# ugadiarov-la-phystech-edu/OCRL

Measured on AMD Instinct MI355X. Metric: images/sec (node) SLATE pretrain 128x128, 6 slots, 3 iters, higher is better.
Workload: dtype f32

## Files before the change

include/ocrl_hip.h:

```cpp
#ifndef OCRL_HIP_H
#define OCRL_HIP_H
#include <stddef.h>

#ifdef __cplusplus
extern "C" {
#endif

#define OCRL_ABI_VERSION 5

const char* ocrl_last_error(void);
int ocrl_abi_version(void);

typedef struct ocrl_slate ocrl_slate;
typedef struct ocrl_slate_config {
    int obs_size, obs_channels;
    int vocab_size, d_model;
    int cnn_hidden;
    int num_slots, num_iterations, slot_size, mlp_hidden;
    int num_dec_blocks, num_dec_heads;
    float dropout;
    int max_batch;
    int use_bcdec;
    int hard;
    int num_slot_heads;
} ocrl_slate_config;

size_t ocrl_slate_config_size(void);
int ocrl_slate_create(const ocrl_slate_config* cfg, ocrl_slate** out);
void ocrl_slate_destroy(ocrl_slate* h);

int ocrl_slate_param_count(const ocrl_slate* h);
int ocrl_slate_param_info(const ocrl_slate* h, int i, char* name, int name_cap, int shape[4], int* ndim,
                          long long* offset, long long* numel, int* group);
long long ocrl_slate_flat_size(const ocrl_slate* h);
long long ocrl_slate_group_begin(const ocrl_slate* h, int group);
size_t ocrl_slate_workspace_bytes(const ocrl_slate* h);

int ocrl_slate_bind(ocrl_slate* h, float* params, float* grads, float* adam_m, float* adam_v, void* workspace, size_t workspace_bytes);

int ocrl_slate_forward(ocrl_slate* h, const float* obs, int B, float tau, int train, unsigned long long seed,
                       const float* noise_z, const float* noise_zh, const float* noise_slots, void* stream);
int ocrl_slate_backward(ocrl_slate* h, void* stream);
int ocrl_slate_encode(ocrl_slate* h, const float* obs, int B, unsigned long long seed, const float* noise_slots, void* stream);
int ocrl_slate_encode_backward(ocrl_slate* h, const float* dslots, void* stream);
int ocrl_slate_freeze_weights(ocrl_slate* h, int on);
int ocrl_slate_generate(ocrl_slate* h, void* stream);
int ocrl_slate_clip_adam(ocrl_slate* h, const float lr[3], float clip, int step, float grad_scale, void* stream);
int ocrl_slate_grad_norm(ocrl_slate* h, void* stream);
float* ocrl_slate_metrics(const ocrl_slate* h);
int ocrl_slate_tensor(const ocrl_slate* h, const char* name, float** ptr, long long* count);
int ocrl_slate_soft_z(ocrl_slate* h, void* stream);
int ocrl_slate_dropout_mask(const ocrl_slate* h, unsigned site, long long n, float* out, void* stream);

int ocrl_gemm(const float* A, const float* B, float* C, int M, int N, int K, int lda, int ldb, int ldc, int akc, int bkc,
              float alpha, const float* bias, int relu, const float* mask, int ldmask, const float* resid, int ldr,
              int splitk, float* ws, void* stream);
typedef struct ocrl_gemm_desc {
    const float* A; const float* B; float* C;
    int M, N, K, lda, ldb, ldc;
    int akc, bkc;
    int batch, batch_inner;
    long long sA, sB, sC, sAi, sBi, sCi;
    int splitk; float alpha;
    const float* bias; int relu;
    float drop_p; unsigned long long drop_seed; unsigned drop_site;
    const float* mask; int ldmask; long long sMask; int mask_elu;
    const float* resid; int ldr; long long sR;
    float adrop_p; unsigned adrop_site; int adrop_ld;
    float* bias_out; long long sBias;
    int a_mode, b_mode; const float* x_lse; const int* x_tok; float x_scale;
    int epi_mode; float* stat; float* hstat; int* hidx; const float* e1; const float* e2; unsigned long long e_seed;
    const float* e_lse; const float* e_rowvec; float e_scale;
    int force_tile, force_sb;
} ocrl_gemm_desc;
size_t ocrl_gemm_desc_size(void);
int ocrl_gemm_ex(const ocrl_gemm_desc* d, float* ws, size_t ws_floats, void* stream);
int ocrl_gemm_plan(const ocrl_gemm_desc* d, int out[6]);
int ocrl_conv2d_fwd(const float* x, const float* w, const float* bias, float* y, int B, int H, int W, int cin, int cin_pad, int ks,
                    int relu, float* ws, void* stream);
int ocrl_conv2d_fwd_lowlat(const float* x, const float* w, const float* bias, float* y, int B, int H, int W, int cin, int cin_pad, int ks,
                           int relu, float* ws, void* stream);
size_t ocrl_conv2d_x3_ws_floats(void);
int ocrl_conv2d_fwd_x3(const float* x, const float* w, const float* bias, float* y, int B, int H, int W, int ks, int relu, float* ws, void* stream);
int ocrl_conv2d_bwd_data_x3(const float* dy, const float* w, const float* mask, float* dx, int B, int H, int W, int ks, float* ws, void* stream);
int ocrl_conv2d_bwd_weight_x3(const float* x, const float* dy, float* dw, int B, int H, int W, int ks, float* ws, size_t ws_floats, void* stream);
int ocrl_conv2d_bwd_data(const float* dy, const float* w, const float* mask, float* dx, int B, int H, int W, int ks, float* ws, void* stream);
size_t ocrl_conv2d_wgrad_ws_floats(int B, int H, int W, int ks, int cin_pad);
int ocrl_conv2d_bwd_weight(const float* x, const float* dy, float* dw, float* db, int B, int H, int W, int cin, int cin_pad, int ks,
                           float* ws, size_t ws_floats, void* stream);
typedef struct ocrl_conv_desc {
    const float* x; const float* w; float* y;
    int B, H, W, cin, cin_pad, ks;
    const float* bias; int relu;
    const float* posmap; const float* mask; int mask_elu;
    int transposed, low_latency;
} ocrl_conv_desc;
size_t ocrl_conv_desc_size(void);
int ocrl_conv2d_ex(const ocrl_conv_desc* d, float* ws, size_t ws_floats, void* stream);
typedef struct ocrl_conv_wgrad_desc {
    const float* x; const float* dy; float* dw; float* db;
    int B, H, W, cin, cin_pad, ks;
    int accumulate;
} ocrl_conv_wgrad_desc;
size_t ocrl_conv_wgrad_desc_size(void);
int ocrl_conv2d_bwd_weight_ex(const ocrl_conv_wgrad_desc* d, float* ws, size_t ws_floats, void* stream);
size_t ocrl_conv2d_first_fwd_ws_floats(void);
int ocrl_conv2d_first_fwd(const float* obs, const float* w, const float* bias, float* y, int B, int H, int W, int relu, float* ws, size_t ws_floats,
                          void* stream);
size_t ocrl_conv2d_first_wgrad_ws_floats(int B, int H, int W);
int ocrl_conv2d_first_bwd_weight(const float* obs, const float* dy, float* dw, float* db, int B, int H, int W, int accumulate, float* ws, size_t ws_floats,
                                 void* stream);
int ocrl_layernorm_fwd(const float* x, const float* gamma, const float* beta, float* y, float* mean, float* rstd, long long R, int F, void* stream);
int ocrl_layernorm_bwd(const float* dy, const float* x, const float* mean, const float* rstd, const float* gamma, float* dx, float* dgb,
                       long long R, int F, float* ws, size_t ws_floats, void* stream);

int ocrl_sa_input_plan(long long R, int out[3]);
int ocrl_sa_input_fwd(const float* e4, const float* gamma, const float* beta, const float* W0, const float* b0, const float* W2, const float* b2,
                      float* mean, float* rstd, float* h1, float* x, long long R, int max_wgs, void* stream);
int ocrl_sa_input_bwd(const float* dx, const float* h1, const float* e4, const float* mean, const float* rstd, const float* gamma, const float* beta,
                      const float* W0, const float* W2, float* de4, float* dW0, float* db0, float* dW2, float* db2, float* dgamma, float* dbeta,
                      long long R, int max_wgs, float* ws, size_t ws_floats, void* stream);

int ocrl_attention_fwd(const float* q, const float* k, const float* v, float* o, float* lse, int B, int T, int d, int h, int ld,
                       float p, unsigned long long seed, unsigned site, void* stream);
int ocrl_attention_bwd(const float* q, const float* k, const float* v, const float* o, const float* lse, const float* dO,
                       float* dq, float* dk, float* dv, float* delta, int B, int T, int d, int h, int ld,
                       float p, unsigned long long seed, unsigned site, void* stream);

int ocrl_obs_u8_to_f32(const unsigned char* obs_hwc, float* obs_chw, int B, int H, int W, int C, void* stream);

int ocrl_prof_enable(unsigned tag_mask);
int ocrl_prof_collect(double* ms, long long* count, int ntags);

size_t ocrl_slot_attention_ws_floats(int B, int K, int D, int H, int I);
int ocrl_slot_attention_fwd(const float* x, const float* slots0, const float* const* w, float* slots, float* attn, int B, int N, int K, int D,
                            int H, int I, float* ws, size_t ws_floats, void* stream);
int ocrl_slot_attention_bwd(const float* x, const float* dslots, float* dx, float* dslots0, float* const* dw, int B, int N, int K, int D, int H,
                            int I, float* ws, size_t ws_floats, void* stream);
size_t ocrl_slot_attention_mh_ws_floats(int B, int N, int K, int D, int H, int I, int heads);
int ocrl_slot_attention_mh_fwd(const float* x, const float* slots0, const float* const* w, float* slots, float* attn, int B, int N, int K, int D,
                               int H, int I, int heads, float* ws, size_t ws_floats, void* stream);
int ocrl_slot_attention_mh_bwd(const float* x, const float* dslots, float* dx, float* dslots0, float* const* dw, int B, int N, int K, int D, int H,
                               int I, int heads, float* ws, size_t ws_floats, void* stream);
int ocrl_slot_attention_plan(int K, int D, int H, int heads, int* out6);

#define OCRL_POOL_MAX_LAYERS 8
size_t ocrl_pool_transformer_ws_floats(int B, int K, int d, int nhead, int ff, int L);
int ocrl_pool_transformer_fwd(const float* slots, const float* const* w, const float* pos, float* out, int B, int K, int Din, int d, int nhead,
                              int ff, int L, float drop_p, unsigned long long seed, float* ws, size_t ws_floats, void* stream);
int ocrl_pool_transformer_bwd(const float* slots, const float* dout, const float* const* w, float* dslots, float* const* dw, int B, int K, int Din,
                              int d, int nhead, int ff, int L, float drop_p, unsigned long long seed, float* ws, size_t ws_floats, void* stream);
int ocrl_pool_transformer_dropout_mask(int layer, int which, long long n, float drop_p, unsigned long long seed, float* out, void* stream);
size_t ocrl_pool_transformer_long_ws_floats(int B, int K, int Din, int d, int nhead, int ff, int L);
int ocrl_pool_transformer_long_fwd(const float* slots, const float* const* w, const float* pos, float* out, int B, int K, int Din, int d, int nhead,
                                   int ff, int L, float drop_p, unsigned long long seed, float* ws, size_t ws_floats, void* stream);
int ocrl_pool_transformer_long_bwd(const float* slots, const float* dout, const float* const* w, float* dslots, float* const* dw, int B, int K,
                                   int Din, int d, int nhead, int ff, int L, float drop_p, unsigned long long seed, float* ws, size_t ws_floats,
                                   void* stream);

#define OCRL_POOL_RN_MAX_LAYERS 16
size_t ocrl_pool_rn_ws_floats(int B, int K, int D, int ng, const int* g_dims, int nf, const int* f_dims);
int ocrl_pool_rn_fwd(const float* slots, const float* const* w, float* out, int B, int K, int D, int ng, const int* g_dims, int nf, const int* f_dims,
                     float* ws, size_t ws_floats, void* stream);
int ocrl_pool_rn_bwd(const float* slots, const float* dout, const float* const* w, float* dslots, float* const* dw, int B, int K, int D, int ng,
                     const int* g_dims, int nf, const int* f_dims, float* ws, size_t ws_floats, void* stream);

#define OCRL_NATURECNN_MAX_GROUPS 16
#define OCRL_NATURECNN_MAX_CONVS 4
size_t ocrl_naturecnn_ws_floats(int B, int H, int W, int cin, int groups, int cnn_feat_size, int use_cnn_feat, int rep_dim);
int ocrl_naturecnn_fwd(const float* obs, const float* const* w, float* out, int B, int H, int W, int cin, int groups, int cnn_feat_size,
                       int use_cnn_feat, int rep_dim, int save, float* ws, size_t ws_floats, void* stream);
int ocrl_naturecnn_bwd(const float* obs, const float* dout, const float* const* w, float* const* dw, int B, int H, int W, int cin, int groups,
                       int cnn_feat_size, int use_cnn_feat, int rep_dim, float* ws, size_t ws_floats, void* stream);

size_t ocrl_pool_cnn_ws_floats(int B, int H, int W, int D, int rep_dim);
int ocrl_pool_cnn_fwd(const float* tokens, const float* const* w, float* out, int B, int H, int W, int D, int rep_dim, int save, float* ws,
                      size_t ws_floats, void* stream);
int ocrl_pool_cnn_bwd(const float* tokens, const float* dout, const float* const* w, float* dtokens, float* const* dw, int B, int H, int W, int D,
                      int rep_dim, float* ws, size_t ws_floats, void* stream);

#define OCRL_VAE_MAX_STAGES 6
size_t ocrl_vae_ws_floats(int B, int obs_size, int obs_channels, int cnn_feat_size, int latent_dim, int use_cnn_feat, int full);
int ocrl_vae_fwd(const float* obs, const float* const* w, const float* eps, float* rep, float* metrics, float* recon, int B, int obs_size,
                 int obs_channels, int cnn_feat_size, int latent_dim, int use_cnn_feat, float kld_weight, int full, float* ws, size_t ws_floats,
                 void* stream);
int ocrl_vae_bwd(const float* obs, const float* eps, const float* const* w, const float* dloss, const float* drep, float* const* dw, int B,
                 int obs_size, int obs_channels, int cnn_feat_size, int latent_dim, int use_cnn_feat, float kld_weight, int full, float* ws,
                 size_t ws_floats, void* stream);

#define OCRL_MAE_MAX_DEPTH 32
size_t ocrl_mae_ws_floats(int B, int obs_size, int patch, int D, int depth, int heads, int Dd, int ddepth, int dheads, int len_keep, int full);
int ocrl_mae_fwd(const float* obs, const float* const* w, const float* noise, float* rep, float* metrics, float* pred, float* mask,
                 int* ids_restore, int B, int obs_size, int patch, int D, int depth, int heads, int Dd, int ddepth, int dheads, int len_keep,
                 int full, float* ws, size_t ws_floats, void* stream);
int ocrl_mae_bwd(const float* obs, const float* const* w, const float* dloss, const float* drep, float* const* dw, int B, int obs_size,
                 int patch, int D, int depth, int heads, int Dd, int ddepth, int dheads, int len_keep, int full, float* ws, size_t ws_floats,
                 void* stream);
int ocrl_mae_rank(const float* noise, int* ids_restore, int* ids_keep, float* mask, int B, int L, int len_keep, void* stream);

#define OCRL_PROBE_MAX_SLOTS 12
#define OCRL_PROBE_MAX_PROPS 8
#define OCRL_PROBE_MAX_LAYERS 8
size_t ocrl_probe_ws_floats(int B, int K, int N, int D, int O, int slot_rows, int nl, const int* dims, int P);
int ocrl_probe_fwd(const float* rows, const float* const* w, const float* y, float* out, float* cost, int* col, float* metrics, int B, int K, int N,
                   int D, int T, int O, int slot_rows, int nl, const int* dims, float slope, int P, const int* tgt_range, const int* out_range,
                   const int* kind, float* ws, size_t ws_floats, void* stream);
int ocrl_probe_bwd(const float* rows, const float* dloss, const float* const* w, float* const* dw, int B, int K, int N, int D, int O, int slot_rows,
                   int nl, const int* dims, float slope, int P, float* ws, size_t ws_floats, void* stream);
size_t ocrl_probe_match_ws_floats(int B, int P);
int ocrl_probe_match(const float* out, int ld_row, long long ld_img, const float* y, const float* dloss, float* cost, int* col, float* metrics,
                     float* dout, int B, int K, int N, int T, int O, int P, const int* tgt_range, const int* out_range, const int* kind, float* ws,
                     size_t ws_floats, void* stream);

#define OCRL_ARI_MAX_CHANNELS 32
int ocrl_ari_counts(const float* truth, long long t_sb, long long t_sc, long long t_sn, int Ct, const float* pred, long long p_sb,
                    long long p_sc, long long p_sn, int Cp, int fuse_fg, int B, long long N, int* table, long long* sums, void* stream);

#define OCRL_ACNET_MAX_LAYERS 8
typedef struct {
    int B, F, A;
    int n[3];
    int dims[3][OCRL_ACNET_MAX_LAYERS];
    int acts[3][OCRL_ACNET_MAX_LAYERS];
} ocrl_acnet_desc;
size_t ocrl_acnet_desc_size(void);
size_t ocrl_acnet_ws_floats(const ocrl_acnet_desc* d);
int ocrl_acnet_fwd(const ocrl_acnet_desc* d, const float* features, const float* const* w, float* latent_pi, float* latent_vf, float* logits,
                   float* values, int save, float* ws, size_t ws_floats, void* stream);
int ocrl_acnet_bwd(const ocrl_acnet_desc* d, const float* features, const float* const* w, const float* dlatent_pi, const float* dlatent_vf,
                   const float* dlogits, const float* dvalues, float* dfeatures, float* const* dw, float* ws, size_t ws_floats, void* stream);
int ocrl_acnet_ppo_fwd_bwd(const ocrl_acnet_desc* d, const float* features, const float* const* w, const long long* actions,
                           const float* old_log_prob, const float* advantages, const float* returns, float clip_range, float vf_coef,
                           float ent_coef, int normalize_advantage, float* scalars, float* dfeatures, float* const* dw, float* ws,
                           size_t ws_floats, void* stream);
int ocrl_acnet_a2c_fwd_bwd(const ocrl_acnet_desc* d, const float* features, const float* const* w, const long long* actions,
                           const float* advantages, const float* returns, float vf_coef, float ent_coef, int normalize_advantage,
                           float* scalars, float* dfeatures, float* const* dw, float* ws, size_t ws_floats, void* stream);
int ocrl_acnet_act(const ocrl_acnet_desc* d, const float* features, const float* const* w, unsigned long long seed,
                   unsigned long long row_offset, const float* uniforms , int deterministic, long long* actions, float* values,
                   float* log_prob, float* logits , void* stream);
int ocrl_acnet_act_uniforms(unsigned long long seed, unsigned long long row_offset, long long n, float* out, void* stream);
int ocrl_gae(const float* rewards, const float* values, const float* episode_starts, const float* last_values, const float* dones,
             float* advantages, float* returns, int T, int E, float gamma, float gae_lambda, void* stream);

#define OCRL_SPRITE_MAX_OBJECTS 15
typedef struct {
    int E, H;
    int lo, hi;
    int mode;
    int rew_type;
    int occlusion, max_steps;
    int n_colors, n_shapes, n_scales;
    int colors[8], shapes[8];
    float scales[8];
    int target_color, target_shape;
    float target_scale;
    int agent_color, agent_shape;
    float agent_scale, agent_x, agent_y;
    float step_size, dist_agent, dist_objs, dist_wall;
    int task;
    int obj_comp;
    int unseen_mode;
    int unseen_colors[2];
} ocrl_sprite_env_desc;
size_t ocrl_sprite_env_desc_size(void);
size_t ocrl_sprite_env_state_floats(const ocrl_sprite_env_desc* d);
int ocrl_sprite_env_reset(const ocrl_sprite_env_desc* d, float* state, unsigned long long seed, const unsigned char* mask ,
                          long long episode, void* stream);
// ... 65 lines not shown
```

ocrl_amd/_lib.py:

```python
import ctypes
import os
from ctypes import POINTER, c_char_p, c_float, c_int, c_longlong, c_size_t, c_uint, c_ulonglong, c_void_p

_HERE = os.path.dirname(os.path.abspath(__file__))
LIB_PATH = os.environ.get("OCRL_HIP_LIB") or os.path.join(_HERE, "libocrl_hip.so")
_lib = None


class SlateConfig(ctypes.Structure):
    _fields_ = [(n, c_int) for n in ("obs_size", "obs_channels", "vocab_size", "d_model", "cnn_hidden", "num_slots",
                                      "num_iterations", "slot_size", "mlp_hidden", "num_dec_blocks", "num_dec_heads")] + \
               [("dropout", c_float), ("max_batch", c_int), ("use_bcdec", c_int), ("hard", c_int), ("num_slot_heads", c_int)]


class IodineConfig(ctypes.Structure):
    _fields_ = [(n, c_int) for n in ("obs_size", "obs_channels", "slot_size", "num_iterations", "num_slots")] + \
               [("sigma", c_float), ("beta", c_float), ("layer_norm", c_int), ("ref_mlp_hidden", c_int), ("max_batch", c_int)]


class GemmDesc(ctypes.Structure):
    _fields_ = [("A", c_void_p), ("B", c_void_p), ("C", c_void_p)] + \
               [(n, c_int) for n in ("M", "N", "K", "lda", "ldb", "ldc", "akc", "bkc", "batch", "batch_inner")] + \
               [(n, c_longlong) for n in ("sA", "sB", "sC", "sAi", "sBi", "sCi")] + \
               [("splitk", c_int), ("alpha", c_float), ("bias", c_void_p), ("relu", c_int),
                ("drop_p", c_float), ("drop_seed", c_ulonglong), ("drop_site", c_uint),
                ("mask", c_void_p), ("ldmask", c_int), ("sMask", c_longlong), ("mask_elu", c_int),
                ("resid", c_void_p), ("ldr", c_int), ("sR", c_longlong),
                ("adrop_p", c_float), ("adrop_site", c_uint), ("adrop_ld", c_int),
                ("bias_out", c_void_p), ("sBias", c_longlong),
                ("a_mode", c_int), ("b_mode", c_int), ("x_lse", c_void_p), ("x_tok", c_void_p), ("x_scale", c_float),
                ("epi_mode", c_int), ("stat", c_void_p), ("hstat", c_void_p), ("hidx", c_void_p), ("e1", c_void_p), ("e2", c_void_p),
                ("e_seed", c_ulonglong), ("e_lse", c_void_p), ("e_rowvec", c_void_p), ("e_scale", c_float),
                ("force_tile", c_int), ("force_sb", c_int)]


class ConvDesc(ctypes.Structure):
    _fields_ = [("x", c_void_p), ("w", c_void_p), ("y", c_void_p)] + \
               [(n, c_int) for n in ("B", "H", "W", "cin", "cin_pad", "ks")] + \
               [("bias", c_void_p), ("relu", c_int), ("posmap", c_void_p), ("mask", c_void_p), ("mask_elu", c_int),
                ("transposed", c_int), ("low_latency", c_int)]


class ConvWgradDesc(ctypes.Structure):
    _fields_ = [("x", c_void_p), ("dy", c_void_p), ("dw", c_void_p), ("db", c_void_p)] + \
               [(n, c_int) for n in ("B", "H", "W", "cin", "cin_pad", "ks", "accumulate")]


class AcnetDesc(ctypes.Structure):
    _fields_ = [("B", c_int), ("F", c_int), ("A", c_int), ("n", c_int * 3), ("dims", (c_int * 8) * 3), ("acts", (c_int * 8) * 3)]


class SpriteEnvDesc(ctypes.Structure):
    _fields_ = [(n, c_int) for n in ("E", "H", "lo", "hi", "mode", "rew_type", "occlusion", "max_steps", "n_colors", "n_shapes", "n_scales")] + \
               [("colors", c_int * 8), ("shapes", c_int * 8), ("scales", c_float * 8), ("target_color", c_int), ("target_shape", c_int),
                ("target_scale", c_float), ("agent_color", c_int), ("agent_shape", c_int)] + \
               [(n, c_float) for n in ("agent_scale", "agent_x", "agent_y", "step_size", "dist_agent", "dist_objs", "dist_wall")] + \
               [("task", c_int), ("obj_comp", c_int), ("unseen_mode", c_int), ("unseen_colors", c_int * 2)]


class ScenesDesc(ctypes.Structure):
    _fields_ = [("H", c_int), ("K", c_int)]


def acnet_desc(B, F, A, dims, acts):
    d = AcnetDesc(B=B, F=F, A=A)
    for t in range(3):
        if len(dims[t]) > 8:
            raise ValueError(f"ocrl_amd: at most 8 layers per trunk (got {len(dims[t])})")
        d.n[t] = len(dims[t])
        for l, (w, a) in enumerate(zip(dims[t], acts[t])):
            d.dims[t][l], d.acts[t][l] = int(w), int(a)
    return d


def gemm_desc(**kw):
    d = GemmDesc(batch=1, batch_inner=1, splitk=1, alpha=1.0, x_scale=1.0, e_scale=1.0, force_sb=-1)
    for k, v in kw.items():
        setattr(d, k, v)
    return d


def conv_desc(**kw):
    d = ConvDesc()
    for k, v in kw.items():
        setattr(d, k, v)
    return d


def conv_wgrad_desc(**kw):
    d = ConvWgradDesc()
    for k, v in kw.items():
        setattr(d, k, v)
    return d


def lib():
    global _lib
    if _lib is not None:
        return _lib
    if not os.path.exists(LIB_PATH):
        raise RuntimeError(
            f"{LIB_PATH} is missing: build it with `python -c 'import __graft_entry__ as g; g.build()'` "
            "(make -C ocrl_amd/csrc).  ocrl_amd has no CPU fallback.")
    import torch
    L = ctypes.CDLL(LIB_PATH)
    p = c_void_p
    L.ocrl_last_error.restype = c_char_p
    L.ocrl_abi_version.restype = c_int
    L.ocrl_slate_config_size.restype = c_size_t
    if L.ocrl_slate_config_size() != ctypes.sizeof(SlateConfig):
        raise RuntimeError(f"libocrl_hip.so: ocrl_slate_config is {L.ocrl_slate_config_size()} bytes, this binding's SlateConfig {ctypes.sizeof(SlateConfig)}")
    L.ocrl_slate_create.argtypes = [POINTER(SlateConfig), POINTER(p)]
    L.ocrl_slate_destroy.argtypes = [p]
    L.ocrl_slate_destroy.restype = None
    L.ocrl_slate_param_count.argtypes = [p]
    L.ocrl_slate_param_info.argtypes = [p, c_int, c_char_p, c_int, POINTER(c_int * 4), POINTER(c_int), POINTER(c_longlong),
                                        POINTER(c_longlong), POINTER(c_int)]
    L.ocrl_slate_flat_size.argtypes = [p]
    L.ocrl_slate_flat_size.restype = c_longlong
    L.ocrl_slate_group_begin.argtypes = [p, c_int]
    L.ocrl_slate_group_begin.restype = c_longlong
    L.ocrl_slate_workspace_bytes.argtypes = [p]
    L.ocrl_slate_workspace_bytes.restype = c_size_t
    L.ocrl_slate_bind.argtypes = [p, p, p, p, p, p, c_size_t]
    L.ocrl_slate_forward.argtypes = [p, p, c_int, c_float, c_int, c_ulonglong, p, p, p, p]
    L.ocrl_slate_backward.argtypes = [p, p]
    L.ocrl_slate_generate.argtypes = [p, p]
    L.ocrl_slate_encode.argtypes = [p, p, c_int, c_ulonglong, p, p]
    L.ocrl_slate_encode_backward.argtypes = [p, p, p]
    L.ocrl_slate_freeze_weights.argtypes = [p, c_int]
    L.ocrl_slate_clip_adam.argtypes = [p, POINTER(c_float * 3), c_float, c_int, c_float, p]
    L.ocrl_slate_grad_norm.argtypes = [p, p]
    L.ocrl_slate_metrics.argtypes = [p]
    L.ocrl_slate_metrics.restype = p
    L.ocrl_slate_tensor.argtypes = [p, c_char_p, POINTER(p), POINTER(c_longlong)]
    L.ocrl_slate_dropout_mask.argtypes = [p, c_uint, c_longlong, p, p]
    L.ocrl_slate_soft_z.argtypes = [p, p]
    L.ocrl_gemm.argtypes = [p, p, p, c_int, c_int, c_int, c_int, c_int, c_int, c_int, c_int, c_float, p, c_int, p, c_int, p, c_int,
                            c_int, p, p]
    L.ocrl_gemm_desc_size.restype = c_size_t
    L.ocrl_gemm_ex.argtypes = [POINTER(GemmDesc), p, c_size_t, p]
    L.ocrl_gemm_plan.argtypes = [POINTER(GemmDesc), POINTER(c_int * 6)]
    L.ocrl_conv2d_fwd.argtypes = [p, p, p, p, c_int, c_int, c_int, c_int, c_int, c_int, c_int, p, p]
    L.ocrl_conv2d_fwd_lowlat.argtypes = [p, p, p, p, c_int, c_int, c_int, c_int, c_int, c_int, c_int, p, p]
    L.ocrl_conv2d_x3_ws_floats.restype = c_size_t
    L.ocrl_conv2d_fwd_x3.argtypes = [p, p, p, p, c_int, c_int, c_int, c_int, c_int, p, p]
    L.ocrl_conv2d_bwd_data_x3.argtypes = [p, p, p, p, c_int, c_int, c_int, c_int, p, p]
    L.ocrl_conv2d_bwd_weight_x3.argtypes = [p, p, p, c_int, c_int, c_int, c_int, p, c_size_t, p]
    L.ocrl_conv2d_bwd_data.argtypes = [p, p, p, p, c_int, c_int, c_int, c_int, p, p]
    L.ocrl_conv2d_wgrad_ws_floats.argtypes = [c_int, c_int, c_int, c_int, c_int]
    L.ocrl_conv2d_wgrad_ws_floats.restype = c_size_t
    L.ocrl_conv2d_bwd_weight.argtypes = [p, p, p, p, c_int, c_int, c_int, c_int, c_int, c_int, p, c_size_t, p]
    L.ocrl_conv_desc_size.restype = c_size_t
    L.ocrl_conv_wgrad_desc_size.restype = c_size_t
    for name, cls in (("ocrl_conv_desc", ConvDesc), ("ocrl_conv_wgrad_desc", ConvWgradDesc)):
        n = getattr(L, name + "_size")()
        if n != ctypes.sizeof(cls):
            raise RuntimeError(f"libocrl_hip.so: {name} is {n} bytes, this binding's {cls.__name__} {ctypes.sizeof(cls)}")
    L.ocrl_conv2d_ex.argtypes = [POINTER(ConvDesc), p, c_size_t, p]
    L.ocrl_conv2d_bwd_weight_ex.argtypes = [POINTER(ConvWgradDesc), p, c_size_t, p]
    L.ocrl_conv2d_first_fwd_ws_floats.restype = c_size_t
    L.ocrl_conv2d_first_fwd.argtypes = [p, p, p, p, c_int, c_int, c_int, c_int, p, c_size_t, p]
    L.ocrl_conv2d_first_wgrad_ws_floats.argtypes = [c_int, c_int, c_int]
    L.ocrl_conv2d_first_wgrad_ws_floats.restype = c_size_t
    L.ocrl_conv2d_first_bwd_weight.argtypes = [p, p, p, p, c_int, c_int, c_int, c_int, p, c_size_t, p]
    L.ocrl_layernorm_fwd.argtypes = [p, p, p, p, p, p, c_longlong, c_int, p]
    L.ocrl_layernorm_bwd.argtypes = [p, p, p, p, p, p, p, c_longlong, c_int, p, c_size_t, p]
    L.ocrl_sa_input_plan.argtypes = [c_longlong, POINTER(c_int * 3)]
    L.ocrl_sa_input_fwd.argtypes = [p] * 11 + [c_longlong, c_int, p]
    L.ocrl_sa_input_bwd.argtypes = [p] * 16 + [c_longlong, c_int, p, c_size_t, p]
    L.ocrl_attention_fwd.argtypes = [p, p, p, p, p, c_int, c_int, c_int, c_int, c_int, c_float, c_ulonglong, c_uint, p]
    L.ocrl_attention_bwd.argtypes = [p, p, p, p, p, p, p, p, p, p, c_int, c_int, c_int, c_int, c_int, c_float, c_ulonglong, c_uint, p]
    L.ocrl_obs_u8_to_f32.argtypes = [p, p, c_int, c_int, c_int, c_int, p]
    L.ocrl_prof_enable.argtypes = [c_uint]
    L.ocrl_prof_collect.argtypes = [POINTER(ctypes.c_double * 8), POINTER(c_longlong * 8), c_int]
    L.ocrl_iodine_create.argtypes = [POINTER(IodineConfig), POINTER(p)]
    L.ocrl_iodine_destroy.argtypes = [p]
    L.ocrl_iodine_destroy.restype = None
    L.ocrl_iodine_param_count.argtypes = [p]
    L.ocrl_iodine_param_info.argtypes = [p, c_int, c_char_p, c_int, POINTER(c_int * 4), POINTER(c_int), POINTER(c_longlong), POINTER(c_longlong)]
    L.ocrl_iodine_flat_size.argtypes = [p]
    L.ocrl_iodine_flat_size.restype = c_longlong
    L.ocrl_iodine_workspace_bytes.argtypes = [p]
    L.ocrl_iodine_workspace_bytes.restype = c_size_t
    L.ocrl_iodine_bind.argtypes = [p, p, p, p, p, p, c_size_t]
    L.ocrl_iodine_forward.argtypes = [p, p, c_int, c_ulonglong, p, p]
    L.ocrl_iodine_backward.argtypes = [p, p]
    L.ocrl_iodine_clip_adam.argtypes = [p, c_float, c_float, c_int, c_float, p]
    L.ocrl_iodine_grad_norm.argtypes = [p, p]
    L.ocrl_iodine_metrics.argtypes = [p]
    L.ocrl_iodine_metrics.restype = p
    L.ocrl_iodine_tensor.argtypes = [p, c_char_p, POINTER(p), POINTER(c_longlong)]
    L.ocrl_slot_attention_ws_floats.argtypes = [c_int, c_int, c_int, c_int, c_int]
    L.ocrl_slot_attention_ws_floats.restype = c_size_t
    L.ocrl_slot_attention_fwd.argtypes = [p, p, POINTER(p), p, p, c_int, c_int, c_int, c_int, c_int, c_int, p, c_size_t, p]
    L.ocrl_slot_attention_bwd.argtypes = [p, p, p, p, POINTER(p), c_int, c_int, c_int, c_int, c_int, c_int, p, c_size_t, p]
    L.ocrl_slot_attention_mh_ws_floats.argtypes = [c_int] * 7
    L.ocrl_slot_attention_mh_ws_floats.restype = c_size_t
    L.ocrl_slot_attention_mh_fwd.argtypes = [p, p, POINTER(p), p, p] + [c_int] * 7 + [p, c_size_t, p]
    L.ocrl_slot_attention_mh_bwd.argtypes = [p, p, p, p, POINTER(p)] + [c_int] * 7 + [p, c_size_t, p]
    L.ocrl_slot_attention_plan.argtypes = [c_int, c_int, c_int, c_int, POINTER(c_int * 6)]
    L.ocrl_pool_transformer_ws_floats.argtypes = [c_int, c_int, c_int, c_int, c_int, c_int]
    L.ocrl_pool_transformer_ws_floats.restype = c_size_t
    L.ocrl_pool_transformer_fwd.argtypes = [p, POINTER(p), p, p, c_int, c_int, c_int, c_int, c_int, c_int, c_int, c_float, c_ulonglong, p, c_size_t, p]
    L.ocrl_pool_transformer_bwd.argtypes = [p, p, POINTER(p), p, POINTER(p), c_int, c_int, c_int, c_int, c_int, c_int, c_int, c_float, c_ulonglong, p,
                                            c_size_t, p]
    L.ocrl_pool_transformer_dropout_mask.argtypes = [c_int, c_int, c_longlong, c_float, c_ulonglong, p, p]
    L.ocrl_pool_transformer_long_ws_floats.argtypes = [c_int] * 7
    L.ocrl_pool_transformer_long_ws_floats.restype = c_size_t
    L.ocrl_pool_transformer_long_fwd.argtypes = L.ocrl_pool_transformer_fwd.argtypes
    L.ocrl_pool_transformer_long_bwd.argtypes = L.ocrl_pool_transformer_bwd.argtypes
    L.ocrl_pool_rn_ws_floats.argtypes = [c_int, c_int, c_int, c_int, POINTER(c_int), c_int, POINTER(c_int)]
    L.ocrl_pool_rn_ws_floats.restype = c_size_t
    L.ocrl_pool_rn_fwd.argtypes = [p, POINTER(p), p, c_int, c_int, c_int, c_int, POINTER(c_int), c_int, POINTER(c_int), p, c_size_t, p]
    L.ocrl_pool_rn_bwd.argtypes = [p, p, POINTER(p), p, POINTER(p), c_int, c_int, c_int, c_int, POINTER(c_int), c_int, POINTER(c_int), p, c_size_t, p]
    L.ocrl_naturecnn_ws_floats.argtypes = [c_int] * 8
    L.ocrl_naturecnn_ws_floats.restype = c_size_t
    L.ocrl_naturecnn_fwd.argtypes = [p, POINTER(p), p] + [c_int] * 9 + [p, c_size_t, p]
    L.ocrl_naturecnn_bwd.argtypes = [p, p, POINTER(p), POINTER(p)] + [c_int] * 8 + [p, c_size_t, p]
    L.ocrl_pool_cnn_ws_floats.argtypes = [c_int] * 5
    L.ocrl_pool_cnn_ws_floats.restype = c_size_t
    L.ocrl_pool_cnn_fwd.argtypes = [p, POINTER(p), p] + [c_int] * 6 + [p, c_size_t, p]
    L.ocrl_pool_cnn_bwd.argtypes = [p, p, POINTER(p), p, POINTER(p)] + [c_int] * 5 + [p, c_size_t, p]
    L.ocrl_vae_ws_floats.argtypes = [c_int] * 7
    L.ocrl_vae_ws_floats.restype = c_size_t
    L.ocrl_vae_fwd.argtypes = [p, POINTER(p), p, p, p, p] + [c_int] * 6 + [c_float, c_int, p, c_size_t, p]
    L.ocrl_vae_bwd.argtypes = [p, p, POINTER(p), p, p, POINTER(p)] + [c_int] * 6 + [c_float, c_int, p, c_size_t, p]
    L.ocrl_mae_ws_floats.argtypes = [c_int] * 11
    L.ocrl_mae_ws_floats.restype = c_size_t
    L.ocrl_mae_fwd.argtypes = [p, POINTER(p), p, p, p, p, p, p] + [c_int] * 11 + [p, c_size_t, p]
    L.ocrl_mae_bwd.argtypes = [p, POINTER(p), p, p, POINTER(p)] + [c_int] * 11 + [p, c_size_t, p]
    L.ocrl_mae_rank.argtypes = [p, p, p, p, c_int, c_int, c_int, p]
    L.ocrl_probe_ws_floats.argtypes = [c_int] * 7 + [POINTER(c_int), c_int]
    L.ocrl_probe_ws_floats.restype = c_size_t
    L.ocrl_probe_fwd.argtypes = [p, POINTER(p), p, p, p, p, p] + [c_int] * 8 + [POINTER(c_int), c_float, c_int, POINTER(c_int), POINTER(c_int),
                                 POINTER(c_int), p, c_size_t, p]
    L.ocrl_probe_bwd.argtypes = [p, p, POINTER(p), POINTER(p)] + [c_int] * 7 + [POINTER(c_int), c_float, c_int, p, c_size_t, p]
    L.ocrl_probe_match_ws_floats.argtypes = [c_int, c_int]
    L.ocrl_probe_match_ws_floats.restype = c_size_t
    L.ocrl_probe_match.argtypes = [p, c_int, c_longlong, p, p, p, p, p, p] + [c_int] * 6 + [POINTER(c_int)] * 3 + [p, c_size_t, p]
    L.ocrl_ari_counts.argtypes = [p, c_longlong, c_longlong, c_longlong, c_int, p, c_longlong, c_longlong, c_longlong, c_int, c_int, c_int, c_longlong, p, p, p]
    L.ocrl_acnet_desc_size.restype = c_size_t
    if L.ocrl_acnet_desc_size() != ctypes.sizeof(AcnetDesc):
        raise RuntimeError(f"libocrl_hip.so: ocrl_acnet_desc is {L.ocrl_acnet_desc_size()} bytes, this binding's AcnetDesc {ctypes.sizeof(AcnetDesc)}")
    L.ocrl_acnet_ws_floats.argtypes = [POINTER(AcnetDesc)]
    L.ocrl_acnet_ws_floats.restype = c_size_t
    L.ocrl_acnet_fwd.argtypes = [POINTER(AcnetDesc), p, POINTER(p), p, p, p, p, c_int, p, c_size_t, p]
    L.ocrl_acnet_bwd.argtypes = [POINTER(AcnetDesc), p, POINTER(p), p, p, p, p, p, POINTER(p), p, c_size_t, p]
    L.ocrl_acnet_ppo_fwd_bwd.argtypes = [POINTER(AcnetDesc), p, POINTER(p), p, p, p, p, c_float, c_float, c_float, c_int, p, p, POINTER(p), p, c_size_t, p]
    L.ocrl_acnet_a2c_fwd_bwd.argtypes = [POINTER(AcnetDesc), p, POINTER(p), p, p, p, c_float, c_float, c_int, p, p, POINTER(p), p, c_size_t, p]
    L.ocrl_acnet_act.argtypes = [POINTER(AcnetDesc), p, POINTER(p), c_ulonglong, c_ulonglong, p, c_int, p, p, p, p, p]
    L.ocrl_acnet_act_uniforms.argtypes = [c_ulonglong, c_ulonglong, c_longlong, p, p]
    L.ocrl_flat_clip_adam_ws_floats.argtypes = []
    L.ocrl_flat_clip_adam_ws_floats.restype = c_size_t
    L.ocrl_flat_clip_adam_l2.argtypes = [p, p, p, p, c_longlong, c_float, c_float, c_float, c_float, c_float, c_int, p, p, c_size_t, p]
    L.ocrl_flat_clip_rmsprop_ws_floats.argtypes = []
    L.ocrl_flat_clip_rmsprop_ws_floats.restype = c_size_t
    L.ocrl_flat_clip_rmsprop_l2.argtypes = [p, p, p, c_longlong, c_float, c_float, c_float, c_float, p, p, c_size_t, p]
    L.ocrl_gae.argtypes = [p, p, p, p, p, p, p, c_int, c_int, c_float, c_float, p]
    L.ocrl_sprite_env_desc_size.restype = c_size_t
    if L.ocrl_sprite_env_desc_size() != ctypes.sizeof(SpriteEnvDesc):
        raise RuntimeError(f"libocrl_hip.so: ocrl_sprite_env_desc is {L.ocrl_sprite_env_desc_size()} bytes, this binding's SpriteEnvDesc "
                           f"{ctypes.sizeof(SpriteEnvDesc)}")
    L.ocrl_sprite_env_state_floats.argtypes = [POINTER(SpriteEnvDesc)]
    L.ocrl_sprite_env_state_floats.restype = c_size_t
    L.ocrl_sprite_env_reset.argtypes = [POINTER(SpriteEnvDesc), p, c_ulonglong, p, c_longlong, p]
    L.ocrl_sprite_env_step.argtypes = [POINTER(SpriteEnvDesc), p, c_ulonglong, p, p, p, p, p, p, p]
    L.ocrl_sprite_render.argtypes = [p, c_int, c_int, c_int, c_int, p, p]
    L.ocrl_sprite_state_obs.argtypes = [p, c_int, c_int, p, p]
    L.ocrl_gt_mlp_ws_floats.argtypes = [c_int, c_int, c_int, POINTER(c_int)]
    L.ocrl_gt_mlp_ws_floats.restype = c_size_t
    L.ocrl_gt_mlp_fwd.argtypes = [p, POINTER(p), p, c_int, c_int, c_int, POINTER(c_int), POINTER(c_int), p, c_size_t, p]
    L.ocrl_gt_mlp_bwd.argtypes = [p, p, POINTER(p), p, POINTER(p), c_int, c_int, c_int, POINTER(c_int), POINTER(c_int), p, c_size_t, p]
    L.ocrl_sprite_env_uniforms.argtypes = [c_ulonglong, c_longlong, c_int, c_longlong, c_int, c_int, p, p]
    L.ocrl_scenes_batch.argtypes = [POINTER(ScenesDesc), c_ulonglong, p, c_int, p, p, p, p, p]
    L.ocrl_scenes_uniforms.argtypes = [c_ulonglong, c_longlong, c_int, c_int, p, p]
    L.ocrl_comm_unique_id.argtypes = [p, c_size_t]
    L.ocrl_comm_init.argtypes = [POINTER(p), c_int, c_int, p]
    L.ocrl_comm_allreduce.argtypes = [p, p, c_longlong, p]
    L.ocrl_comm_world.argtypes = [p]
    L.ocrl_comm_destroy.argtypes = [p]
    L.ocrl_comm_destroy.restype = None
    if L.ocrl_abi_version() != 5:
        raise RuntimeError("libocrl_hip.so ABI version mismatch")
    _lib = L
    return L


def check(rc):
    if rc:
        raise RuntimeError("ocrl_hip: " + lib().ocrl_last_error().decode())


def ptr(t):
    return None if t is None else ctypes.c_void_p(t.data_ptr())


def ptrs(ts):
    return (ctypes.c_void_p * len(ts))(*[t.data_ptr() if t is not None else None for t in ts])


def stream(device=None):
    import torch
    return ctypes.c_void_p(torch.cuda.current_stream(device).cuda_stream)
```

ocrl_amd/csrc/capi.cpp:

```cpp
#include <stdarg.h>
#include <stdint.h>
#include <string.h>

#include <new>

#include "../../include/ocrl_hip.h"
#include "iodine_model.h"
#include "slate_model.h"

static thread_local char g_err[512] = "";

void ocrl_set_error(const char* fmt, ...) {
    va_list ap;
    va_start(ap, fmt);
    vsnprintf(g_err, sizeof g_err, fmt, ap);
    va_end(ap);
}

template <class M>
struct Handle {
    using Model = M;
    M* m = nullptr;
};
struct ocrl_slate : Handle<SlateModel> {};
// ... 140 lines not shown
    a.A = d.A; a.B = d.B; a.C = d.C; a.M = d.M; a.N = d.N; a.K = d.K; a.lda = d.lda; a.ldb = d.ldb; a.ldc = d.ldc; a.akc = d.akc; a.bkc = d.bkc;
    a.batch = d.batch; a.batch_inner = d.batch_inner; a.sA = d.sA; a.sB = d.sB; a.sC = d.sC; a.sAi = d.sAi; a.sBi = d.sBi; a.sCi = d.sCi;
    a.splitk = d.splitk; a.alpha = d.alpha; a.bias = d.bias; a.relu = d.relu; a.drop_p = d.drop_p; a.drop_seed = d.drop_seed; a.drop_site = d.drop_site;
    a.mask = d.mask; a.ldmask = d.ldmask; a.sMask = d.sMask; a.mask_elu = d.mask_elu; a.resid = d.resid; a.ldr = d.ldr; a.sR = d.sR;
    a.adrop_p = d.adrop_p; a.adrop_site = d.adrop_site; a.adrop_ld = d.adrop_ld; a.bias_out = d.bias_out; a.sBias = d.sBias;
    a.a_mode = d.a_mode; a.b_mode = d.b_mode; a.x_lse = d.x_lse; a.x_tok = d.x_tok; a.x_scale = d.x_scale;
    a.epi_mode = d.epi_mode; a.stat = d.stat; a.hstat = d.hstat; a.hidx = d.hidx; a.e1 = d.e1; a.e2 = d.e2; a.e_seed = d.e_seed;
    a.e_lse = d.e_lse; a.e_rowvec = d.e_rowvec; a.e_scale = d.e_scale; a.force_tile = d.force_tile; a.force_sb = d.force_sb;
    return a;
}
size_t ocrl_gemm_desc_size(void) { return sizeof(ocrl_gemm_desc); }
int ocrl_gemm_plan(const ocrl_gemm_desc* d, int out[6]) {
    if (!d || !out) { ocrl_set_error("ocrl_gemm_plan: null argument"); return 1; }
    GemmArgs a = gemm_args(*d);
    if (a.splitk > 1) gemm_splitk_layout(a, a.C, a.sBias ? a.sBias : (a.M + 3) & ~3);
    GemmPlan p;
    if (gemm_plan(a, &p)) return 1;
    out[0] = p.bm; out[1] = p.bn; out[2] = p.sb; out[3] = p.xf; out[4] = p.epi; out[5] = p.layout;
    return 0;
}
int ocrl_gemm_ex(const ocrl_gemm_desc* d, float* ws, size_t ws_floats, void* stream) {
    if (!d) { ocrl_set_error("ocrl_gemm_ex: null descriptor"); return 1; }
    GemmArgs a = gemm_args(*d);
    if (a.splitk <= 1) return gemm_launch(a, ST(stream));
    const long long slab = (long long)a.M * a.N, bslab = a.sBias ? a.sBias : (a.M + 3) & ~3;
    const size_t need = (size_t)a.splitk * slab + (a.bias_out ? (size_t)a.splitk * bslab : 0);
    if (a.ldc != a.N || !ws || ws_floats < need || bslab % 4) {
        ocrl_set_error("ocrl_gemm_ex: split-k needs ldc == N, sBias %% 4 == 0 and a workspace of %zu floats", need);
        return 1;
    }
    if (a.bias || a.relu || a.drop_p > 0.f || a.mask || a.resid || a.epi_mode) {
        ocrl_set_error("ocrl_gemm_ex: split-k partial products take no epilogue");
        return 1;
    }
    return gemm_splitk_launch(a, ws, bslab, 0, ST(stream));
}
int ocrl_conv2d_fwd(const float* x, const float* w, const float* bias, float* y, int B, int H, int W, int cin, int cin_pad, int ks, int relu,
                    float* ws, void* stream) {
    if (conv_pack_launch(w, ws, nullptr, ks, cin_pad, 64, cin, ST(stream))) return 1;
    ConvArgs a;
    a.X = x; a.Wp = ws; a.Y = y; a.B = B; a.H = H; a.W = W; a.bias = bias; a.relu = relu;
    return conv_fwd_launch(a, ks, cin_pad, 64, ST(stream));
}
int ocrl_conv2d_fwd_lowlat(const float* x, const float* w, const float* bias, float* y, int B, int H, int W, int cin, int cin_pad, int ks, int relu,
                           float* ws, void* stream) {
    if (conv_pack_launch(w, ws, nullptr, ks, cin_pad, 64, cin, ST(stream))) return 1;
    ConvArgs a;
    a.X = x; a.Wp = ws; a.Y = y; a.B = B; a.H = H; a.W = W; a.bias = bias; a.relu = relu;
    return conv_fwd_launch(a, ks, cin_pad, 64, ST(stream), 1);
}
size_t ocrl_conv2d_x3_ws_floats(void) { return 2 * conv_x3_pack_floats(5); }
int ocrl_conv2d_fwd_x3(const float* x, const float* w, const float* bias, float* y, int B, int H, int W, int ks, int relu, float* ws, void* stream) {
    if (ks != 3 && ks != 5) { ocrl_set_error("ocrl_conv2d_fwd_x3: ks must be 3 or 5"); return 1; }
    if (conv_pack_x3_launch(w, ws, nullptr, ST(stream), ks)) return 1;
    ConvArgs a;
    a.X = x; a.Y = y; a.B = B; a.H = H; a.W = W; a.bias = bias; a.relu = relu;
    return conv_x3_launch(a, ws, ST(stream), ks);
}
int ocrl_conv2d_bwd_data_x3(const float* dy, const float* w, const float* mask, float* dx, int B, int H, int W, int ks, float* ws, void* stream) {
    if (ks != 3 && ks != 5) { ocrl_set_error("ocrl_conv2d_bwd_data_x3: ks must be 3 or 5"); return 1; }
    if (conv_pack_x3_launch(w, ws, ws + conv_x3_pack_floats(5), ST(stream), ks)) return 1;
    ConvArgs a;
    a.X = dy; a.Y = dx; a.B = B; a.H = H; a.W = W; a.mask = mask;
    return conv_x3_launch(a, ws + conv_x3_pack_floats(5), ST(stream), ks);
}
int ocrl_conv2d_bwd_data(const float* dy, const float* w, const float* mask, float* dx, int B, int H, int W, int ks, float* ws, void* stream) {
    float* bw = ws + (size_t)ks * ks * 64 * 64;
    if (conv_pack_launch(w, ws, bw, ks, 64, 64, 64, ST(stream))) return 1;
    ConvArgs a;
    a.X = dy; a.Wp = bw; a.Y = dx; a.B = B; a.H = H; a.W = W; a.mask = mask;
    return conv_fwd_launch(a, ks, 64, 64, ST(stream));
}
size_t ocrl_conv2d_wgrad_ws_floats(int B, int H, int W, int ks, int cin_pad) {
    const size_t slabs = (size_t)conv_wgrad_slabs(B, H, W, ks, cin_pad);
    return slabs * ks * ks * 64 * cin_pad + (1 << 16);
}
int ocrl_conv2d_bwd_weight(const float* x, const float* dy, float* dw, float* db, int B, int H, int W, int cin, int cin_pad, int ks, float* ws,
                           size_t ws_floats, void* stream) {
    if (ws_floats < ocrl_conv2d_wgrad_ws_floats(B, H, W, ks, cin_pad)) { ocrl_set_error("ocrl_conv2d_bwd_weight: workspace too small"); return 1; }
    WgradArgs a;
    a.X = x; a.dY = dy; a.part = ws; a.B = B; a.H = H; a.W = W;
    return conv_wgrad_launch(a, ks, cin_pad, 64, cin, dw, db, 0, ST(stream), 0);
}
int ocrl_conv2d_bwd_weight_x3(const float* x, const float* dy, float* dw, int B, int H, int W, int ks, float* ws, size_t ws_floats, void* stream) {
    if (ks != 3 && ks != 5) { ocrl_set_error("ocrl_conv2d_bwd_weight_x3: ks must be 3 or 5"); return 1; }
    if (ws_floats < ocrl_conv2d_wgrad_ws_floats(B, H, W, ks, 64)) { ocrl_set_error("ocrl_conv2d_bwd_weight_x3: workspace too small"); return 1; }
    WgradArgs a;
    a.X = x; a.dY = dy; a.part = ws; a.B = B; a.H = H; a.W = W;
    return conv_wgrad_launch(a, ks, 64, 64, 64, dw, nullptr, 0, ST(stream), 1);
}
static bool conv_kernel_built(int ks, int cin_pad) { return (ks == 5 && (cin_pad == 64 || cin_pad == 8)) || (ks == 3 && cin_pad == 64); }
static bool aligned16(const void* p) { return ((uintptr_t)p & 15) == 0; }
size_t ocrl_conv_desc_size(void) { return sizeof(ocrl_conv_desc); }
int ocrl_conv2d_ex(const ocrl_conv_desc* d, float* ws, size_t ws_floats, void* stream) {
    if (!d) { ocrl_set_error("ocrl_conv2d_ex: null descriptor"); return 1; }
    if (!d->x || !d->w || !d->y || !ws || d->B < 1 || d->H < 1 || d->W < 1) { ocrl_set_error("ocrl_conv2d_ex: x, w, y, ws and a non-empty image are required"); return 1; }
    if (!conv_kernel_built(d->ks, d->cin_pad)) { ocrl_set_error("ocrl_conv2d_ex: no kernel for ks=%d cin_pad=%d (built: 5/64, 5/8, 3/64)", d->ks, d->cin_pad); return 1; }
    if (d->cin < 1 || d->cin > d->cin_pad) { ocrl_set_error("ocrl_conv2d_ex: cin %d outside 1 .. cin_pad %d", d->cin, d->cin_pad); return 1; }
    if (d->relu < 0 || d->relu > 2) { ocrl_set_error("ocrl_conv2d_ex: relu must be 0, 1 (ReLU) or 2 (ELU), got %d", d->relu); return 1; }
    if (d->mask_elu && !d->mask) { ocrl_set_error("ocrl_conv2d_ex: mask_elu needs a mask"); return 1; }
    if (d->transposed && (d->cin != 64 || d->cin_pad != 64)) { ocrl_set_error("ocrl_conv2d_ex: the transposed (backward-data) form needs cin = cin_pad = 64"); return 1; }
    if (!aligned16(d->x) || !aligned16(d->y) || !aligned16(ws) || !aligned16(d->bias) || !aligned16(d->posmap) || !aligned16(d->mask)) {
        ocrl_set_error("ocrl_conv2d_ex: x, y, ws, bias, posmap and mask must be 16-byte aligned");
        return 1;
    }
    const size_t pack = (size_t)d->ks * d->ks * d->cin_pad * 64, need = d->transposed ? 2 * pack : pack;
    if (ws_floats < need) { ocrl_set_error("ocrl_conv2d_ex: workspace of %zu floats, %zu needed", ws_floats, need); return 1; }
    float* bw = d->transposed ? ws + pack : nullptr;
    if (conv_pack_launch(d->w, ws, bw, d->ks, d->cin_pad, 64, d->cin, ST(stream))) return 1;
    ConvArgs a;
    a.X = d->x; a.Wp = bw ? bw : ws; a.Y = d->y; a.B = d->B; a.H = d->H; a.W = d->W; a.bias = d->bias; a.relu = d->relu;
    a.posmap = d->posmap; a.mask = d->mask; a.mask_elu = d->mask_elu ? 1 : 0;
    return conv_fwd_launch(a, d->ks, d->cin_pad, 64, ST(stream), d->low_latency ? 1 : 0);
}
size_t ocrl_conv_wgrad_desc_size(void) { return sizeof(ocrl_conv_wgrad_desc); }
int ocrl_conv2d_bwd_weight_ex(const ocrl_conv_wgrad_desc* d, float* ws, size_t ws_floats, void* stream) {
    if (!d) { ocrl_set_error("ocrl_conv2d_bwd_weight_ex: null descriptor"); return 1; }
    if (!d->x || !d->dy || !d->dw || !ws || d->B < 1 || d->H < 1 || d->W < 1) { ocrl_set_error("ocrl_conv2d_bwd_weight_ex: x, dy, dw, ws and a non-empty image are required"); return 1; }
    if (!conv_kernel_built(d->ks, d->cin_pad)) { ocrl_set_error("ocrl_conv2d_bwd_weight_ex: no kernel for ks=%d cin_pad=%d (built: 5/64, 5/8, 3/64)", d->ks, d->cin_pad); return 1; }
    if (d->cin < 1 || d->cin > d->cin_pad) { ocrl_set_error("ocrl_conv2d_bwd_weight_ex: cin %d outside 1 .. cin_pad %d", d->cin, d->cin_pad); return 1; }
    if (!aligned16(d->x) || !aligned16(d->dy) || !aligned16(ws)) { ocrl_set_error("ocrl_conv2d_bwd_weight_ex: x, dy and ws must be 16-byte aligned"); return 1; }
    const size_t need = ocrl_conv2d_wgrad_ws_floats(d->B, d->H, d->W, d->ks, d->cin_pad);
    if (ws_floats < need) { ocrl_set_error("ocrl_conv2d_bwd_weight_ex: workspace of %zu floats, %zu needed", ws_floats, need); return 1; }
    const int acc = d->accumulate ? 1 : 0;
    WgradArgs a;
    a.X = d->x; a.dY = d->dy; a.part = ws; a.B = d->B; a.H = d->H; a.W = d->W;
    return conv_wgrad_launch(a, d->ks, d->cin_pad, 64, d->cin, d->dw, d->db, acc, ST(stream), 0);
}
size_t ocrl_conv2d_first_fwd_ws_floats(void) { return conv_first_pack_floats(); }
int ocrl_conv2d_first_fwd(const float* obs, const float* w, const float* bias, float* y, int B, int H, int W, int relu, float* ws, size_t ws_floats,
                          void* stream) {
    if (!obs || !w || !y || !ws || B < 1 || H < 1 || W < 1) { ocrl_set_error("ocrl_conv2d_first_fwd: obs, w, y, ws and a non-empty image are required"); return 1; }
    if (relu < 0 || relu > 1) { ocrl_set_error("ocrl_conv2d_first_fwd: relu must be 0 or 1, got %d", relu); return 1; }
    if (ws_floats < conv_first_pack_floats()) { ocrl_set_error("ocrl_conv2d_first_fwd: workspace of %zu floats, %zu needed", ws_floats, conv_first_pack_floats()); return 1; }
    if (conv_first_pack_launch(w, ws, ST(stream))) return 1;
    return conv_first_fwd_launch(obs, ws, bias, y, B, H, W, relu, ST(stream));
}
size_t ocrl_conv2d_first_wgrad_ws_floats(int B, int H, int W) { return conv_first_wgrad_ws_floats(B, H, W); }
int ocrl_conv2d_first_bwd_weight(const float* obs, const float* dy, float* dw, float* db, int B, int H, int W, int accumulate, float* ws, size_t ws_floats,
                                 void* stream) {
    if (!obs || !dy || !dw || !ws || B < 1 || H < 1 || W < 1) { ocrl_set_error("ocrl_conv2d_first_bwd_weight: obs, dy, dw, ws and a non-empty image are required"); return 1; }
    const size_t need = conv_first_wgrad_ws_floats(B, H, W);
    if (ws_floats < need) { ocrl_set_error("ocrl_conv2d_first_bwd_weight: workspace of %zu floats, %zu needed", ws_floats, need); return 1; }
    return conv_first_wgrad_launch(obs, dy, ws, dw, db, B, H, W, accumulate ? 1 : 0, ST(stream));
}
int ocrl_layernorm_fwd(const float* x, const float* g, const float* b, float* y, float* mean, float* rstd, long long R, int F, void* stream) {
    return layernorm_fwd_launch(x, g, b, y, mean, rstd, R, F, ST(stream));
}
int ocrl_layernorm_bwd(const float* dy, const float* x, const float* mean, const float* rstd, const float* g, float* dx, float* dgb, long long R,
                       int F, float* ws, size_t ws_floats, void* stream) {
    return layernorm_bwd_launch(dy, x, mean, rstd, g, dx, dgb, R, F, 0, 0, ws, ws_floats, ST(stream));
}

int ocrl_sa_input_plan(long long R, int out[3]) {
    if (!out || R <= 0) { ocrl_set_error("ocrl_sa_input_plan: needs R > 0 and an output array"); return 1; }
    sa_input_plan(R, 0, out);
    return 0;
}
int ocrl_sa_input_fwd(const float* e4, const float* gamma, const float* beta, const float* W0, const float* b0, const float* W2, const float* b2,
                      float* mean, float* rstd, float* h1, float* x, long long R, int max_wgs, void* stream) {
    return sa_input_fwd_launch(e4, gamma, beta, W0, b0, W2, b2, mean, rstd, nullptr, h1, x, R, max_wgs, ST(stream));
}
int ocrl_sa_input_bwd(const float* dx, const float* h1, const float* e4, const float* mean, const float* rstd, const float* gamma, const float* beta,
                      const float* W0, const float* W2, float* de4, float* dW0, float* db0, float* dW2, float* db2, float* dgamma, float* dbeta,
                      long long R, int max_wgs, float* ws, size_t ws_floats, void* stream) {
    return sa_input_bwd_launch(dx, h1, e4, mean, rstd, gamma, beta, W0, W2, de4, dW0, db0, dW2, db2, dgamma, dbeta, R, max_wgs, ws, ws_floats,
                               ST(stream));
}

int ocrl_attention_fwd(const float* q, const float* k, const float* v, float* o, float* lse, int B, int T, int d, int h, int ld, float p,
                       unsigned long long seed, unsigned site, void* stream) {
    AttnArgs a;
    a.q = q; a.k = k; a.v = v; a.o = o; a.lse = lse; a.B = B; a.T = T; a.d = d; a.h = h; a.ld = ld; a.p = p; a.seed = seed; a.site = site;
    return attn_launch(a, 0, ST(stream));
}
int ocrl_attention_bwd(const float* q, const float* k, const float* v, const float* o, const float* lse, const float* dO, float* dq,
                       float* dk, float* dv, float* delta, int B, int T, int d, int h, int ld, float p, unsigned long long seed,
                       unsigned site, void* stream) {
    AttnArgs a;
    a.q = q; a.k = k; a.v = v; a.o = const_cast<float*>(o); a.lse = const_cast<float*>(lse); a.B = B; a.T = T; a.d = d; a.h = h; a.ld = ld;
    a.p = p; a.seed = seed; a.site = site; a.dO = dO; a.dq = dq; a.dk = dk; a.dv = dv; a.delta = delta;
    return attn_launch(a, 1, ST(stream));
}


int ocrl_iodine_create(const ocrl_iodine_config* c, ocrl_iodine** out) {
    if (!c || !out) { ocrl_set_error("ocrl_iodine_create: null argument"); return 1; }
    if (c->obs_size < 16 || c->obs_size % 16 || c->obs_channels != 3 || c->slot_size < 4 || c->slot_size % 4 || c->slot_size > 256 ||
        c->num_iterations < 1 || c->num_slots < 1 || c->num_slots > 16 || c->ref_mlp_hidden < 64 || c->ref_mlp_hidden % 64 || c->max_batch < 1 ||
        !(c->sigma > 0.f)) {
        ocrl_set_error("ocrl_iodine_create: invalid configuration");
        return 1;
    }
    IodineConfig k;
    k.obs_size = c->obs_size; k.obs_channels = c->obs_channels; k.slot_size = c->slot_size; k.num_iters = c->num_iterations;
    k.num_slots = c->num_slots; k.sigma = c->sigma; k.beta = c->beta; k.layer_norm = c->layer_norm; k.ref_mlp_hidden = c->ref_mlp_hidden;
    k.max_batch = c->max_batch;
    return h_create(k, out);
}
void ocrl_iodine_destroy(ocrl_iodine* h) { h_destroy(h); }
int ocrl_iodine_param_count(const ocrl_iodine* h) { return h_param_count(h); }
int ocrl_iodine_param_info(const ocrl_iodine* h, int i, char* name, int name_cap, int shape[4], int* ndim, long long* offset, long long* numel) {
    return h_param_info(h, i, name, name_cap, shape, ndim, offset, numel, nullptr);
}
long long ocrl_iodine_flat_size(const ocrl_iodine* h) { return h_flat_size(h); }
size_t ocrl_iodine_workspace_bytes(const ocrl_iodine* h) { return h_workspace_bytes(h); }
int ocrl_iodine_bind(ocrl_iodine* h, float* p, float* g, float* m, float* v, void* ws, size_t n) { return h_bind(h, p, g, m, v, ws, n); }
int ocrl_iodine_forward(ocrl_iodine* h, const float* obs, int B, unsigned long long seed, const float* noise, void* stream) {
    GUARD(h);
    return h->m->forward(obs, B, seed, noise, ST(stream));
}
int ocrl_iodine_backward(ocrl_iodine* h, void* stream) { GUARD(h); return h->m->backward(ST(stream)); }
int ocrl_iodine_clip_adam(ocrl_iodine* h, float lr, float clip, int step, float gscale, void* stream) {
    GUARD(h);
    return h->m->clip_adam(lr, clip, step, gscale, ST(stream));
}
int ocrl_iodine_grad_norm(ocrl_iodine* h, void* stream) { GUARD(h); return h->m->grad_norm(ST(stream)); }
float* ocrl_iodine_metrics(const ocrl_iodine* h) { return h_metrics(h); }
int ocrl_iodine_tensor(const ocrl_iodine* h, const char* name, float** ptr, long long* count) { return h_tensor(h, name, ptr, count); }
}
```

ocrl_amd/csrc/kernels.h:

```cpp
#pragma once
#include "common.h"
#include "../../include/ocrl_hip.h"

enum { PROF_CONV5 = 0, PROF_CONV_OTHER = 1, PROF_WGRAD = 2, PROF_GEMM = 3, PROF_SA_FWD = 4, PROF_SA_BWD = 5, PROF_ATTN_FWD = 6, PROF_ATTN_BWD = 7, PROF_NTAGS = 8 };
int prof_begin(int tag, hipStream_t st);
void prof_end(int idx, hipStream_t st);

struct GemmArgs {
    const float* A = nullptr;
    const float* B = nullptr;
    float* C = nullptr;
    int M = 0, N = 0, K = 0;
    int lda = 0, ldb = 0, ldc = 0;
    int akc = 1, bkc = 1;
    int batch = 1;
    int batch_inner = 1;
    long long sA = 0, sB = 0, sC = 0;
    long long sAi = 0, sBi = 0, sCi = 0;
    int splitk = 1;
    long long sCsplit = 0;
    float alpha = 1.f;
    const float* bias = nullptr;
    int relu = 0;
    float drop_p = 0.f;
// ... 69 lines not shown
int rn_pairsum_fwd_launch(const float* gL, float* y, int B, int P, int g, hipStream_t st);
int rn_pairsum_bwd_launch(const float* dy, const float* gL, float* dgL, int B, int P, int g, hipStream_t st);

struct NcMap { long long sN = 0, sG = 0, sC = 0, sH = 0, sW = 0; };
struct NcFwdArgs {
    const float* X = nullptr; NcMap x;
    float* Y = nullptr; float* Y2 = nullptr; NcMap y;
    const float* w[OCRL_NATURECNN_MAX_GROUPS] = {}; const float* bias[OCRL_NATURECNN_MAX_GROUPS] = {};
    int B = 0, G = 1, cin = 0, cout = 0, H = 0, W = 0, OH = 0, OW = 0, ks = 0, stride = 0;
    int pad = 0;
};
struct NcBwdArgs {
    const float* X = nullptr; NcMap x;
    const float* dY = nullptr; NcMap dy;
    float* dX = nullptr;
    float* part = nullptr;
    int slabs = 1, slab_rows = 0;
    const float* w[OCRL_NATURECNN_MAX_GROUPS] = {};
    int B = 0, G = 1, cin = 0, cout = 0, H = 0, W = 0, OH = 0, OW = 0, ks = 0, stride = 0;
    int pad = 0;
    long long dw_tiles = 0, dx_tiles = 0; int dw_blocks = 0;
};
struct NcReduceLayer { const float* part = nullptr; int slabs = 0, G = 0, cout = 0, K = 0; long long n = 0; };
struct NcReduceArgs {
    NcReduceLayer L[OCRL_NATURECNN_MAX_CONVS];
    float* dw[OCRL_NATURECNN_MAX_CONVS][OCRL_NATURECNN_MAX_GROUPS] = {};
    float* db[OCRL_NATURECNN_MAX_CONVS][OCRL_NATURECNN_MAX_GROUPS] = {};
    int nlayers = 0;
};
int nc_conv_fwd_launch(const NcFwdArgs& a, hipStream_t st);
int nc_conv_bwd_launch(NcBwdArgs a, hipStream_t st);
int nc_dw_reduce_launch(const NcReduceArgs& a, hipStream_t st);
int nc_relu_mask_launch(const float* d, const float* act, float* out, long long n, hipStream_t st);

struct PcGeom {
    int OH = 0, OW = 0, OWT = 0;
    int NG = 0, nchunk = 0;
    size_t wp_floats = 0;
    long long units = 0; int slab_units = 0, slabs = 0; size_t part_floats = 0;
    int passes = 0, nbg = 0, Dp = 0; size_t wd_floats = 0;
    int HB = 0, WB = 0, WT = 0; long long dx_units = 0; int upw = 0;
};
PcGeom pc_geom(int B, int H, int W, int D);
struct PcFwdArgs {
    const float* X = nullptr; const float* Wp = nullptr; const float* bias = nullptr; float* Y = nullptr;
    int B = 0, H = 0, W = 0, D = 0, OH = 0, OW = 0, OWT = 0, nchunk = 0, NG = 0;
};
struct PcDwArgs {
    const float* X = nullptr; const float* dY = nullptr; float* part = nullptr; float* partb = nullptr;
    int B = 0, H = 0, W = 0, D = 0, OH = 0, OW = 0, OWT = 0, nchunk = 0, slab_units = 0;
    long long units = 0;
};
struct PcDxArgs {
    const float* dY = nullptr; const float* Wd = nullptr; float* dX = nullptr;
    int H = 0, W = 0, D = 0, OH = 0, OW = 0, HB = 0, WT = 0, Dp = 0, passes = 0, upw = 0;
    long long units = 0, groups = 0;
};
int pc_conv1_fwd_launch(const float* X, const float* w, const float* bias, float* Wp, float* Y, int B, int H, int W, int D, hipStream_t st);
int pc_conv1_dw_launch(const float* X, const float* dY, float* part, int B, int H, int W, int D, hipStream_t st);
int pc_conv1_dw_reduce_launch(const float* part, float* dw, float* db, int B, int H, int W, int D, hipStream_t st);
int pc_conv1_dx_launch(const float* dY, const float* w, float* Wd, float* dX, int B, int H, int W, int D, hipStream_t st);

#define PROBE_MAX_SLOTS 12
#define PROBE_MAX_PROPS 8
#define PROBE_MAX_WIDTH 256
struct ProbeSchema { int P; int t[PROBE_MAX_PROPS], a[PROBE_MAX_PROPS], b[PROBE_MAX_PROPS], kind[PROBE_MAX_PROPS]; };
int probe_schema_check(const ProbeSchema& sc, int T, int O);
int probe_match_check(int B, int K, int N, int T, int O);
int probe_match_launch(const float* out, int ld_row, long long ld_img, const float* y, const float* dloss, float* cost, int* col, float* part,
                       float* metrics, float* dout, int B, int K, int N, int T, int O, const ProbeSchema& sc, hipStream_t st);
int probe_leaky_fwd_launch(float* x, long long n, float slope, hipStream_t st);
int probe_leaky_bwd_launch(float* dx, const float* h, long long n, float slope, hipStream_t st);

int vae_permute_launch(const float* src, float* dst, long long R, int C, int HW, int rows, int pack, hipStream_t st);
int vae_pad_rows_launch(const float* src, float* dst, int rows, int rows_pad, int K, hipStream_t st);
int vae_kl_fwd_launch(const float* ml, const float* eps, float* latent, float* part, float* rep, int B, int L, hipStream_t st);
int vae_loss_launch(const float* part, float* metrics, int B, float kld_weight, hipStream_t st);
int vae_kl_bwd_launch(const float* ml, const float* eps, const float* dlat, const float* drep, const float* dloss, float* dml, int B, int L,
                      float kld_weight, hipStream_t st);
int vae_scale_launch(const float* x, float* y, const float* g, long long n, hipStream_t st);
int vae_recon_nchw_launch(const float* r4, float* out, int B, int C, int HW, hipStream_t st);

#define MAE_MAX_PATCHES 1024
int mae_rank_launch(const float* noise, int* restore, int* keep, float* mask, int* restore_out, float* mask_out, int B, int L, int len_keep,
                    hipStream_t st);
int mae_patch_gather_launch(const float* obs, const int* ids, float* out, int B, int n, int S, int p, hipStream_t st);
int mae_tokens_fwd_launch(const float* embed, const float* cls, const float* pos, const int* ids, float* x0, int B, int n, int D, hipStream_t st);
int mae_tokens_bwd_launch(const float* dx0, float* dembed, float* dcls, int B, int n, int D, hipStream_t st);
int mae_unshuffle_fwd_launch(const float* e, const float* mtok, const float* dpos, const int* restore, float* xd, int B, int L, int len_keep, int Dd,
                             hipStream_t st);
int mae_unshuffle_bwd_launch(const float* dxd, const int* keep, const float* mask, float* de, float* dmtok, float* part, int B, int L, int len_keep,
                             int Dd, hipStream_t st);
int mae_gelu_fwd_launch(const float* pre, float* y, long long n, hipStream_t st);
int mae_gelu_bwd_launch(const float* dy, const float* pre, float* dpre, long long n, hipStream_t st);
int mae_ln_fwd_launch(const float* x, const float* g, const float* b, float* y, float* mean, float* rstd, long long R, int F, float eps, hipStream_t st);
int mae_ln_chunks(long long R);
int mae_ln_bwd_launch(const float* dy, const float* x, const float* mean, const float* rstd, const float* g, const float* resid, float* dx, float* dg,
                      float* db, float* part, long long R, int F, hipStream_t st);
int mae_loss_launch(const float* pred, const float* obs, const float* mask, const float* dloss, float* part, float* loss, float* dpred, int B, int L,
                    int len_keep, int S, int p, hipStream_t st);

struct ConvArgs {
    const float* X = nullptr;
    const float* Wp = nullptr;
    float* Y = nullptr;
    int B = 0, H = 0, W = 0;
    const float* bias = nullptr;
    int relu = 0;
    const float* posmap = nullptr;
    const float* mask = nullptr;
    int mask_elu = 0;
};
size_t conv_x3_pack_floats(int KS = 5);
int conv_pack_x3_launch(const float* W, float* fwd3, float* bwd3, hipStream_t st, int KS = 5);
int conv_x3_launch(const ConvArgs& a, const float* pack3, hipStream_t st, int KS = 5);
struct WgradArgs;
int conv_wgrad_x3_stage(const WgradArgs& a, int nchunk, hipStream_t st, int KS = 5);
struct WgradArgs {
    const float* X = nullptr;
    const float* dY = nullptr;
    float* part = nullptr;
    int B = 0, H = 0, W = 0;
    float* bpart = nullptr;
};
int conv_fwd_launch(const ConvArgs& a, int KS, int CIN, int COUT, hipStream_t st, int low_latency = 0);
int conv_wgrad_launch(const WgradArgs& a, int KS, int CIN, int COUT, int cin_real, float* dW, float* db, int accumulate, hipStream_t st, int x3 = -1);
int conv_wgrad_slabs(int B, int H, int W, int KS, int CIN);
size_t conv_wgrad_ws_floats(int B, int H, int W, int KS, int CIN, bool with_db = true);
int conv_pack_launch(const float* W, float* fwd, float* bwd, int KS, int CIN, int COUT, int cin_real, hipStream_t st);

size_t conv_first_pack_floats();
int conv_first_pack_launch(const float* W, float* pack, hipStream_t st);
int conv_first_fwd_launch(const float* obs, const float* pack, const float* bias, float* Y, int B, int H, int W, int relu, hipStream_t st);
int conv_first_wgrad_workers(int B, int H, int W);
size_t conv_first_wgrad_ws_floats(int B, int H, int W);
int conv_first_wgrad_launch(const float* obs, const float* dY, float* ws, float* dW, float* db, int B, int H, int W, int accumulate, hipStream_t st);

int nchw_to_nhwc8_launch(const float* in, float* out, int B, int C, int H, int W, hipStream_t st);
int patchify4_launch(const float* in, float* out, int B, int C, int S, hipStream_t st);
int pixel_shuffle_launch(const float* in, float* out, int B, int h, int w, int Cout, int forward, const float* mask, hipStream_t st);
int layernorm_fwd_launch(const float* x, const float* g, const float* b, float* y, float* mean, float* rstd, long long R, int F, hipStream_t st);
int layernorm_bwd_launch(const float* dy, const float* x, const float* mean, const float* rstd, const float* g, float* dx,
                         float* dgb, long long R, int F, int accumulate_dx, int accumulate_dgb, float* ws, size_t ws_floats, hipStream_t st);
int colsum_launch(const float* X, long long ld, float* out, long long R, int F, int accumulate, float scale, float* ws, size_t ws_floats, hipStream_t st);

#define SA_INPUT_SLAB (2 * 4096 + 4 * 64)
void sa_input_plan(long long R, int max_wgs, int out[3]);
int sa_input_fwd_launch(const float* e4, const float* gamma, const float* beta, const float* W0, const float* b0, const float* W2, const float* b2,
                        float* mean, float* rstd, float* ln0, float* h1, float* x, long long R, int max_wgs, hipStream_t st);
int sa_input_bwd_launch(const float* dx, const float* h1, const float* e4, const float* mean, const float* rstd, const float* gamma, const float* beta,
                        const float* W0, const float* W2, float* de4, float* dW0, float* db0, float* dW2, float* db2, float* dgamma, float* dbeta,
                        long long R, int max_wgs, float* ws, size_t ws_floats, hipStream_t st);
int reduce_partials_launch(const float* part, int n, float* out, float scale, int accumulate, hipStream_t st);
int mse_launch(const float* obs, const float* recon, float* drecon, float* out, int B, int C, int H, int W, float* ws, size_t ws_floats, hipStream_t st);
int gumbel_softmax_launch(const float* raw, const float* e1, const float* e2, float* z, int* tokens, long long R, int V, float tau,
                          unsigned long long seed, hipStream_t st, float* zst = nullptr);
int softmax_bwd_rows_launch(const float* z, float* d, long long R, int V, float scale, hipStream_t st);
int softmax_stat_combine_launch(const float* stat, int nseg, long long R, float* lse, const float* hstat, const int* hidx, int* tokens,
                                const float* pred, int ldp, const int* tok, float* out, float scale, float* ws, size_t ws_floats, hipStream_t st,
                                const float* cdf_scores = nullptr, int cdf_V = 0, float cdf_tau = 1.f, unsigned long long cdf_seed = 0);
int exp_rows_launch(const float* y, const float* lse, float* z, long long R, int V, hipStream_t st);
int rowdot_bias64_launch(const float* g, const float* act, const float* bias, long long R, float* out, hipStream_t st);
int embed_fwd_launch(const int* tokens, const float* dict, const float* bos, const float* pe, float* out, int B, int T, int d, float p,
                     unsigned long long seed, hipStream_t st);
size_t embed_bwd_ws_floats(long long BT, int V, int d);
int embed_bwd_launch(float* g, const int* tokens, float* ddict, int B, int T, int V, int d, float p, unsigned long long seed, float* ws,
                     size_t ws_floats, hipStream_t st);
int dropout_apply_launch(const float* x, float* y, long long n, float p, unsigned long long seed, unsigned site, hipStream_t st);
int dropout_mask_launch(float* y, long long n, float p, unsigned long long seed, unsigned site, hipStream_t st);
int cross_attn_fwd_launch(const float* Q, const float* Km, const float* Vm, float* O, float* P, int B, int T, int K, int d, int h, float p,
                          unsigned long long seed, unsigned site, hipStream_t st);
size_t cross_attn_bwd_ws_floats(int B, int T, int K, int d, int h);
int cross_attn_bwd_launch(const float* dO, const float* Q, const float* Km, const float* Vm, const float* P, float* dQ, float* dKm, float* dVm,
                          int B, int T, int K, int d, int h, float p, unsigned long long seed, unsigned site, float* part, size_t part_floats,
                          hipStream_t st);
int obs_u8_to_f32_launch(const unsigned char* in, float* out, int B, int H, int W, int C, hipStream_t st);
int fill_launch(float* x, long long n, float v, hipStream_t st);
int axpy_launch(const float* x, float* y, long long n, float a, hipStream_t st);
int posmap_launch(const float* Wpos, const float* bpos, float* out, int S, int C, hipStream_t st);
int posgrid_launch(float* out, int S, hipStream_t st);
int im2col5_launch(const float* x8, float* col, long long npix, int H, int W, int C, int ldc, hipStream_t st);
int unpack5_launch(const float* dWp, float* dW, int C, int ldc, hipStream_t st);
int pad_cols_launch(const float* in, int ldi, float* out, int ldo, long long R, int C, int Cout, hipStream_t st);

bool xattn_supported(int K, int d, int h);
int xattn_kp(int K, int h);
struct XaFoldHost {
    const float* mem = nullptr;
    const float* Wq[8]; const float* Wk[8]; const float* Wv[8]; const float* Wo[8];
    float* ck[8]; float* cv[8];
    float* Ab[8]; float* AbT[8]; float* Vo[8]; float* VoT[8];
    int B = 0, K = 0, d = 0, h = 0, nblk = 0;
};
int xattn_fold_fwd_launch(const XaFoldHost& f, hipStream_t st);
struct XaHost {
    const float* x = nullptr;
    const float* resid = nullptr;
    float* y = nullptr;
    float* P = nullptr;
    const float *Ab = nullptr, *AbT = nullptr, *Vo = nullptr, *VoT = nullptr;
    const float* gd = nullptr;
    float *Pd = nullptr, *dS = nullptr;
    int B = 0, T = 0, K = 0, d = 0, h = 0;
    float p = 0.f; unsigned long long seed = 0; unsigned site_p = 0, site_o = 0;
};
int xattn_launch(const XaHost& h, int backward, hipStream_t st);


struct SaWts {
    int ln_in_g, ln_in_b, ln_s_g, ln_s_b, ln_m_g, ln_m_b;
    int Wq, WqT, Wk, WkT, Wv, WvT, Wih, WihT, Whh, WhhT, bih, bhh, W0, W0T, b0, W2, W2T, b2;
    int total;
};
static inline SaWts sa_wts_layout(int C, int D, int H) {
    SaWts o; int a = 0;
    auto take = [&](int n) { int r = a; a += (n + 3) & ~3; return r; };
    o.ln_in_g = take(C); o.ln_in_b = take(C); o.ln_s_g = take(D); o.ln_s_b = take(D); o.ln_m_g = take(D); o.ln_m_b = take(D);
    o.Wq = take(D * D); o.WqT = take(D * D); o.Wk = take(D * C); o.WkT = take(C * D); o.Wv = take(D * C); o.WvT = take(C * D);
    o.Wih = take(3 * D * D); o.WihT = take(3 * D * D); o.Whh = take(3 * D * D); o.WhhT = take(3 * D * D);
    o.bih = take(3 * D); o.bhh = take(3 * D);
    o.W0 = take(H * D); o.W0T = take(H * D); o.b0 = take(H); o.W2 = take(D * H); o.W2T = take(D * H); o.b2 = take(D);
    o.total = a;
    return o;
}
struct SaSave { int sprev, sn, q, u, r, z, n, hn, sg, m, hid, qp, up, upn, csum, ld; };
static inline SaSave sa_save_layout(int C, int D, int H, int NH = 1) {
    SaSave o;
    o.sprev = 0; o.sn = D; o.q = 2 * D; o.u = 3 * D; o.r = 4 * D; o.z = 5 * D; o.n = 6 * D; o.hn = 7 * D; o.sg = 8 * D; o.m = 9 * D;
    o.hid = 10 * D; o.qp = 10 * D + H; o.up = o.qp + NH * C; o.upn = o.up + NH * C; o.csum = o.upn + NH * C; o.ld = o.csum + ((NH + 3) & ~3);
    return o;
}
struct SaGrad { int out, hid, gi, gh, u, q, qp, ld; };
static inline SaGrad sa_grad_layout(int C, int D, int H, int NH = 1) {
    SaGrad o;
    o.out = 0; o.hid = D; o.gi = D + H; o.gh = 4 * D + H; o.u = 7 * D + H; o.q = 8 * D + H; o.qp = 9 * D + H; o.ld = 9 * D + H + NH * C;
    return o;
}
struct SlotAttnArgs {
    int B = 0, N = 0, C = 64, K = 0, D = 0, H = 0, I = 0;
    int NH = 1;
    float eps = 1e-8f, scale = 1.f;
    const float* x = nullptr;
    const float* slots0 = nullptr;
    const float* wts = nullptr;
    float* slots = nullptr;
    float* attn = nullptr;
    float* attn_heads = nullptr;
    float* save = nullptr;
    const float* dslots = nullptr;
    float* dx = nullptr;
    float* dslots0 = nullptr;
    float* grows = nullptr;
    float* g_small = nullptr;
    float* xchg = nullptr;
    float* parts = nullptr;
    int phase = 0;
};
size_t sa_xchg_floats_host(int K, int D);
size_t sa_parts_floats_host(int B, int K);
struct SaPlan { int G, NB, KB, KS; size_t smem_fwd, smem_bwd; };
int sa_plan(int K, int D, int H, int NH, SaPlan* plan);
int slot_attn_launch(const SlotAttnArgs& a, int backward, hipStream_t st);

struct PackEntry { const float* src; int rows, cols, dst_off, transpose; };
int pack_launch(const PackEntry* entries_dev, int n_entries, int max_elems, float* dst, hipStream_t st);

int absmax_launch(const float* g, long long n, float* out, float* ws, size_t ws_floats, hipStream_t st);
int clip_adam_launch(float* p, const float* g, float* m, float* v, long long n, const float* norm, float clip, float lr, double b1,
                     double b2, double eps, int step, float gscale, hipStream_t st);
int clip_adam_tail_launch(float* p, const float* g, float* m, float* v, int n, const float* norm, float clip, float lr, double b1, double b2,
                          double eps, int step, float gscale, hipStream_t st);
int clip_rmsprop_launch(float* p, const float* g, float* sq, long long n, const float* norm, float clip, float lr, double alpha, double eps,
                        hipStream_t st);
int clip_rmsprop_tail_launch(float* p, const float* g, float* sq, int n, const float* norm, float clip, float lr, double alpha, double eps,
                             hipStream_t st);
int store_u64_launch(unsigned long long* dst, unsigned long long v, hipStream_t st);
int slot_init_launch(const float* mu, const float* logsig, const float* noise, float* slots0, int BK, int D, unsigned long long seed, hipStream_t st,
                     const unsigned long long* seed_dev = nullptr);
int slot_init_bwd_launch(const float* dslots0, const float* logsig, const float* noise, float* dmu, float* dlogsig, int BK, int D, unsigned long long seed, hipStream_t st);
int copy_launch(const float* src, float* dst, long long n, hipStream_t st);
int argmax_pos_launch(const float* pred, int* tokens, int B, int T, int V, int t, hipStream_t st, int dense_rows = 0);
int embed_step_launch(const int* tokens, const float* dict, const float* bos, const float* pe, float* out, int B, int T, int d, int t, hipStream_t st);
int decode_attn_launch(const float* qkv, float* out, int B, int T, int t, int d, int h, int ld, hipStream_t st);
int onehot_launch(const int* tokens, float* z, long long rows, int V, hipStream_t st);

struct AttnArgs {
    const float *q = nullptr, *k = nullptr, *v = nullptr;
    float* o = nullptr;
    float* lse = nullptr;
    int B = 0, T = 0, d = 0, h = 0;
    int ld = 0;
    float p = 0.f;
    unsigned long long seed = 0;
    unsigned site = 0;
    const float* dO = nullptr;
    float *dq = nullptr, *dk = nullptr, *dv = nullptr, *delta = nullptr;
};
int attn_launch(const AttnArgs& a, int mode, hipStream_t st);

enum { BCAST_L1_RELU = 0, BCAST_L1_ELU = 1 };
int bcast_l1_class_sum_launch(const float* in, float* out, long long BK, int ks, int forward, hipStream_t st);
int bcast_l1_fwd_launch(const float* P1, const float* T, const float* bias, float* c1, long long BK, int S, int ks, int act, hipStream_t st);
size_t bcast_l1_bwd_ws_floats(long long BK, int S, int ks);
int bcast_l1_bwd_launch(const float* g, float* dT, long long BK, int S, int ks, float* ws, size_t ws_floats, hipStream_t st);
int bc_posconv_launch(const float* Wc, float* P1, int S, hipStream_t st);
int bc_posconv_bwd_launch(const float* G, float* dWc, int S, hipStream_t st);
// ... 38 lines not shown
```

ocrl_amd/csrc/slate_model.cpp:

```cpp
#include "slate_model.h"

#include <stdlib.h>

#include <math.h>
#include <stdarg.h>
#include <string.h>

static std::string fmt(const char* f, ...) {
    char buf[256];
    va_list ap;
    va_start(ap, f);
    vsnprintf(buf, sizeof buf, f, ap);
    va_end(ap);
    return buf;
}

SlateModel::SlateModel(const SlateConfig& c) : cfg(c) {
    S = c.obs_size; E = S / 4; T = E * E; N = S * S; V = c.vocab; d = c.d_model; C = c.cnn_hidden;
    K = c.num_slots; I = c.num_iters; D = c.slot_size; H = c.mlp_hidden; NB = c.num_blocks; NH = c.num_heads;
    DH = d / NH; Bmax = c.max_batch; SH = c.slot_heads > 0 ? c.slot_heads : 1;
    const int ch = c.obs_channels;
    add_param("_dvae._encoder.0.m.weight", {64, ch, 4, 4}, 0); add_param("_dvae._encoder.0.m.bias", {64}, 0);
    for (int i = 1; i < 7; ++i) { add_param(fmt("_dvae._encoder.%d.m.weight", i), {64, 64, 1, 1}, 0); add_param(fmt("_dvae._encoder.%d.m.bias", i), {64}, 0); }
    add_param("_dvae._encoder.7.weight", {V, 64, 1, 1}, 0); add_param("_dvae._encoder.7.bias", {V}, 0);
// ... 41 lines not shown
        add_param(p + "ffn_layer_norm.weight", {d}, 2); add_param(p + "ffn_layer_norm.bias", {d}, 2);
        add_param(p + "ffn.0.weight", {4 * d, d}, 2); add_param(p + "ffn.0.bias", {4 * d}, 2);
        add_param(p + "ffn.2.weight", {d, 4 * d}, 2); add_param(p + "ffn.2.bias", {d}, 2);
    }
    add_param("_tfdec.layer_norm.weight", {d}, 2); add_param("_tfdec.layer_norm.bias", {d}, 2);
    add_param("_out.weight", {V, d}, 2);

    finish_params(group_begin_, 3);
    resolve_params();
    blk_.resize(NB);
    layout_workspace(false);
}

void SlateModel::resolve_params() {
    Weights& w = w_;
    for (int i = 0; i < 8; ++i) w.dvae_enc[i] = ref_pair(fmt(i < 7 ? "_dvae._encoder.%d.m" : "_dvae._encoder.%d", i));
    for (int i = 0; i < 12; ++i)
        if (i != 5 && i != 10) w.dvae_dec[i] = ref_pair(fmt(i < 11 ? "_dvae._decoder.%d.m" : "_dvae._decoder.%d", i));
    for (int i = 0; i < 4; ++i) w.enc[i] = ref_pair(fmt(i < 3 ? "_enc._encoder.%d.m" : "_enc._encoder.%d", i));
    w.enc_pos = ref_pair("_enc_pos.channels_map");
    w.sa.mu = ref("_slotattn.slot_mu"); w.sa.log_sigma = ref("_slotattn.slot_log_sigma");
    w.sa.ln = ref_pair("_slotattn.layer_norm"); w.sa.mlp0 = ref_pair("_slotattn.mlp.0"); w.sa.mlp2 = ref_pair("_slotattn.mlp.2");
    const std::string sa = "_slotattn.slot_attention.";
    w.sa.norm_inputs = ref_pair(sa + "norm_inputs"); w.sa.norm_slots = ref_pair(sa + "norm_slots"); w.sa.norm_mlp = ref_pair(sa + "norm_mlp");
    w.sa.q = ref(sa + "project_q.weight"); w.sa.k = ref(sa + "project_k.weight"); w.sa.v = ref(sa + "project_v.weight");
    w.sa.gru_wih = ref(sa + "gru.weight_ih"); w.sa.gru_whh = ref(sa + "gru.weight_hh");
    w.sa.gru_bih = ref(sa + "gru.bias_ih"); w.sa.gru_bhh = ref(sa + "gru.bias_hh");
    w.sa.m0 = ref_pair(sa + "mlp.0"); w.sa.m2 = ref_pair(sa + "mlp.2");
    w.slotproj = ref("_slotproj.weight");
    if (cfg.use_bcdec) {
        for (int i = 0; i < 4; ++i) w.bc[i] = ref_pair(fmt(i < 3 ? "_dec._decoder.%d.m" : "_dec._decoder.%d", i));
        w.bc_pos = ref_pair("_dec._pos_emb.channels_map");
    }
    w.dict = ref("_dict.dictionary.weight"); w.bos = ref("_bos_token._bos_token"); w.pe = ref("_z_pos.pe");
    w.blk.resize(NB);
    for (int b = 0; b < NB; ++b) {
        const std::string p = fmt("_tfdec.blocks.%d.", b);
        DecBlockW& k = w.blk[b];
        k.ln1 = ref_pair(p + "self_attn_layer_norm"); k.ln2 = ref_pair(p + "encoder_decoder_attn_layer_norm"); k.ln3 = ref_pair(p + "ffn_layer_norm");
        k.qkv = ref(p + "self_attn.proj_q.weight"); k.o = ref(p + "self_attn.proj_o.weight");
        k.cq = ref(p + "encoder_decoder_attn.proj_q.weight"); k.ck = ref(p + "encoder_decoder_attn.proj_k.weight");
        k.cv = ref(p + "encoder_decoder_attn.proj_v.weight"); k.co = ref(p + "encoder_decoder_attn.proj_o.weight");
        k.ffn0 = ref_pair(p + "ffn.0"); k.ffn2 = ref_pair(p + "ffn.2");
    }
    w.lnf = ref_pair("_tfdec.layer_norm"); w.out = ref("_out.weight");
    w.enc_grads_end = group_begin_[2];
    for (const ParamInfo& q : params_)
        if (q.group == 1 && (q.name.rfind("_slotproj.", 0) == 0 || q.name.rfind("_dec.", 0) == 0) && q.offset < w.enc_grads_end) w.enc_grads_end = q.offset;
}

SlateModel::~SlateModel() {
    if (ev_fork_) (void)hipEventDestroy(ev_fork_);
    if (ev_join_) (void)hipEventDestroy(ev_join_);
    if (ev_tokens_) (void)hipEventDestroy(ev_tokens_);
    if (side_) (void)hipStreamDestroy(side_);
    for (auto& kv : enc_graphs_) if (kv.second.exec) (void)hipGraphExecDestroy(kv.second.exec);
    for (hipEvent_t e : ev_dw_) if (e) (void)hipEventDestroy(e);
    if (ev_join2_) (void)hipEventDestroy(ev_join2_);
    if (side2_) (void)hipStreamDestroy(side2_);
    if (cap_) (void)hipStreamDestroy(cap_);
}

void SlateModel::layout_workspace(bool commit) {
    begin_layout(commit);
    x3_of_.clear();
    const size_t B = Bmax, BT = B * T, BN = B * N, BK = B * K;
    metrics_ = carve("metrics", 64);
    scratch_floats_ = 0;
    {
        size_t need = conv_wgrad_ws_floats((int)(B * (cfg.use_bcdec ? K : 1)), S, S, 5, 64) + (size_t)512 * 2304 * 2;
        if (conv_first_wgrad_ws_floats((int)B, S, S) > need) need = conv_first_wgrad_ws_floats((int)B, S, S);
        size_t sk = (size_t)32 * V * d + (size_t)(1 << 20);
        if (sk > need) need = sk;
        size_t cs = (size_t)N * C * 8 + (size_t)T * d * 8 + (1 << 20);
        if (cs > need) need = cs;
        if (cfg.use_bcdec && bcast_l1_bwd_ws_floats((long long)BK, S, 5) > need) need = bcast_l1_bwd_ws_floats((long long)BK, S, 5);
        const size_t ca = cross_attn_bwd_ws_floats((int)B, T, K, d, NH), eb = embed_bwd_ws_floats((long long)B * T, V, d);
        if (ca > need) need = ca;
        if (eb > need) need = eb;
        scratch_floats_ = need + (1 << 20);
    }
    scratch_ = carve(nullptr, scratch_floats_);
    scratch2_ = cfg.use_bcdec ? scratch_ : carve(nullptr, scratch_floats_);
    obs8_ = first_direct() ? nullptr : carve("obs8", BN * 8);
    obs_keep_ = first_direct() ? carve(nullptr, BN * cfg.obs_channels) : nullptr;
    obs_stage_ = carve(nullptr, (B < 32 ? B : 32) * (size_t)cfg.obs_channels * N);
    seed_dev_ = reinterpret_cast<unsigned long long*>(carve(nullptr, 64));
    e1_ = carve("enc1", BN * 64); e2_ = carve("enc2", BN * 64); e3_ = carve("enc3", BN * 64); e4_ = carve("feats", BN * 64);
    posmap_ = carve(nullptr, (size_t)N * C); gridT_ = carve(nullptr, (size_t)N * 4);
    ln0_ = carve(nullptr, BN * 64); ln0_mean_ = carve(nullptr, BN); ln0_rstd_ = carve(nullptr, BN);
    h1_ = carve("sa_mlp_hidden", BN * 64); x_ = carve("sa_inputs", BN * 64);
    slots0_ = carve("slots0", BK * D); slot_noise_ = carve(nullptr, BK * D); slots_ = carve("slots", BK * D);
    attn_ = carve("attn", BN * K);
    attn_heads_ = SH > 1 ? carve(nullptr, BN * K * SH) : nullptr;
    const SaSave so = sa_save_layout(C, D, H, SH);
    const SaGrad go = sa_grad_layout(C, D, H, SH);
    const SaWts wo = sa_wts_layout(C, D, H);
    sa_save_ = carve("sa_save", BK * I * so.ld);
    sa_grows_ = carve(nullptr, BK * I * go.ld);
    sa_wts_ = carve(nullptr, wo.total);
    sa_small_ = carve(nullptr, B * (4 * D + 2 * C));
    sa_xchg_ = carve(nullptr, B * sa_xchg_floats_host(K * SH, D));
    sa_parts_ = carve(nullptr, sa_parts_floats_host((int)B, K * SH));
    sa_pack_dev_ = reinterpret_cast<PackEntry*>(carve(nullptr, 64 * sizeof(PackEntry) / 4 + 64));
    for (int i = 0; i < 4; ++i) {
        const int cin = i == 0 ? 8 : 64;
        cw_fwd_[i] = carve(nullptr, (size_t)25 * cin * 64);
        cw_bwd_[i] = i == 0 ? nullptr : carve(nullptr, (size_t)25 * 64 * 64);
        if (conv_x3_ < 0) { const char* e = getenv("OCRL_CONV_X3"); conv_x3_ = e ? atoi(e) : 0; }
        if (conv_x3_ && i > 0) {
            float* f3 = carve(nullptr, conv_x3_pack_floats());
            float* b3 = carve(nullptr, conv_x3_pack_floats());
            if (ws_commit_) { x3_of_[cw_fwd_[i]] = f3; x3_of_[cw_bwd_[i]] = b3; }
        }
    }
    gslots_ = carve(nullptr, BK * D); gslots0_ = carve(nullptr, BK * D);
    gA_ = carve(nullptr, BN * 64); gB_ = carve(nullptr, BN * 64); gC_ = cfg.use_bcdec ? gA_ : carve(nullptr, BN * 64);
    gmap_ = carve(nullptr, (size_t)N * C);
    if (cfg.use_bcdec) {
        const size_t BKN = BK * (size_t)N;
        bc_Wc_ = carve(nullptr, 25 * 64 * 5 + 64); bc_W1r_ = carve(nullptr, (size_t)25 * 64 * D); bc_P1_ = carve(nullptr, (size_t)N * 64);
        bc_M_ = carve(nullptr, BK * 1600); bc_T_ = carve(nullptr, BK * 1600);
        bc_c1_ = carve("bc_c1", BKN * 64); bc_c2_ = carve("bc_c2", BKN * 64); bc_c3_ = carve("bc_c3", BKN * 64);
        bc_out4_ = carve(nullptr, BKN * 4); bc_dout4_ = carve(nullptr, BKN * 4);
        bc_gA_ = carve(nullptr, BKN * 64); bc_gB_ = carve(nullptr, BKN * 64);
        for (int i = 0; i < 2; ++i) {
            bc_pk_[i] = carve(nullptr, 25 * 64 * 64); bc_pkb_[i] = carve(nullptr, 25 * 64 * 64);
            if (conv_x3_ > 0) {
                float* f3 = carve(nullptr, conv_x3_pack_floats());
                float* b3 = carve(nullptr, conv_x3_pack_floats());
                if (ws_commit_) { x3_of_[bc_pk_[i]] = f3; x3_of_[bc_pkb_[i]] = b3; }
            }
        }
        bc_Wk4_ = carve(nullptr, 9 * 64 * 4); bc_Wb4_ = carve(nullptr, 9 * 64 * 4);
        bc_dW1r_ = carve(nullptr, (size_t)25 * 64 * D); bc_dWc_ = carve(nullptr, 25 * 64 * 5 + 64);
        bc_dT_ = carve(nullptr, BK * 1600); bc_dM_ = carve(nullptr, BK * 1600); bc_G1_ = carve(nullptr, (size_t)N * 64);
        recon_ = carve("recon", BN * 4);
    } else {
    patches_ = carve("patches", BT * 16 * cfg.obs_channels);
    for (int i = 0; i < 7; ++i) de_[i] = carve(fmt("dvae_enc%d", i).c_str(), BT * 64);
    zraw_ = carve("zraw", BT * V);
    z_ = carve("z", BT * V);
    zdec_ = cfg.hard ? carve("z_st", BT * V) : z_;
    tokens_ = reinterpret_cast<int*>(carve("tokens", BT));
    {
        const size_t nseg = (size_t)gemm_stat_segments(V);
        zstat_ = carve(nullptr, BT * nseg * 2); zhstat_ = carve(nullptr, BT * nseg); zhidx_ = reinterpret_cast<int*>(carve(nullptr, BT * nseg));
        zlse_ = carve("z_lse", BT); zdot_ = carve(nullptr, BT);
        cestat_ = carve(nullptr, BT * nseg * 2); celse_ = carve("ce_lse", BT); cepart_ = carve(nullptr, BT / 16 + 16);
    }
    dd0_ = carve("dvae_dec0", BT * 64); dd1_ = carve("dvae_dec1", BT * 64); dd2_ = carve("dvae_dec2", BT * 64); dd3_ = carve("dvae_dec3", BT * 64);
    dd4_ = carve("dvae_dec4", BT * 256); ps1_ = carve(nullptr, BT * 256);
    dd6_ = carve("dvae_dec6", BT * 256); dd7_ = carve("dvae_dec7", BT * 256); dd8_ = carve("dvae_dec8", BT * 256);
    dd9_ = carve("dvae_dec9", BT * 1024); ps2_ = carve(nullptr, BN * 64);
    recon_ = carve("recon", BN * 4); drecon_ = carve(nullptr, BN * 4);
    for (int i = 0; i < 2; ++i) {
        dw_fwd_[i] = carve(nullptr, 9 * 64 * 64); dw_bwd_[i] = carve(nullptr, 9 * 64 * 64);
        if (conv_x3_ > 0) {
            float* f3 = carve(nullptr, conv_x3_pack_floats(3));
            float* b3 = carve(nullptr, conv_x3_pack_floats(3));
            if (ws_commit_) { x3_of_[dw_fwd_[i]] = f3; x3_of_[dw_bwd_[i]] = b3; }
        }
    }
    w11p_ = carve(nullptr, 4 * 64);
    mem_ = carve("mem", BK * d); emb_ = carve("emb", BT * d);
    for (int b = 0; b < NB; ++b) {
        Blk& k = blk_[b];
        k.ln1 = carve(nullptr, BT * d); k.ln1_mean = carve(nullptr, BT); k.ln1_rstd = carve(nullptr, BT);
        k.q = carve(nullptr, BT * 3 * d); k.k = k.q + d; k.v = k.q + 2 * d;
        k.lse = carve(nullptr, B * NH * (size_t)T); k.ao = carve(nullptr, BT * d); k.x1 = carve(nullptr, BT * d);
        k.ln2 = carve(nullptr, BT * d); k.ln2_mean = carve(nullptr, BT); k.ln2_rstd = carve(nullptr, BT);
        k.cq = carve(nullptr, BT * d); k.ck = carve(nullptr, BK * d); k.cv = carve(nullptr, BK * d);
        k.cP = carve(nullptr, B * NH * (size_t)T * K); k.cao = carve(nullptr, BT * d); k.x2 = carve(nullptr, BT * d);
        k.ln3 = carve(nullptr, BT * d); k.ln3_mean = carve(nullptr, BT); k.ln3_rstd = carve(nullptr, BT);
        k.f1 = carve(fmt("blk%d.ffn_hidden", b).c_str(), BT * 4 * d); k.x3 = carve(nullptr, BT * d);
    }
    bg_.resize(NB);
    {
        const size_t NC = xattn_supported(K, d, NH) ? (size_t)NH * xattn_kp(K, NH) : 16;
        xa_zero_base_ = carve_pos();
        for (int b = 0; b < NB; ++b) {
            Blk& k = blk_[b];
            k.xaAb = carve(nullptr, B * NC * d); k.xaAbT = carve(nullptr, B * NC * d); k.xaVo = carve(nullptr, B * NC * d); k.xaVoT = carve(nullptr, B * NC * d);
        }
        xa_zero_floats_ = (size_t)(carve_pos() - xa_zero_base_);
        for (int b = 0; b < NB; ++b) { bg_[b].xaPd = carve(nullptr, BT * NC); bg_[b].xaDs = carve(nullptr, BT * NC); }
        xa_dAb_ = carve(nullptr, B * NC * d); xa_dVo_ = carve(nullptr, B * NC * d);
        xa_pq_ = carve(nullptr, B * (size_t)d * d); xa_po_ = carve(nullptr, B * (size_t)d * d);
    }
    attn_delta_ = carve(nullptr, B * NH * (size_t)T);
    lnf_ = carve("dec_out", BT * d); lnf_mean_ = carve(nullptr, BT); lnf_rstd_ = carve(nullptr, BT);
    pred_ = carve("pred", BT * V);
    gx_ = carve(nullptr, BT * d); gbr_ = carve(nullptr, BT * d); gt1_ = carve(nullptr, BT * d); gt2_ = carve(nullptr, BT * d);
    gt3_ = carve(nullptr, BT * d); gf1_ = carve(nullptr, BT * 4 * d); gqkv_ = carve(nullptr, BT * 3 * d);
    for (int b = 0; b < NB; ++b) {
        BlkG& q = bg_[b];
        if (b == 0) { q.gbr[0] = gbr_; q.gf1 = gf1_; q.gt2 = gt2_; q.gqkv = gqkv_; }
        else { q.gbr[0] = carve(nullptr, BT * d); q.gf1 = carve(nullptr, BT * 4 * d); q.gt2 = carve(nullptr, BT * d); q.gqkv = carve(nullptr, BT * 3 * d); }
        q.gbr[1] = carve(nullptr, BT * d); q.gbr[2] = carve(nullptr, BT * d);
    }
    scratch3_ = carve(nullptr, scratch_floats_);
    gmem_ = carve(nullptr, BK * d); gck_ = carve(nullptr, BK * d); gcv_ = carve(nullptr, BK * d);
    gdA_ = carve(nullptr, BN * 64); gdB_ = carve(nullptr, BN * 64);
    }
    col0_ = dw0p_ = nullptr;
    if (!first_direct()) {
        const int ldc0 = (25 * cfg.obs_channels + 3) & ~3;
        col0_ = carve(nullptr, BN * ldc0); dw0p_ = carve(nullptr, (size_t)64 * ldc0);
    }
    end_layout();
}

int SlateModel::bind(float* p, float* g, float* m, float* v, void* ws, size_t ws_bytes) {
    RC(check_buffers(p, g, ws, ws_bytes));
    OCRL_REQUIRE(d % 64 == 0 && d <= 256 && D % 64 == 0 && C == 64 && V % 256 == 0 && S % 4 == 0 && d % NH == 0 && DH % 4 == 0 && DH <= 64,
                 "unsupported configuration (d_model/slot_size multiples of 64 <= 256, cnn hidden 64, vocab %% 256, obs_size %% 4)");
    OCRL_REQUIRE(cfg.obs_channels == 3, "obs_channels must be 3");
    OCRL_REQUIRE(T % 4 == 0, "obs_size/4 squared must be a multiple of 4");
    adopt_buffers(p, g, m, v, ws);
    clear_encode_graphs();
    packs_valid_ = false;
    layout_workspace(true);
    if (!side_) {
        const char* e = getenv("OCRL_OVERLAP");
        overlap_mode_ = e ? atoi(e) : 5;
        if (overlap_mode_) {
            OCRL_HIP(hipStreamCreateWithFlags(&side_, hipStreamNonBlocking));
            OCRL_HIP(hipEventCreateWithFlags(&ev_fork_, hipEventDisableTiming));
            OCRL_HIP(hipEventCreateWithFlags(&ev_join_, hipEventDisableTiming));
            OCRL_HIP(hipEventCreateWithFlags(&ev_tokens_, hipEventDisableTiming));
            const char* w = getenv("OCRL_DW_SIDE");
            dw_mode_ = (overlap_mode_ >= 3 && !cfg.use_bcdec) ? (w ? atoi(w) : 2) : 0;
            if (dw_mode_) {
                for (hipEvent_t& ev : ev_dw_) OCRL_HIP(hipEventCreateWithFlags(&ev, hipEventDisableTiming));
                OCRL_HIP(hipEventCreateWithFlags(&ev_join2_, hipEventDisableTiming));
                if (dw_mode_ == 2) OCRL_HIP(hipStreamCreateWithFlags(&side2_, hipStreamNonBlocking));
            }
        }
    }
    {
        const char* e = getenv("OCRL_SA_INPUT");
        sa_input_ = e ? atoi(e) : 1;
    }
    {
        const char* e = getenv("OCRL_XATTN");
        xattn_ = !cfg.use_bcdec && xattn_supported(K, d, NH) && (e ? atoi(e) != 0 : true);
        if (!cfg.use_bcdec && xa_zero_floats_) OCRL_HIP(hipMemset(xa_zero_base_, 0, xa_zero_floats_ * sizeof(float)));
    }
    RC(posgrid_launch(gridT_, S, 0));
    RC(fill_launch(recon_, (long long)Bmax * N * 4, 0.f, 0));
    const SaWts wo = sa_wts_layout(C, D, H);
    const SlotAttnW& sa = w_.sa;
    std::vector<PackEntry> ent;
    auto e = [&](ParamRef r, int rows, int cols, int off, int tr) {
        PackEntry x; x.src = P(r); x.rows = rows; x.cols = cols; x.dst_off = off; x.transpose = tr;
        ent.push_back(x);
    };
    e(sa.norm_inputs.w, 1, C, wo.ln_in_g, 0); e(sa.norm_inputs.b, 1, C, wo.ln_in_b, 0);
    e(sa.norm_slots.w, 1, D, wo.ln_s_g, 0); e(sa.norm_slots.b, 1, D, wo.ln_s_b, 0);
    e(sa.norm_mlp.w, 1, D, wo.ln_m_g, 0); e(sa.norm_mlp.b, 1, D, wo.ln_m_b, 0);
    e(sa.q, D, D, wo.Wq, 2); e(sa.q, D, D, wo.WqT, 3);
    e(sa.k, D, C, wo.Wk, 2); e(sa.k, D, C, wo.WkT, 3);
    e(sa.v, D, C, wo.Wv, 2); e(sa.v, D, C, wo.WvT, 3);
    e(sa.gru_wih, 3 * D, D, wo.Wih, 2); e(sa.gru_wih, 3 * D, D, wo.WihT, 3);
    e(sa.gru_whh, 3 * D, D, wo.Whh, 2); e(sa.gru_whh, 3 * D, D, wo.WhhT, 3);
    e(sa.gru_bih, 1, 3 * D, wo.bih, 0); e(sa.gru_bhh, 1, 3 * D, wo.bhh, 0);
    e(sa.m0.w, H, D, wo.W0, 2); e(sa.m0.w, H, D, wo.W0T, 3); e(sa.m0.b, 1, H, wo.b0, 0);
    e(sa.m2.w, D, H, wo.W2, 2); e(sa.m2.w, D, H, wo.W2T, 3); e(sa.m2.b, 1, D, wo.b2, 0);
    sa_pack_n_ = (int)ent.size();
    sa_pack_max_ = 3 * D * D;
    OCRL_REQUIRE(sa_pack_n_ <= 64, "pack table overflow");
    OCRL_HIP(hipMemcpy(sa_pack_dev_, ent.data(), ent.size() * sizeof(PackEntry), hipMemcpyHostToDevice));
    OCRL_HIP(hipDeviceSynchronize());
    have_fwd_ = false;
    return 0;
}

int SlateModel::soft_z(hipStream_t st) {
    if (!fused_heads() || cfg.use_bcdec) return 0;
    OCRL_REQUIRE(have_scores_, "soft_z: no forward since the last backward (the scores have been overwritten by their gradient)");
    return exp_rows_launch(zraw_, zlse_, z_, (long long)last_.B * T, V, st);
}
int SlateModel::dropout_mask(unsigned site, long long n, float* out, hipStream_t st) const {
    return dropout_mask_launch(out, n, pdrop_, last_.seed, site, st);
}

int SlateModel::conv_layer_fwd(const float* x, const float* pack, const float* bias, float* y, int Bn, int Hh, int Ww, int KS, int CIN,
                               int relu, const float* posmap, const float* mask, const Lane& L) {
    ConvArgs a;
    a.X = x; a.Wp = pack; a.Y = y; a.B = Bn; a.H = Hh; a.W = Ww; a.bias = bias; a.relu = relu; a.posmap = posmap; a.mask = mask;
    if (conv_x3_ > 0 && (KS == 5 || KS == 3) && CIN == 64 && !conv_lowlat_) {
        auto it = x3_of_.find(pack);
        if (it != x3_of_.end()) return conv_x3_launch(a, it->second, L, KS);
    }
    return conv_fwd_launch(a, KS, CIN, 64, L, conv_lowlat_);
}
int SlateModel::conv_layer_wgrad(const float* x, const float* dy, float* dW, float* db, int Bn, int Hh, int Ww, int KS, int CIN,
                                 int cin_real, const Lane& L) {
    WgradArgs a;
    a.X = x; a.dY = dy; a.part = L.scratch; a.B = Bn; a.H = Hh; a.W = Ww;
    OCRL_REQUIRE(conv_wgrad_ws_floats(Bn, Hh, Ww, KS, CIN) <= L.scratch_floats, "conv wgrad: scratch too small");
    const bool x3 = conv_x3_ > 0 && CIN == 64;
    RC(conv_wgrad_launch(a, KS, CIN, 64, cin_real, dW, x3 ? nullptr : db, 0, L, x3 ? 1 : 0));
    if (db && x3) RC(colsum_launch(dy, 64, db, (long long)Bn * Hh * Ww, 64, 0, 1.f, L.scratch, L.scratch_floats, L));
    return 0;
}

int SlateModel::pack_weights(const Lane& L, bool encoder_only) {
    if (first_direct()) RC(conv_first_pack_launch(P(w_.enc[0].w), cw_fwd_[0], L));
    else RC(conv_pack_launch(P(w_.enc[0].w), cw_fwd_[0], nullptr, 5, 8, 64, cfg.obs_channels, L));
    RC(conv_pack_launch(P(w_.enc[1].w), cw_fwd_[1], cw_bwd_[1], 5, 64, 64, 64, L));
    RC(conv_pack_launch(P(w_.enc[2].w), cw_fwd_[2], cw_bwd_[2], 5, 64, 64, 64, L));
    RC(conv_pack_launch(P(w_.enc[3].w), cw_fwd_[3], cw_bwd_[3], 5, 64, 64, 64, L));
    if (conv_x3_ > 0) {
        for (int i = 1; i < 4; ++i) {
            auto f = x3_of_.find(cw_fwd_[i]), b = x3_of_.find(cw_bwd_[i]);
            if (f != x3_of_.end()) RC(conv_pack_x3_launch(P(w_.enc[i].w), const_cast<float*>(f->second), b != x3_of_.end() ? const_cast<float*>(b->second) : nullptr, L));
        }
    }
    if (!cfg.use_bcdec && !encoder_only) {
        RC(conv_pack_launch(P(w_.dvae_dec[1].w), dw_fwd_[0], dw_bwd_[0], 3, 64, 64, 64, L));
        RC(conv_pack_launch(P(w_.dvae_dec[6].w), dw_fwd_[1], dw_bwd_[1], 3, 64, 64, 64, L));
        if (conv_x3_ > 0) {
            for (int i = 0; i < 2; ++i) {
                auto f = x3_of_.find(dw_fwd_[i]), b = x3_of_.find(dw_bwd_[i]);
                if (f != x3_of_.end()) RC(conv_pack_x3_launch(P(w_.dvae_dec[i ? 6 : 1].w), const_cast<float*>(f->second), b != x3_of_.end() ? const_cast<float*>(b->second) : nullptr, L, 3));
            }
        }
        RC(copy_launch(P(w_.dvae_dec[11].w), w11p_, cfg.obs_channels * 64, L));
        RC(fill_launch(w11p_ + cfg.obs_channels * 64, (4 - cfg.obs_channels) * 64, 0.f, L));
    }
    RC(pack_launch(sa_pack_dev_, sa_pack_n_, sa_pack_max_, sa_wts_, L));
    RC(posmap_launch(P(w_.enc_pos.w), P(w_.enc_pos.b), posmap_, S, C, L));
    return 0;
}

int SlateModel::fwd_encoder(const StepInputs& in, const Lane& L, int fork_dvae) {
    const int B = in.B;
    const long long BN = (long long)B * N;
    auto fork_here = [&]() -> int {
        RC(after(dvae_lane(), L, ev_fork_));
        return fwd_dvae(in, dvae_lane());
    };
    RC(slot_init_launch(P(w_.sa.mu), P(w_.sa.log_sigma), in.noise_slots, slots0_, B * K, D, in.seed, L, in.seed_dev));
    SlotAttnArgs a;
    a.B = B; a.N = N; a.C = C; a.K = K; a.D = D; a.H = H; a.I = I; a.NH = SH; a.eps = 1e-8f; a.scale = 1.0f / sqrtf((float)(D / SH));
    a.x = x_; a.slots0 = slots0_; a.wts = sa_wts_; a.slots = slots_; a.attn = attn_; a.attn_heads = attn_heads_; a.save = sa_save_;
    if (conv_lowlat_ && frozen_) a.save = nullptr;
    a.xchg = sa_xchg_; a.parts = sa_parts_;
    a.phase = 1;
    RC(slot_attn_launch(a, 0, L));
    if (fork_dvae == 2) RC(fork_here());
    if (first_direct()) {
        RC(conv_first_fwd_launch(in.obs, cw_fwd_[0], P(w_.enc[0].b), e1_, B, S, S, 1, L));
        if (!(conv_lowlat_ && frozen_))
            OCRL_HIP(hipMemcpyAsync(obs_keep_, in.obs, (size_t)BN * cfg.obs_channels * sizeof(float), hipMemcpyDeviceToDevice, L));
    } else {
        RC(nchw_to_nhwc8_launch(in.obs, obs8_, B, cfg.obs_channels, S, S, L));
        RC(conv_layer_fwd(obs8_, cw_fwd_[0], P(w_.enc[0].b), e1_, B, S, S, 5, 8, 1, nullptr, nullptr, L));
    }
    RC(conv_layer_fwd(e1_, cw_fwd_[1], P(w_.enc[1].b), e2_, B, S, S, 5, 64, 1, nullptr, nullptr, L));
    RC(conv_layer_fwd(e2_, cw_fwd_[2], P(w_.enc[2].b), e3_, B, S, S, 5, 64, 1, nullptr, nullptr, L));
    RC(conv_layer_fwd(e3_, cw_fwd_[3], P(w_.enc[3].b), e4_, B, S, S, 5, 64, 0, posmap_, nullptr, L));
    if (fork_dvae == 3) RC(fork_here());
    if (sa_input_ && C == 64 && !(conv_lowlat_ && frozen_)) {
        RC(sa_input_fwd_launch(e4_, P(w_.sa.ln.w), P(w_.sa.ln.b), P(w_.sa.mlp0.w),
                               P(w_.sa.mlp0.b), P(w_.sa.mlp2.w), P(w_.sa.mlp2.b), ln0_mean_, ln0_rstd_,
                               sa_input_ == 2 ? ln0_ : nullptr, h1_, x_, BN, 0, L));
    } else {
        RC(layernorm_fwd_launch(e4_, P(w_.sa.ln.w), P(w_.sa.ln.b), ln0_, ln0_mean_, ln0_rstd_, BN, C, L));
        RC(lin_fwd(ln0_, C, P(w_.sa.mlp0.w), P(w_.sa.mlp0.b), h1_, C, BN, C, C, 1, nullptr, 0, 0.f, 0, L));
        RC(lin_fwd(h1_, C, P(w_.sa.mlp2.w), P(w_.sa.mlp2.b), x_, C, BN, C, C, 0, nullptr, 0, 0.f, 0, L));
    }
    if (fork_dvae == 1) RC(fork_here());
    a.phase = 2;
    RC(slot_attn_launch(a, 0, L));
    return 0;
}

int SlateModel::fwd_dvae(const StepInputs& in, const Lane& L) {
    const int B = in.B;
    const long long BT = (long long)B * T, BN = (long long)B * N;
    const int ch = cfg.obs_channels;
    RC(patchify4_launch(in.obs, patches_, B, ch, S, L));
    RC(lin_fwd(patches_, 16 * ch, P(w_.dvae_enc[0].w), P(w_.dvae_enc[0].b), de_[0], 64, BT, 64, 16 * ch, 1, nullptr, 0, 0.f, 0, L));
    for (int i = 1; i < 7; ++i)
        RC(lin_fwd(de_[i - 1], 64, P(w_.dvae_enc[i].w), P(w_.dvae_enc[i].b), de_[i], 64, BT, 64, 64, 1, nullptr, 0, 0.f, 0, L));
    if (fused_heads()) {
        GemmArgs a;
        a.A = de_[6]; a.B = P(w_.dvae_enc[7].w); a.C = zraw_; a.M = (int)BT; a.N = V; a.K = 64; a.lda = 64; a.ldb = 64; a.ldc = V;
        a.bias = P(w_.dvae_enc[7].b);
        a.epi_mode = 2; a.stat = zstat_; a.hstat = zhstat_; a.hidx = zhidx_; a.e1 = in.noise_z; a.e2 = in.noise_zh; a.e_seed = in.seed;
        a.e_scale = 1.0f / in.tau;
        RC(gemm_launch(a, L));
        RC(softmax_stat_combine_launch(zstat_, gemm_stat_segments(V), BT, zlse_, zhstat_, zhidx_, tokens_, nullptr, 0, nullptr, nullptr, 0.f, nullptr, 0, L,
                                       in.noise_z ? nullptr : zraw_, V, in.tau, in.seed));
        have_scores_ = true;
    } else {
    RC(lin_fwd(de_[6], 64, P(w_.dvae_enc[7].w), P(w_.dvae_enc[7].b), zraw_, V, BT, V, 64, 0, nullptr, 0, 0.f, 0, L));
    RC(gumbel_softmax_launch(zraw_, in.noise_z, in.noise_zh, z_, tokens_, BT, V, in.tau, in.seed, L, cfg.hard ? zdec_ : nullptr));
    }
    if (side_ && L.st == side_ && ev_tokens_) OCRL_HIP(hipEventRecord(ev_tokens_, L.st));
    RC(dvae_decode(B, drecon_, L));
    return 0;
}

int SlateModel::dvae_decode(int B, float* drecon, const Lane& L, const float* zin) {
    const long long BT = (long long)B * T, BN = (long long)B * N;
    const int ch = cfg.obs_channels;
    if (!zin && fused_heads()) {
        GemmArgs a;
        a.A = zraw_; a.B = P(w_.dvae_dec[0].w); a.C = dd0_; a.M = (int)BT; a.N = 64; a.K = V; a.lda = V; a.ldb = V; a.ldc = 64;
        a.bias = P(w_.dvae_dec[0].b); a.relu = 1; a.a_mode = 2; a.x_lse = zlse_;
        RC(gemm_launch(a, L));
    } else {
    if (!zin) zin = zdec_;
    RC(lin_fwd(zin, V, P(w_.dvae_dec[0].w), P(w_.dvae_dec[0].b), dd0_, 64, BT, 64, V, 1, nullptr, 0, 0.f, 0, L));
    }
    RC(conv_layer_fwd(dd0_, dw_fwd_[0], P(w_.dvae_dec[1].b), dd1_, B, E, E, 3, 64, 1, nullptr, nullptr, L));
    RC(lin_fwd(dd1_, 64, P(w_.dvae_dec[2].w), P(w_.dvae_dec[2].b), dd2_, 64, BT, 64, 64, 1, nullptr, 0, 0.f, 0, L));
    RC(lin_fwd(dd2_, 64, P(w_.dvae_dec[3].w), P(w_.dvae_dec[3].b), dd3_, 64, BT, 64, 64, 1, nullptr, 0, 0.f, 0, L));
    RC(lin_fwd(dd3_, 64, P(w_.dvae_dec[4].w), P(w_.dvae_dec[4].b), dd4_, 256, BT, 256, 64, 1, nullptr, 0, 0.f, 0, L));
    RC(pixel_shuffle_launch(dd4_, ps1_, B, E, E, 64, 1, nullptr, L));
    RC(conv_layer_fwd(ps1_, dw_fwd_[1], P(w_.dvae_dec[6].b), dd6_, B, 2 * E, 2 * E, 3, 64, 1, nullptr, nullptr, L));
    RC(lin_fwd(dd6_, 64, P(w_.dvae_dec[7].w), P(w_.dvae_dec[7].b), dd7_, 64, 4 * BT, 64, 64, 1, nullptr, 0, 0.f, 0, L));
    RC(lin_fwd(dd7_, 64, P(w_.dvae_dec[8].w), P(w_.dvae_dec[8].b), dd8_, 64, 4 * BT, 64, 64, 1, nullptr, 0, 0.f, 0, L));
    RC(lin_fwd(dd8_, 64, P(w_.dvae_dec[9].w), P(w_.dvae_dec[9].b), dd9_, 256, 4 * BT, 256, 64, 1, nullptr, 0, 0.f, 0, L));
    RC(pixel_shuffle_launch(dd9_, ps2_, B, 2 * E, 2 * E, 64, 1, nullptr, L));
    RC(lin_fwd(ps2_, 64, P(w_.dvae_dec[11].w), P(w_.dvae_dec[11].b), recon_, 4, BN, ch, 64, 0, nullptr, 0, 0.f, 0, L));
    RC(mse_launch(last_.obs, recon_, drecon, metrics_ + (drecon ? 0 : 4), B, ch, S, S, L.scratch, L.scratch_floats, L));
    return 0;
}

AttnArgs SlateModel::self_attn_args(int b) const {
    const Blk& k = blk_[b];
    AttnArgs a;
    a.q = k.q; a.k = k.k; a.v = k.v; a.o = k.ao; a.lse = k.lse; a.B = last_.B; a.T = T; a.d = d; a.h = NH; a.ld = 3 * d;
    a.p = pdrop_; a.seed = last_.seed; a.site = SITE_BLK_BASE + 8 * b + 0;
    return a;
}
XaHost SlateModel::xattn_args(int b) const {
    const Blk& k = blk_[b];
    const unsigned site = SITE_BLK_BASE + 8 * b;
    XaHost hx;
    hx.x = k.ln2; hx.P = k.cP; hx.Ab = k.xaAb; hx.AbT = k.xaAbT; hx.Vo = k.xaVo; hx.VoT = k.xaVoT;
    hx.B = last_.B; hx.T = T; hx.K = K; hx.d = d; hx.h = NH; hx.p = pdrop_; hx.seed = last_.seed; hx.site_p = site + 2; hx.site_o = site + 3;
    return hx;
}

int SlateModel::fwd_decoder(const Lane& L, bool with_ce) {
    const int B = last_.B;
    const long long BT = (long long)B * T;
    const float p = pdrop_;
    RC(lin_fwd(slots_, D, P(w_.slotproj), nullptr, mem_, d, (long long)B * K, d, D, 0, nullptr, 0, 0.f, 0, L));
    RC(embed_fwd_launch(tokens_, P(w_.dict), P(w_.bos), P(w_.pe), emb_, B, T, d, p, last_.seed, L));
    const Lane F = side2_ ? dw_lane(L) : L;
    if (xattn_) {
        XaFoldHost f;
        f.mem = mem_; f.B = B; f.K = K; f.d = d; f.h = NH; f.nblk = NB;
        OCRL_REQUIRE(NB <= 8, "more than 8 decoder blocks: set OCRL_XATTN=0");
        for (int b = 0; b < NB; ++b) {
            const DecBlockW& bw = w_.blk[b];
            f.Wq[b] = P(bw.cq); f.Wk[b] = P(bw.ck); f.Wv[b] = P(bw.cv); f.Wo[b] = P(bw.co);
            f.ck[b] = blk_[b].ck; f.cv[b] = blk_[b].cv; f.Ab[b] = blk_[b].xaAb; f.AbT[b] = blk_[b].xaAbT; f.Vo[b] = blk_[b].xaVo; f.VoT[b] = blk_[b].xaVoT;
        }
        RC(after(F, L, ring_event()));
        RC(xattn_fold_fwd_launch(f, F));
    }
    const float* xin = emb_;
    for (int b = 0; b < NB; ++b) {
        Blk& k = blk_[b];
        const DecBlockW& bw = w_.blk[b];
        const unsigned site = SITE_BLK_BASE + 8 * b;
        RC(layernorm_fwd_launch(xin, P(bw.ln1.w), P(bw.ln1.b), k.ln1, k.ln1_mean, k.ln1_rstd, BT, d, L));
        const float* res = (b == 0) ? k.ln1 : xin;
        RC(lin_fwd(k.ln1, d, P(bw.qkv), nullptr, k.q, 3 * d, BT, 3 * d, d, 0, nullptr, 0, 0.f, 0, L));
        {
            const AttnArgs a = self_attn_args(b);
            RC(attn_launch(a, 0, L));
        }
        RC(lin_fwd(k.ao, d, P(bw.o), nullptr, k.x1, d, BT, d, d, 0, res, d, p, site + 1, L));
        RC(layernorm_fwd_launch(k.x1, P(bw.ln2.w), P(bw.ln2.b), k.ln2, k.ln2_mean, k.ln2_rstd, BT, d, L));
        if (xattn_) {
            if (b == 0) RC(after(L, F, ev_join2_));
            XaHost hx = xattn_args(b);
            hx.resid = k.x1; hx.y = k.x2;
            RC(xattn_launch(hx, 0, L));
        } else {
        RC(lin_fwd(k.ln2, d, P(bw.cq), nullptr, k.cq, d, BT, d, d, 0, nullptr, 0, 0.f, 0, L));
        RC(lin_fwd(mem_, d, P(bw.ck), nullptr, k.ck, d, (long long)B * K, d, d, 0, nullptr, 0, 0.f, 0, L));
        RC(lin_fwd(mem_, d, P(bw.cv), nullptr, k.cv, d, (long long)B * K, d, d, 0, nullptr, 0, 0.f, 0, L));
        RC(cross_attn_fwd_launch(k.cq, k.ck, k.cv, k.cao, k.cP, B, T, K, d, NH, p, last_.seed, site + 2, L));
        RC(lin_fwd(k.cao, d, P(bw.co), nullptr, k.x2, d, BT, d, d, 0, k.x1, d, p, site + 3, L));
        }
        RC(layernorm_fwd_launch(k.x2, P(bw.ln3.w), P(bw.ln3.b), k.ln3, k.ln3_mean, k.ln3_rstd, BT, d, L));
        RC(lin_fwd(k.ln3, d, P(bw.ffn0.w), P(bw.ffn0.b), k.f1, 4 * d, BT, 4 * d, d, 1, nullptr, 0, 0.f, 0, L));
        RC(lin_fwd(k.f1, 4 * d, P(bw.ffn2.w), P(bw.ffn2.b), k.x3, d, BT, d, 4 * d, 0, k.x2, d, p, site + 4, L));
        xin = k.x3;
    }
    RC(layernorm_fwd_launch(xin, P(w_.lnf.w), P(w_.lnf.b), lnf_, lnf_mean_, lnf_rstd_, BT, d, L));
    if (with_ce) {
        GemmArgs a;
        a.A = lnf_; a.B = P(w_.out); a.C = pred_; a.M = (int)BT; a.N = V; a.K = d; a.lda = d; a.ldb = d; a.ldc = V;
        a.epi_mode = 1; a.stat = cestat_;
        RC(gemm_launch(a, L));
        RC(softmax_stat_combine_launch(cestat_, gemm_stat_segments(V), BT, celse_, nullptr, nullptr, nullptr, pred_, V, tokens_, metrics_ + 1, 1.0f / B,
                                       cepart_, (size_t)(BT / 16 + 16), L));
    } else RC(lin_fwd(lnf_, d, P(w_.out), nullptr, pred_, V, BT, V, d, 0, nullptr, 0, 0.f, 0, L));
    return 0;
}

int SlateModel::forward(const StepInputs& in, hipStream_t st) {
    OCRL_REQUIRE(p_ && ws_, "forward: model not bound");
    OCRL_REQUIRE(in.B >= 1 && in.B <= Bmax, "forward: batch %d outside [1,%d]", in.B, Bmax);
    OCRL_REQUIRE(in.obs && in.tau > 0.f, "forward: bad inputs");
    last_ = in;
    have_enc_ = false;
    pdrop_ = in.train ? cfg.dropout : 0.f;
    const Lane L = main_lane(st);
    RC(pack_weights(L));
    if (cfg.use_bcdec) {
        RC(fwd_encoder(in, L));
        RC(pack_bcdec(L));
        RC(fwd_bcdec(L));
        RC(fill_launch(metrics_ + 1, 1, 0.f, L));
        RC(copy_launch(metrics_ + 0, metrics_ + 2, 1, L));
        have_fwd_ = true;
        return 0;
    }
    if (side_ && overlap_mode_ >= 2) {
        RC(fwd_encoder(in, L, overlap_mode_ == 4 ? 2 : (overlap_mode_ == 5 ? 3 : 1)));
        if (overlap_mode_ >= 3 && !getenv("OCRL_TOKENS_LATE")) {
            OCRL_HIP(hipStreamWaitEvent(L, ev_tokens_, 0));
            RC(fwd_decoder(L));
            RC(after(L, dvae_lane(), ev_join_));
            RC(copy_launch(metrics_ + 0, metrics_ + 2, 1, L));
            RC(axpy_launch(metrics_ + 1, metrics_ + 2, 1, 1.f, L));
            have_fwd_ = true;
            return 0;
        }
        RC(after(L, dvae_lane(), ev_join_));
    } else if (side_) {
        RC(after(dvae_lane(), L, ev_fork_));
        RC(fwd_dvae(in, dvae_lane()));
        RC(fwd_encoder(in, L));
        RC(after(L, dvae_lane(), ev_join_));
    } else {
        RC(fwd_dvae(in, L));
        RC(fwd_encoder(in, L));
    }
    RC(fwd_decoder(L));
    RC(copy_launch(metrics_ + 0, metrics_ + 2, 1, L));
    RC(axpy_launch(metrics_ + 1, metrics_ + 2, 1, 1.f, L));
    have_fwd_ = true;
    return 0;
}

int SlateModel::encode(const StepInputs& in, hipStream_t st) {
    OCRL_REQUIRE(p_ && ws_, "encode: model not bound");
    OCRL_REQUIRE(in.B >= 1 && in.B <= Bmax && in.obs, "encode: bad inputs");
    last_ = in;
    pdrop_ = 0.f;
    have_fwd_ = false;
    have_enc_ = true;
    const Lane L = main_lane(st);
    if (enc_graph_mode_ < 0) { const char* e = getenv("OCRL_ENCODE_GRAPH"); enc_graph_mode_ = e ? atoi(e) : 0; }
    const bool graph = enc_graph_mode_ && in.B <= 32 && !in.noise_slots && obs_stage_;
    const bool need_pack = !(frozen_ && packs_valid_);
    struct LowLat { int& f; LowLat(int& x) : f(x) { f = 1; } ~LowLat() { f = 0; } } lowlat(conv_lowlat_);
    if (!graph) {
        if (need_pack) RC(pack_weights(L, true));
        packs_valid_ = frozen_;
        return fwd_encoder(in, L);
    }
    EncGraph& eg = enc_graphs_[in.B];
    if (!eg.warm || need_pack) {
        eg.warm = 1;
        if (need_pack) RC(pack_weights(L, true));
        packs_valid_ = frozen_;
// ... 142 lines not shown
                GemmArgs gb;
                gb.M = K; gb.N = dh; gb.K = d; gb.akc = 1; gb.bkc = 1; gb.lda = d; gb.ldb = d; gb.ldc = d; gb.batch = B * NH; gb.batch_inner = NH; gb.alpha = scale;
                gb.A = xa_dAb_; gb.sA = (long long)NC * d; gb.sAi = (long long)KP * d;
                gb.B = Wq; gb.sB = 0; gb.sBi = (long long)dh * d;
                gb.C = gck_; gb.sC = (long long)K * d; gb.sCi = dh;
                RC(gemm_launch(gb, W));
                GemmArgs gc;
                gc.M = K; gc.N = dh; gc.K = d; gc.akc = 1; gc.bkc = 0; gc.lda = d; gc.ldb = d; gc.ldc = d; gc.batch = B * NH; gc.batch_inner = NH;
                gc.A = xa_dVo_; gc.sA = (long long)NC * d; gc.sAi = (long long)KP * d;
                gc.B = Wo; gc.sB = 0; gc.sBi = dh;
                gc.C = gcv_; gc.sC = (long long)K * d; gc.sCi = dh;
                RC(gemm_launch(gc, W));
                GemmArgs gq;
                gq.M = dh; gq.N = d; gq.K = K; gq.akc = 0; gq.bkc = 0; gq.lda = d; gq.ldb = d; gq.ldc = d; gq.batch = B * NH; gq.batch_inner = NH; gq.alpha = scale;
                gq.A = k.ck; gq.sA = (long long)K * d; gq.sAi = dh;
                gq.B = xa_dAb_; gq.sB = (long long)NC * d; gq.sBi = (long long)KP * d;
                gq.C = xa_pq_; gq.sC = (long long)d * d; gq.sCi = (long long)dh * d;
                RC(gemm_launch(gq, W));
                GemmArgs go;
                go.M = d; go.N = dh; go.K = K; go.akc = 0; go.bkc = 0; go.lda = d; go.ldb = d; go.ldc = d; go.batch = B * NH; go.batch_inner = NH;
                go.A = xa_dVo_; go.sA = (long long)NC * d; go.sAi = (long long)KP * d;
                go.B = k.cv; go.sB = (long long)K * d; go.sBi = dh;
                go.C = xa_po_; go.sC = (long long)d * d; go.sCi = dh;
                RC(gemm_launch(go, W));
                RC(colsum_launch(xa_pq_, (long long)d * d, G(bw.cq), B, d * d, 0, 1.f, W.scratch, W.scratch_floats, W));
                RC(colsum_launch(xa_po_, (long long)d * d, G(bw.co), B, d * d, 0, 1.f, W.scratch, W.scratch_floats, W));
            }
        } else {
        RC(lin_bwd_x(gd, d, P(bw.co), gt1_, d, BT, d, d, nullptr, 0, nullptr, 0, L));
        RC(cross_attn_bwd_launch(gt1_, k.cq, k.ck, k.cv, k.cP, q.gt2, gck_, gcv_, B, T, K, d, NH, p, last_.seed, site + 2, L.scratch, L.scratch_floats, L));
        RC(after(W, L, ring_event()));
        RC(lin_bwd_w(gd_co, d, k.cao, d, G(bw.co), nullptr, BT, d, d, 1.f, W));
        RC(lin_bwd_w(q.gt2, d, k.ln2, d, G(bw.cq), nullptr, BT, d, d, 1.f, W));
        RC(lin_bwd_x(q.gt2, d, P(bw.cq), gt1_, d, BT, d, d, nullptr, 0, nullptr, 0, L));
        }
        {
            const Lane& X = xattn_ ? W : L;
            RC(lin_bwd_w(gck_, d, mem_, d, G(bw.ck), nullptr, BK, d, d, 1.f, X));
            RC(lin_bwd_w(gcv_, d, mem_, d, G(bw.cv), nullptr, BK, d, d, 1.f, X));
            RC(lin_bwd_x(gck_, d, P(bw.ck), gmem_, d, BK, d, d, nullptr, 0, gmem_, d, X));
            RC(lin_bwd_x(gcv_, d, P(bw.cv), gmem_, d, BK, d, d, nullptr, 0, gmem_, d, X));
        }
        RC(layernorm_bwd_launch(gt1_, k.x1, k.ln2_mean, k.ln2_rstd, P(bw.ln2.w), gx_,
                                G(bw.ln2.w), BT, d, 1, 0, L.scratch, L.scratch_floats, L));
        RC(drop_gx(site + 1, q.gbr[2]));
        const float* gd_o = gd;
        RC(lin_bwd_x(gd, d, P(bw.o), gt1_, d, BT, d, d, nullptr, 0, nullptr, 0, L));
        {
            AttnArgs a = self_attn_args(b);
            a.dO = gt1_; a.dq = q.gqkv; a.dk = q.gqkv + d; a.dv = q.gqkv + 2 * d; a.delta = attn_delta_;
            RC(attn_launch(a, 1, L));
        }
        RC(after(W, L, ring_event()));
        RC(lin_bwd_w(gd_o, d, k.ao, d, G(bw.o), nullptr, BT, d, d, 1.f, W));
        RC(lin_bwd_w(q.gqkv, 3 * d, k.ln1, d, G(bw.qkv), nullptr, BT, 3 * d, d, 1.f, W));
        RC(lin_bwd_x(q.gqkv, 3 * d, P(bw.qkv), gt1_, d, BT, 3 * d, d, nullptr, 0, nullptr, 0, L));
        if (b == 0) {
            RC(axpy_launch(gx_, gt1_, BT * d, 1.f, L));
            RC(layernorm_bwd_launch(gt1_, xin, k.ln1_mean, k.ln1_rstd, P(bw.ln1.w), gx_,
                                    G(bw.ln1.w), BT, d, 0, 0, L.scratch, L.scratch_floats, L));
        } else {
            RC(layernorm_bwd_launch(gt1_, xin, k.ln1_mean, k.ln1_rstd, P(bw.ln1.w), gx_,
                                    G(bw.ln1.w), BT, d, 1, 0, L.scratch, L.scratch_floats, L));
        }
    }
    RC(embed_bwd_launch(gx_, tokens_, G(w_.dict), B, T, V, d, p, last_.seed, L.scratch, L.scratch_floats, L));
    RC(fill_launch(G(w_.pe), (long long)(T + 1) * d, 0.f, L));
    RC(colsum_launch(gx_, (long long)T * d, G(w_.pe), B, T * d, 0, 1.f, L.scratch, L.scratch_floats, L));
    RC(copy_launch(G(w_.pe), G(w_.bos), d, L));
    if (xattn_) RC(after(L, W, ring_event()));
    RC(lin_bwd_w(gmem_, d, slots_, D, G(w_.slotproj), nullptr, BK, d, D, 1.f, L));
    RC(lin_bwd_x(gmem_, d, P(w_.slotproj), gslots_, D, BK, d, D, nullptr, 0, nullptr, 0, L));
    return 0;
}

int SlateModel::bwd_encoder(const Lane& L, bool fork_dvae) {
    const int B = last_.B;
    const long long BN = (long long)B * N, R = (long long)B * I * K;
    const SaSave so = sa_save_layout(C, D, H, SH);
    const SaGrad go = sa_grad_layout(C, D, H, SH);
    const SlotAttnW& sa = w_.sa;
    SlotAttnArgs a;
    a.B = B; a.N = N; a.C = C; a.K = K; a.D = D; a.H = H; a.I = I; a.NH = SH; a.eps = 1e-8f; a.scale = 1.0f / sqrtf((float)(D / SH));
    a.x = x_; a.wts = sa_wts_; a.save = sa_save_; a.dslots = gslots_; a.dx = gA_; a.dslots0 = gslots0_; a.grows = sa_grows_; a.g_small = sa_small_;
    a.xchg = sa_xchg_; a.parts = sa_parts_;
    if (fork_dvae) {
        RC(after(dvae_lane(), L, ev_fork_));
        RC(bwd_dvae(dvae_lane()));
    }
    RC(slot_attn_launch(a, 1, L));
    const bool side_w = side_ && overlap_mode_ >= 3 && !cfg.use_bcdec && !fork_dvae;
    const Lane W = side_w ? dvae_lane() : L;
    if (side_w) RC(after(W, L, ev_fork_));
    const bool sa_in_bwd = sa_input_ == 1 && C == 64;
    RC(lin_bwd_w(sa_grows_ + go.out, go.ld, sa_save_ + so.hid, so.ld, G(sa.m2.w), G(sa.m2.b), R, D, H, 1.f, W));
    RC(lin_bwd_w(sa_grows_ + go.hid, go.ld, sa_save_ + so.m, so.ld, G(sa.m0.w), G(sa.m0.b), R, H, D, 1.f, W));
    RC(lin_bwd_w(sa_grows_ + go.gi, go.ld, sa_save_ + so.u, so.ld, G(sa.gru_wih), G(sa.gru_bih), R, 3 * D, D, 1.f, W));
    RC(lin_bwd_w(sa_grows_ + go.gh, go.ld, sa_save_ + so.sprev, so.ld, G(sa.gru_whh), G(sa.gru_bhh), R, 3 * D, D, 1.f, W));
    RC(lin_bwd_w(sa_grows_ + go.q, go.ld, sa_save_ + so.sn, so.ld, G(sa.q), nullptr, R, D, D, 1.f, W));
    for (int h = 0, dh = D / SH; h < SH; ++h) {
        RC(lin_bwd_w(sa_grows_ + go.u + h * dh, go.ld, sa_save_ + so.up + h * C, so.ld, G(sa.v) + (size_t)h * dh * C, nullptr, R, dh, C, 1.f, W));
        RC(lin_bwd_w(sa_save_ + so.q + h * dh, so.ld, sa_grows_ + go.qp + h * C, go.ld, G(sa.k) + (size_t)h * dh * C, nullptr, R, dh, C, a.scale, W));
    }
    const int SM = 4 * D + 2 * C;
    RC(colsum_launch(sa_small_ + 0, SM, G(sa.norm_slots.w), B, 2 * D, 0, 1.f, W.scratch, W.scratch_floats, W));
    RC(colsum_launch(sa_small_ + 2 * D, SM, G(sa.norm_mlp.w), B, 2 * D, 0, 1.f, W.scratch, W.scratch_floats, W));
    RC(colsum_launch(sa_small_ + 4 * D, SM, G(sa.norm_inputs.w), B, 2 * C, 0, 1.f, W.scratch, W.scratch_floats, W));
    RC(slot_init_bwd_launch(gslots0_, P(w_.sa.log_sigma), last_.noise_slots, G(w_.sa.mu), G(w_.sa.log_sigma),
                            B * K, D, last_.seed, W));
    if (!sa_in_bwd) RC(lin_bwd_w(gA_, C, h1_, C, G(w_.sa.mlp2.w), G(w_.sa.mlp2.b), BN, C, C, 1.f, W));
    if (side_w && !first_direct()) RC(im2col5_launch(obs8_, col0_, BN, S, S, cfg.obs_channels, (25 * cfg.obs_channels + 3) & ~3, W));
    if (sa_in_bwd) {
        const size_t slabs = L.scratch_floats / SA_INPUT_SLAB;
        OCRL_REQUIRE(slabs >= 1, "bwd_encoder: scratch too small for the input-chain slabs");
        RC(sa_input_bwd_launch(gA_, h1_, e4_, ln0_mean_, ln0_rstd_, P(w_.sa.ln.w), P(w_.sa.ln.b),
                               P(w_.sa.mlp0.w), P(w_.sa.mlp2.w), gB_, G(w_.sa.mlp0.w), G(w_.sa.mlp0.b),
                               G(w_.sa.mlp2.w), G(w_.sa.mlp2.b), G(w_.sa.ln.w), G(w_.sa.ln.b),
                               BN, slabs < 512 ? (int)slabs : 0, L.scratch, L.scratch_floats, L));
    } else {
        RC(lin_bwd_x(gA_, C, P(w_.sa.mlp2.w), gB_, C, BN, C, C, h1_, C, nullptr, 0, L));
        RC(lin_bwd_w(gB_, C, ln0_, C, G(w_.sa.mlp0.w), G(w_.sa.mlp0.b), BN, C, C, 1.f, L));
        float* gL = side_w ? gC_ : gA_;
        RC(lin_bwd_x(gB_, C, P(w_.sa.mlp0.w), gL, C, BN, C, C, nullptr, 0, nullptr, 0, L));
        RC(layernorm_bwd_launch(gL, e4_, ln0_mean_, ln0_rstd_, P(w_.sa.ln.w), gB_, G(w_.sa.ln.w), BN, C, 0, 0,
                                L.scratch, L.scratch_floats, L));
    }
    RC(colsum_launch(gB_, (long long)N * C, gmap_, B, N * C, 0, 1.f, L.scratch, L.scratch_floats, L));
    RC(lin_bwd_w(gmap_, C, gridT_, 4, G(w_.enc_pos.w), G(w_.enc_pos.b), N, C, 4, 1.f, L));
    if (fork_dvae || side_w) RC(after(L, dvae_lane(), ev_join_));
    if (dw_mode_ == 2 && side2_) RC(after(L, dw_lane(L), ev_join2_));
    RC(colsum_launch(gmap_, C, G(w_.enc[3].b), N, C, 0, 1.f, L.scratch, L.scratch_floats, L));
    RC(conv_layer_wgrad(e3_, gB_, G(w_.enc[3].w), nullptr, B, S, S, 5, 64, 64, L));
    RC(conv_layer_fwd(gB_, cw_bwd_[3], nullptr, gA_, B, S, S, 5, 64, 0, nullptr, e3_, L));
    RC(conv_layer_wgrad(e2_, gA_, G(w_.enc[2].w), G(w_.enc[2].b), B, S, S, 5, 64, 64, L));
    RC(conv_layer_fwd(gA_, cw_bwd_[2], nullptr, gB_, B, S, S, 5, 64, 0, nullptr, e2_, L));
    RC(conv_layer_wgrad(e1_, gB_, G(w_.enc[1].w), G(w_.enc[1].b), B, S, S, 5, 64, 64, L));
    RC(conv_layer_fwd(gB_, cw_bwd_[1], nullptr, gA_, B, S, S, 5, 64, 0, nullptr, e1_, L));
    if (first_direct()) {
        OCRL_REQUIRE(conv_first_wgrad_ws_floats(B, S, S) <= L.scratch_floats, "first conv wgrad: scratch too small");
        RC(conv_first_wgrad_launch(obs_keep_, gA_, L.scratch, G(w_.enc[0].w), G(w_.enc[0].b), B, S, S, 0, L));
    } else {
        const int ch = cfg.obs_channels, ldc0 = (25 * ch + 3) & ~3;
        if (!side_w) RC(im2col5_launch(obs8_, col0_, BN, S, S, ch, ldc0, L));
        RC(lin_bwd_w(gA_, 64, col0_, ldc0, dw0p_, G(w_.enc[0].b), BN, 64, ldc0, 1.f, L));
        RC(unpack5_launch(dw0p_, G(w_.enc[0].w), ch, ldc0, L));
    }
    return 0;
}

int SlateModel::bwd_dvae(const Lane& L) {
    const int B = last_.B;
    const long long BT = (long long)B * T, BN = (long long)B * N;
    const int ch = cfg.obs_channels;
    float* w4 = L.scratch + L.scratch_floats - 1024;
    {
        GemmArgs a;
        a.A = drecon_; a.B = ps2_; a.C = w4; a.M = 4; a.N = 64; a.K = (int)BN; a.lda = 4; a.ldb = 64; a.ldc = 64; a.akc = 0; a.bkc = 0;
        long long splits = BN / 512; if (splits > 512) splits = 512; if (splits < 1) splits = 1;
        if (splits > 1) {
            a.splitk = (int)splits; a.C = L.scratch; a.sCsplit = 256;
            RC(gemm_launch(a, L));
            RC(splitk_reduce_launch(L.scratch, w4, 256, (int)splits, 256, 0, L));
        } else RC(gemm_launch(a, L));
        RC(copy_launch(w4, G(w_.dvae_dec[11].w), ch * 64, L));
        RC(colsum_launch(drecon_, 4, w4 + 256, BN, 4, 0, 1.f, L.scratch, L.scratch_floats - 1024, L));
        RC(copy_launch(w4 + 256, G(w_.dvae_dec[11].b), ch, L));
    }
    RC(lin_bwd_x(drecon_, 4, w11p_, gdA_, 64, BN, 4, 64, nullptr, 0, nullptr, 0, L));
    RC(pixel_shuffle_launch(gdA_, gdB_, B, 2 * E, 2 * E, 64, 0, dd9_, L));
    RC(lin_bwd_w(gdB_, 256, dd8_, 64, G(w_.dvae_dec[9].w), G(w_.dvae_dec[9].b), 4 * BT, 256, 64, 1.f, L));
    RC(lin_bwd_x(gdB_, 256, P(w_.dvae_dec[9].w), gdA_, 64, 4 * BT, 256, 64, dd8_, 64, nullptr, 0, L));
    RC(lin_bwd_w(gdA_, 64, dd7_, 64, G(w_.dvae_dec[8].w), G(w_.dvae_dec[8].b), 4 * BT, 64, 64, 1.f, L));
    RC(lin_bwd_x(gdA_, 64, P(w_.dvae_dec[8].w), gdB_, 64, 4 * BT, 64, 64, dd7_, 64, nullptr, 0, L));
    RC(lin_bwd_w(gdB_, 64, dd6_, 64, G(w_.dvae_dec[7].w), G(w_.dvae_dec[7].b), 4 * BT, 64, 64, 1.f, L));
    RC(lin_bwd_x(gdB_, 64, P(w_.dvae_dec[7].w), gdA_, 64, 4 * BT, 64, 64, dd6_, 64, nullptr, 0, L));
    RC(conv_layer_wgrad(ps1_, gdA_, G(w_.dvae_dec[6].w), G(w_.dvae_dec[6].b), B, 2 * E, 2 * E, 3, 64, 64, L));
    RC(conv_layer_fwd(gdA_, dw_bwd_[1], nullptr, gdB_, B, 2 * E, 2 * E, 3, 64, 0, nullptr, ps1_, L));
    RC(pixel_shuffle_launch(gdB_, gdA_, B, E, E, 64, 0, nullptr, L));
    RC(lin_bwd_w(gdA_, 256, dd3_, 64, G(w_.dvae_dec[4].w), G(w_.dvae_dec[4].b), BT, 256, 64, 1.f, L));
    RC(lin_bwd_x(gdA_, 256, P(w_.dvae_dec[4].w), gdB_, 64, BT, 256, 64, dd3_, 64, nullptr, 0, L));
    RC(lin_bwd_w(gdB_, 64, dd2_, 64, G(w_.dvae_dec[3].w), G(w_.dvae_dec[3].b), BT, 64, 64, 1.f, L));
    RC(lin_bwd_x(gdB_, 64, P(w_.dvae_dec[3].w), gdA_, 64, BT, 64, 64, dd2_, 64, nullptr, 0, L));
    RC(lin_bwd_w(gdA_, 64, dd1_, 64, G(w_.dvae_dec[2].w), G(w_.dvae_dec[2].b), BT, 64, 64, 1.f, L));
    RC(lin_bwd_x(gdA_, 64, P(w_.dvae_dec[2].w), gdB_, 64, BT, 64, 64, dd1_, 64, nullptr, 0, L));
    RC(conv_layer_wgrad(dd0_, gdB_, G(w_.dvae_dec[1].w), G(w_.dvae_dec[1].b), B, E, E, 3, 64, 64, L));
    RC(conv_layer_fwd(gdB_, dw_bwd_[0], nullptr, gdA_, B, E, E, 3, 64, 0, nullptr, dd0_, L));
    float* dz = zraw_;
    have_scores_ = false;
    if (fused_heads()) {
        Xf zx; zx.b_mode = 2; zx.lse = zlse_;
        RC(lin_bwd_w(gdA_, 64, zraw_, V, G(w_.dvae_dec[0].w), G(w_.dvae_dec[0].b), BT, 64, V, 1.f, L, zx));
        RC(rowdot_bias64_launch(gdA_, dd0_, P(w_.dvae_dec[0].b), BT, zdot_, L));
        GemmArgs a;
        a.A = gdA_; a.B = P(w_.dvae_dec[0].w); a.C = dz; a.M = (int)BT; a.N = V; a.K = 64; a.lda = 64; a.ldb = V; a.ldc = V; a.bkc = 0;
        a.epi_mode = 3; a.mask = zraw_; a.ldmask = V; a.e_lse = zlse_; a.e_rowvec = zdot_; a.e_scale = 1.0f / last_.tau;
        RC(gemm_launch(a, L));
    } else {
    RC(lin_bwd_w(gdA_, 64, zdec_, V, G(w_.dvae_dec[0].w), G(w_.dvae_dec[0].b), BT, 64, V, 1.f, L));
    RC(lin_bwd_x(gdA_, 64, P(w_.dvae_dec[0].w), dz, V, BT, 64, V, nullptr, 0, nullptr, 0, L));
    RC(softmax_bwd_rows_launch(z_, dz, BT, V, 1.0f / last_.tau, L));
    }
    RC(lin_bwd_w(dz, V, de_[6], 64, G(w_.dvae_enc[7].w), G(w_.dvae_enc[7].b), BT, V, 64, 1.f, L));
    RC(lin_bwd_x(dz, V, P(w_.dvae_enc[7].w), gdA_, 64, BT, V, 64, de_[6], 64, nullptr, 0, L));
    float* cur = gdA_;
    float* oth = gdB_;
    for (int i = 6; i >= 1; --i) {
        RC(lin_bwd_w(cur, 64, de_[i - 1], 64, G(w_.dvae_enc[i].w), G(w_.dvae_enc[i].b), BT, 64, 64, 1.f, L));
        RC(lin_bwd_x(cur, 64, P(w_.dvae_enc[i].w), oth, 64, BT, 64, 64, de_[i - 1], 64, nullptr, 0, L));
        float* t = cur; cur = oth; oth = t;
    }
    RC(lin_bwd_w(cur, 64, patches_, 16 * ch, G(w_.dvae_enc[0].w), G(w_.dvae_enc[0].b), BT, 64, 16 * ch, 1.f, L));
    return 0;
}

int SlateModel::backward(hipStream_t st) {
    OCRL_REQUIRE(have_fwd_, "backward: call forward first");
    OCRL_REQUIRE(g_, "backward: no gradient buffer bound");
    enc_only_grads_ = false;
    const Lane L = main_lane(st);
    if (cfg.use_bcdec) {
        RC(fill_launch(g_, flat_size_, 0.f, L));
        RC(bwd_bcdec(L));
        RC(bwd_encoder(L));
        have_fwd_ = false;
        return 0;
    }
    if (side_ && overlap_mode_ == 2) {
        RC(bwd_decoder(L));
        RC(bwd_encoder(L, true));
    } else if (side_ && overlap_mode_ >= 3) {
        RC(after(dvae_lane(), L, ev_fork_));
        RC(bwd_dvae(dvae_lane()));
        RC(bwd_decoder(L));
        if (!dw_mode_) RC(after(L, dvae_lane(), ev_join_));
        RC(bwd_encoder(L));
    } else if (side_) {
        RC(after(dvae_lane(), L, ev_fork_));
        RC(bwd_dvae(dvae_lane()));
        RC(bwd_decoder(L));
        RC(bwd_encoder(L));
        RC(after(L, dvae_lane(), ev_join_));
    } else {
        RC(bwd_decoder(L));
        RC(bwd_encoder(L));
        RC(bwd_dvae(L));
    }
    have_fwd_ = false;
    return 0;
}

int SlateModel::after(const Lane& waiter, const Lane& producer, hipEvent_t ev) {
    if (waiter.st == producer.st) return 0;
    OCRL_HIP(hipEventRecord(ev, producer.st));
    OCRL_HIP(hipStreamWaitEvent(waiter.st, ev, 0));
    return 0;
}

int SlateModel::grad_norm(hipStream_t st) {
    const Lane L = main_lane(st);
    return absmax_launch(g_, flat_size_, metrics_ + 3, L.scratch, L.scratch_floats, L);
}

int SlateModel::clip_adam(const float lr[3], float clip, int step, float gscale, hipStream_t st) {
    OCRL_REQUIRE(m_ && v_, "clip_adam: optimiser state not bound");
    packs_valid_ = false;
    RC(grad_norm(st));
    if (enc_only_grads_) {
        const long long b0 = group_begin_[1], end = w_.enc_grads_end;
        return clip_adam_launch(p_ + b0, g_ + b0, m_ + b0, v_ + b0, end - b0, metrics_ + 3, clip, lr[1], 0.9, 0.999, 1e-8, step, gscale, st);
    }
    for (int g = 0; g < 3; ++g) {
        if (cfg.use_bcdec && g != 1) continue;
        const long long b0 = group_begin_[g], n = group_begin_[g + 1] - b0;
        RC(clip_adam_launch(p_ + b0, g_ + b0, m_ + b0, v_ + b0, n, metrics_ + 3, clip, lr[g], 0.9, 0.999, 1e-8, step, gscale, st));
    }
    return 0;
}

int SlateModel::pack_bcdec(const Lane& L) {
    RC(bc_compose_launch(P(w_.bc[0].w), P(w_.bc_pos.w), P(w_.bc_pos.b), bc_Wc_,
                         bc_W1r_, D, L));
    RC(conv_pack_launch(P(w_.bc[1].w), bc_pk_[0], bc_pkb_[0], 5, 64, 64, 64, L));
    RC(conv_pack_launch(P(w_.bc[2].w), bc_pk_[1], bc_pkb_[1], 5, 64, 64, 64, L));
    if (conv_x3_ > 0) {
        for (int i = 0; i < 2; ++i) {
            auto f = x3_of_.find(bc_pk_[i]), b = x3_of_.find(bc_pkb_[i]);
            if (f != x3_of_.end()) RC(conv_pack_x3_launch(P(w_.bc[i + 1].w), const_cast<float*>(f->second), b != x3_of_.end() ? const_cast<float*>(b->second) : nullptr, L));
        }
    }
    RC(bc_c4_pack_launch(P(w_.bc[3].w), bc_Wk4_, bc_Wb4_, cfg.obs_channels + 1, L));
    return 0;
}

int SlateModel::fwd_bcdec(const Lane& L) {
    const int B = last_.B, BK = B * K;
    RC(bc_posconv_launch(bc_Wc_, bc_P1_, S, L));
    RC(lin_fwd(slots_, D, bc_W1r_, nullptr, bc_M_, 1600, BK, 1600, D, 0, nullptr, 0, 0.f, 0, L));
    RC(bcast_l1_class_sum_launch(bc_M_, bc_T_, BK, 5, 1, L));
    RC(bcast_l1_fwd_launch(bc_P1_, bc_T_, P(w_.bc[0].b), bc_c1_, BK, S, 5, BCAST_L1_RELU, L));
    RC(conv_layer_fwd(bc_c1_, bc_pk_[0], P(w_.bc[1].b), bc_c2_, BK, S, S, 5, 64, 1, nullptr, nullptr, L));
    RC(conv_layer_fwd(bc_c2_, bc_pk_[1], P(w_.bc[2].b), bc_c3_, BK, S, S, 5, 64, 1, nullptr, nullptr, L));
    RC(bc_c4_fwd_launch(bc_c3_, bc_Wk4_, P(w_.bc[3].b), bc_out4_, BK, S, L));
    RC(bc_mix_launch(bc_out4_, last_.obs, recon_, bc_dout4_, metrics_ + 0, B, K, S, cfg.obs_channels, L.scratch, L.scratch_floats, L));
    return 0;
}

int SlateModel::bwd_bcdec(const Lane& L) {
    const int B = last_.B, BK = B * K;
    const long long BKN = (long long)BK * N;
    const int nb = bc_c4_wgrad_blocks(BK, S);
    RC(bc_c4_wgrad_launch(bc_c3_, bc_dout4_, L.scratch, BK, S, L));
    RC(colsum_launch(L.scratch, 4 * 64 * 9, G(w_.bc[3].w), nb, 4 * 64 * 9, 0, 1.f, L.scratch + (size_t)nb * 2304, L.scratch_floats - (size_t)nb * 2304, L));
    RC(colsum_launch(bc_dout4_, 4, G(w_.bc[3].b), BKN, cfg.obs_channels + 1, 0, 1.f, L.scratch, L.scratch_floats, L));
    RC(bc_c4_bwd_data_launch(bc_dout4_, bc_Wb4_, bc_c3_, bc_gA_, BK, S, L));
    RC(conv_layer_wgrad(bc_c2_, bc_gA_, G(w_.bc[2].w), G(w_.bc[2].b), BK, S, S, 5, 64, 64, L));
    RC(conv_layer_fwd(bc_gA_, bc_pkb_[1], nullptr, bc_gB_, BK, S, S, 5, 64, 0, nullptr, bc_c2_, L));
    RC(conv_layer_wgrad(bc_c1_, bc_gB_, G(w_.bc[1].w), G(w_.bc[1].b), BK, S, S, 5, 64, 64, L));
    RC(conv_layer_fwd(bc_gB_, bc_pkb_[0], nullptr, bc_gA_, BK, S, S, 5, 64, 0, nullptr, bc_c1_, L));
    RC(bcast_l1_bwd_launch(bc_gA_, bc_dT_, BK, S, 5, L.scratch, L.scratch_floats, L));
    RC(colsum_launch(bc_dT_, 64, G(w_.bc[0].b), (long long)BK * 25, 64, 0, 1.f, L.scratch, L.scratch_floats, L));
    RC(bcast_l1_class_sum_launch(bc_dT_, bc_dM_, BK, 5, 0, L));
    RC(lin_bwd_x(bc_dM_, 1600, bc_W1r_, gslots_, D, BK, 1600, D, nullptr, 0, nullptr, 0, L));
    RC(lin_bwd_w(bc_dM_, 1600, slots_, D, bc_dW1r_, nullptr, BK, 1600, D, 1.f, L));
    RC(colsum_launch(bc_gA_, (long long)N * 64, bc_G1_, BK, N * 64, 0, 1.f, L.scratch, L.scratch_floats, L));
// ... 6 lines not shown
```

ocrl_amd/csrc/slate_model.h:

```cpp
#pragma once
#include <map>
#include <string>
#include <vector>

#include "kernels.h"
#include "model_base.h"

struct SlateConfig {
    int obs_size = 64, obs_channels = 3, vocab = 4096, d_model = 192, cnn_hidden = 64;
    int num_slots = 5, num_iters = 3, slot_size = 192, mlp_hidden = 192;
    int num_blocks = 4, num_heads = 4;
    float dropout = 0.1f;
    int max_batch = 1;
    int use_bcdec = 0;
    int hard = 0;
    int slot_heads = 1;
};

struct StepInputs {
    const float* obs = nullptr;
    int B = 0;
    float tau = 1.f;
    int train = 1;
    unsigned long long seed = 0;
    const float* noise_z = nullptr;
    const float* noise_zh = nullptr;
    const float* noise_slots = nullptr;
    const unsigned long long* seed_dev = nullptr;
};

struct Lane {
    hipStream_t st = nullptr;
    float* scratch = nullptr;
    size_t scratch_floats = 0;
    operator hipStream_t() const { return st; }
};

class SlateModel : public ModelBase {
public:
    explicit SlateModel(const SlateConfig& c);
    ~SlateModel();
    long long group_begin(int g) const { return group_begin_[g]; }
    int bind(float* p, float* g, float* m, float* v, void* ws, size_t ws_bytes);
    int forward(const StepInputs& in, hipStream_t st);
    int backward(hipStream_t st);
    int encode(const StepInputs& in, hipStream_t st);
    void freeze_weights(bool on) { frozen_ = on; packs_valid_ = false; clear_encode_graphs(); }
    void clear_encode_graphs();
    int encode_backward(const float* dslots, hipStream_t st);
    int generate(hipStream_t st);
    int clip_adam(const float lr[3], float clip, int step, float gscale, hipStream_t st);
    int grad_norm(hipStream_t st);
    int dropout_mask(unsigned site, long long n, float* out, hipStream_t st) const;
    int soft_z(hipStream_t st);
    const SlateConfig cfg;

private:
    void layout_workspace(bool commit);
    int lin_fwd(const float* x, int ldx, const float* W, const float* b, float* y, int ldy, long long M, int N, int K, int relu,
                const float* resid, int ldr, float drop_p, unsigned site, hipStream_t st) {
        return ::lin_fwd(x, ldx, W, b, y, ldy, M, N, K, relu, resid, ldr, st, Drop{drop_p, last_.seed, site});
    }
    int lin_bwd_w(const float* dy, int ld_dy, const float* x, int ldx, float* dW, float* db, long long M, int N_out, int K_in,
                  float alpha, const Lane& L, Xf xf = Xf()) {
        return ::lin_bwd_w(dy, ld_dy, x, ldx, dW, db, M, N_out, K_in, alpha, L.scratch, L.scratch_floats, L.st, Drop(), xf);
    }
    bool fused_heads() const { return !cfg.hard; }
    int conv_layer_fwd(const float* x, const float* pack, const float* bias, float* y, int Bn, int Hh, int Ww, int KS, int CIN, int relu,
                       const float* posmap, const float* mask, const Lane& L);
    int conv_layer_wgrad(const float* x, const float* dy, float* dW, float* db, int Bn, int Hh, int Ww, int KS, int CIN, int cin_real,
                         const Lane& L);
    int pack_weights(const Lane& L, bool encoder_only = false);
    int fwd_encoder(const StepInputs& in, const Lane& L, int fork_dvae = 0);
    int fwd_dvae(const StepInputs& in, const Lane& L);
    int fwd_decoder(const Lane& L, bool with_ce = true);
    int dvae_decode(int B, float* drecon, const Lane& L, const float* zin = nullptr);
    int bwd_decoder(const Lane& L);
    int bwd_encoder(const Lane& L, bool fork_dvae = false);
    int bwd_dvae(const Lane& L);
    int pack_bcdec(const Lane& L);
    int fwd_bcdec(const Lane& L);
    int bwd_bcdec(const Lane& L);
    AttnArgs self_attn_args(int b) const;
    XaHost xattn_args(int b) const;

    Lane main_lane(hipStream_t st) const { return Lane{st, scratch_, scratch_floats_}; }
    Lane dvae_lane() const { return Lane{side_, scratch2_, scratch_floats_}; }
    Lane dw_lane(const Lane& main) const { return dw_mode_ == 2 ? Lane{side2_, scratch3_, scratch_floats_} : dw_mode_ ? dvae_lane() : main; }
    int after(const Lane& waiter, const Lane& producer, hipEvent_t ev);
    hipEvent_t ring_event() { return ev_dw_[ev_dw_next_++ & 7]; }

    struct DecBlockW { ParamPair ln1, ln2, ln3, ffn0, ffn2; ParamRef qkv, o, cq, ck, cv, co; };
    struct SlotAttnW {
        ParamRef mu, log_sigma, q, k, v, gru_wih, gru_whh, gru_bih, gru_bhh;
        ParamPair ln, mlp0, mlp2, norm_inputs, norm_slots, norm_mlp, m0, m2;
    };
    struct Weights {
        ParamPair dvae_enc[8], dvae_dec[12];
        ParamPair enc[4], enc_pos;
        SlotAttnW sa;
        ParamPair bc[4], bc_pos;
        ParamRef slotproj, dict, bos, pe, out;
        ParamPair lnf;
        std::vector<DecBlockW> blk;
        long long enc_grads_end = 0;
    } w_;
    void resolve_params();

    long long group_begin_[4] = {0, 0, 0, 0};

    int S, E, T, N, V, d, C, K, I, D, H, NB, NH, DH, Bmax;
    int SH = 1;
    StepInputs last_;
    float pdrop_ = 0.f;
    bool have_fwd_ = false;
    int conv_lowlat_ = 0;
    bool frozen_ = false, packs_valid_ = false;
    bool have_enc_ = false;
    bool enc_only_grads_ = false;
    bool have_scores_ = false;

    float *scratch_ = nullptr;
    size_t scratch_floats_ = 0;
    float* scratch2_ = nullptr;
    int overlap_mode_ = 0;
    hipStream_t side_ = nullptr;
    hipEvent_t ev_fork_ = nullptr, ev_join_ = nullptr, ev_tokens_ = nullptr;
    float *zstat_ = nullptr, *zhstat_ = nullptr, *zlse_ = nullptr, *zdot_ = nullptr, *cestat_ = nullptr, *celse_ = nullptr, *cepart_ = nullptr;
    int* zhidx_ = nullptr;
    float *obs8_, *patches_, *de_[7], *zraw_, *z_, *zdec_;
    int* tokens_;
    float *dd0_, *dd1_, *dd2_, *dd3_, *dd4_, *ps1_, *dd6_, *dd7_, *dd8_, *dd9_, *ps2_, *recon_, *drecon_;
    float *e1_, *e2_, *e3_, *e4_, *posmap_, *gridT_, *ln0_, *ln0_mean_, *ln0_rstd_, *h1_, *x_;
    float *slots0_, *slot_noise_, *slots_, *attn_, *sa_save_, *sa_wts_, *sa_grows_, *sa_small_, *sa_xchg_;
    float* attn_heads_ = nullptr;
    float* sa_parts_;
    PackEntry* sa_pack_dev_ = nullptr;
    int sa_pack_n_ = 0, sa_pack_max_ = 0;
    float *cw_fwd_[4], *cw_bwd_[4];
    int conv_x3_ = -1;
    std::map<const float*, const float*> x3_of_;
    float *dw_fwd_[2], *dw_bwd_[2];
    float *w11p_;
    float *mem_, *emb_;
    struct Blk {
        float *ln1, *ln1_mean, *ln1_rstd, *q, *k, *v, *lse, *ao, *x1;
        float *ln2, *ln2_mean, *ln2_rstd, *cq, *ck, *cv, *cP, *cao, *x2;
        float *ln3, *ln3_mean, *ln3_rstd, *f1, *x3;
        float *xaAb, *xaAbT, *xaVo, *xaVoT;
    };
    int sa_input_ = 1;
    bool xattn_ = false;
    float *xa_dAb_ = nullptr, *xa_dVo_ = nullptr, *xa_pq_ = nullptr, *xa_po_ = nullptr;
    size_t xa_zero_floats_ = 0;
    float* xa_zero_base_ = nullptr;
    std::vector<Blk> blk_;
    struct BlkG { float *gbr[3], *gf1, *gt2, *gqkv, *xaPd, *xaDs; };
    std::vector<BlkG> bg_;
    struct EncGraph { hipGraphExec_t exec = nullptr; int warm = 0; };
    std::map<int, EncGraph> enc_graphs_;
    int enc_graph_mode_ = -1;
    hipStream_t cap_ = nullptr;
    float* obs_stage_ = nullptr;
    unsigned long long* seed_dev_ = nullptr;
    int dw_mode_ = 0;
    hipStream_t side2_ = nullptr;
    float* scratch3_ = nullptr;
    hipEvent_t ev_dw_[8] = {nullptr, nullptr, nullptr, nullptr, nullptr, nullptr, nullptr, nullptr};
    hipEvent_t ev_join2_ = nullptr;
    int ev_dw_next_ = 0;
    float *attn_delta_;
    float *lnf_, *lnf_mean_, *lnf_rstd_, *pred_;
    float *gqkv_;
    float *gx_, *gbr_, *gt1_, *gt2_, *gt3_, *gf1_, *gmem_, *gck_, *gcv_, *gslots_, *gslots0_;
    float *gA_, *gB_, *gC_;
    float *gdA_, *gdB_;
    float *gmap_;
    float *col0_, *dw0p_;
    float* obs_keep_ = nullptr;
    bool first_direct() const { return cfg.obs_channels == 3; }
    float *bc_Wc_, *bc_W1r_, *bc_P1_, *bc_M_, *bc_T_, *bc_c1_, *bc_c2_, *bc_c3_, *bc_out4_, *bc_dout4_, *bc_gA_, *bc_gB_;
    float *bc_pk_[2], *bc_pkb_[2], *bc_Wk4_, *bc_Wb4_, *bc_dW1r_, *bc_dWc_, *bc_dT_, *bc_dM_, *bc_G1_;
};
```

Baseline: 1762.

## Fuse dVAE decoder head (linear, pixel shuffle, 1x1 conv, MSE) fwd and bwd

Adds dedicated forward and backward kernels for the last stage of the dVAE decoder. The forward kernel does the 64->256 linear with ReLU on MFMA, applies the pixel shuffle in LDS, runs the 64->C output projection and computes the MSE partials in one pass. The backward kernel fuses the output-projection gradient, the shuffle-back, the ReLU mask, the dW9 MFMA accumulation and dX into per-block slabs, followed by a small reduce kernel. The goal is to cut several launches and the intermediate ps2 round trips through global memory. In exchange it uses heavy LDS in the backward pass, changes the reduction order and is gated by the OCRL_DVAE_HEAD environment variable, which is on by default.

```diff
diff --git a/include/ocrl_hip.h b/include/ocrl_hip.h
--- a/include/ocrl_hip.h
+++ b/include/ocrl_hip.h
@@ -114,6 +114,15 @@
 int ocrl_layernorm_bwd(const float* dy, const float* x, const float* mean, const float* rstd, const float* gamma, float* dx, float* dgb,
                        long long R, int F, float* ws, size_t ws_floats, void* stream);
 
+int ocrl_pixel_shuffle(const float* in, float* out, int B, int h, int w, int cout, int forward, const float* mask, void* stream);
+int ocrl_mse_loss(const float* obs, const float* recon, float* drecon, float* out, int B, int C, int H, int W, float* ws, size_t ws_floats, void* stream);
+
+int ocrl_dvae_head_plan(long long R, int out[3]);
+int ocrl_dvae_head_fwd(const float* dd8, const float* W9, const float* b9, const float* W11, const float* b11, const float* obs, float* dd9,
+                       float* recon, float* drecon, float* mse, int B, int S, int C, int max_wgs, float* ws, size_t ws_floats, void* stream);
+int ocrl_dvae_head_bwd(const float* drecon, const float* dd9, const float* dd8, const float* W9, const float* W11, float* ddd8, float* dW9,
+                       float* db9, float* dW11, float* db11, int B, int S, int C, int max_wgs, float* ws, size_t ws_floats, void* stream);
+
 int ocrl_sa_input_plan(long long R, int out[3]);
 int ocrl_sa_input_fwd(const float* e4, const float* gamma, const float* beta, const float* W0, const float* b0, const float* W2, const float* b2,
                       float* mean, float* rstd, float* h1, float* x, long long R, int max_wgs, void* stream);
diff --git a/ocrl_amd/_lib.py b/ocrl_amd/_lib.py
--- a/ocrl_amd/_lib.py
+++ b/ocrl_amd/_lib.py
@@ -169,6 +169,11 @@
     L.ocrl_sa_input_plan.argtypes = [c_longlong, POINTER(c_int * 3)]
     L.ocrl_sa_input_fwd.argtypes = [p] * 11 + [c_longlong, c_int, p]
     L.ocrl_sa_input_bwd.argtypes = [p] * 16 + [c_longlong, c_int, p, c_size_t, p]
+    L.ocrl_pixel_shuffle.argtypes = [p, p, c_int, c_int, c_int, c_int, c_int, p, p]
+    L.ocrl_mse_loss.argtypes = [p, p, p, p, c_int, c_int, c_int, c_int, p, c_size_t, p]
+    L.ocrl_dvae_head_plan.argtypes = [c_longlong, POINTER(c_int * 3)]
+    L.ocrl_dvae_head_fwd.argtypes = [p] * 10 + [c_int, c_int, c_int, c_int, p, c_size_t, p]
+    L.ocrl_dvae_head_bwd.argtypes = [p] * 10 + [c_int, c_int, c_int, c_int, p, c_size_t, p]
     L.ocrl_attention_fwd.argtypes = [p, p, p, p, p, c_int, c_int, c_int, c_int, c_int, c_float, c_ulonglong, c_uint, p]
     L.ocrl_attention_bwd.argtypes = [p, p, p, p, p, p, p, p, p, p, c_int, c_int, c_int, c_int, c_int, c_float, c_ulonglong, c_uint, p]
     L.ocrl_obs_u8_to_f32.argtypes = [p, p, c_int, c_int, c_int, c_int, p]
diff --git a/ocrl_amd/csrc/capi.cpp b/ocrl_amd/csrc/capi.cpp
--- a/ocrl_amd/csrc/capi.cpp
+++ b/ocrl_amd/csrc/capi.cpp
@@ -316,6 +316,29 @@
     return layernorm_bwd_launch(dy, x, mean, rstd, g, dx, dgb, R, F, 0, 0, ws, ws_floats, ST(stream));
 }
 
+int ocrl_pixel_shuffle(const float* in, float* out, int B, int h, int w, int cout, int forward, const float* mask, void* stream) {
+    if (!in || !out || B <= 0 || h <= 0 || w <= 0 || cout <= 0) { ocrl_set_error("ocrl_pixel_shuffle: bad arguments"); return 1; }
+    return pixel_shuffle_launch(in, out, B, h, w, cout, forward, mask, ST(stream));
+}
+int ocrl_mse_loss(const float* obs, const float* recon, float* drecon, float* out, int B, int C, int H, int W, float* ws, size_t ws_floats, void* stream) {
+    if (!obs || !recon || !out || !ws || B <= 0) { ocrl_set_error("ocrl_mse_loss: bad arguments"); return 1; }
+    return mse_launch(obs, recon, drecon, out, B, C, H, W, ws, ws_floats, ST(stream));
+}
+
+int ocrl_dvae_head_plan(long long R, int out[3]) {
+    if (!out || R <= 0) { ocrl_set_error("ocrl_dvae_head_plan: needs R > 0 and an output array"); return 1; }
+    dvae_head_plan(R, 0, out);
+    return 0;
+}
+int ocrl_dvae_head_fwd(const float* dd8, const float* W9, const float* b9, const float* W11, const float* b11, const float* obs, float* dd9,
+                       float* recon, float* drecon, float* mse, int B, int S, int C, int max_wgs, float* ws, size_t ws_floats, void* stream) {
+    return dvae_head_fwd_launch(dd8, W9, b9, W11, b11, obs, dd9, recon, drecon, mse, B, S, C, max_wgs, ws, ws_floats, ST(stream));
+}
+int ocrl_dvae_head_bwd(const float* drecon, const float* dd9, const float* dd8, const float* W9, const float* W11, float* ddd8, float* dW9,
+                       float* db9, float* dW11, float* db11, int B, int S, int C, int max_wgs, float* ws, size_t ws_floats, void* stream) {
+    return dvae_head_bwd_launch(drecon, dd9, dd8, W9, W11, ddd8, dW9, db9, dW11, db11, B, S, C, max_wgs, ws, ws_floats, ST(stream));
+}
+
 int ocrl_sa_input_plan(long long R, int out[3]) {
     if (!out || R <= 0) { ocrl_set_error("ocrl_sa_input_plan: needs R > 0 and an output array"); return 1; }
     sa_input_plan(R, 0, out);
diff --git a/ocrl_amd/csrc/dvae_head.hip b/ocrl_amd/csrc/dvae_head.hip
--- /dev/null
+++ b/ocrl_amd/csrc/dvae_head.hip
@@ -0,0 +1,406 @@
+#include "common.h"
+#include "kernels.h"
+
+#define DVH_TR 64
+#define DVH_LD8 68
+#define DVH_LDG 260
+#define DVH_FWD_MAX_WGS 512
+#define DVH_BWD_MAX_WGS 256
+#define DVH_BWD_LDS_FLOATS (DVH_TR * DVH_LDG + 256 * 64 + DVH_TR * DVH_LD8 + DVH_TR * 16)
+
+__device__ __forceinline__ float4 dvh_ld4(const float* __restrict__ p, long long row, long long R, int ld, int c4) {
+    const float4 v = *reinterpret_cast<const float4*>(p + (row < R ? row : R - 1) * ld + c4 * 4);
+    return row < R ? v : make_float4(0.f, 0.f, 0.f, 0.f);
+}
+__device__ __forceinline__ void dvh_pixel(long long row, int hw, int s, long long& b, int& py, int& px) {
+    const long long per = (long long)hw * hw;
+    b = row / per;
+    const int rem = (int)(row - b * per);
+    py = 2 * (rem / hw) + (s >> 1);
+    px = 2 * (rem % hw) + (s & 1);
+}
+
+__global__ __launch_bounds__(256, 2) void dvae_head_fwd_kernel(const float* __restrict__ dd8, const float* __restrict__ W9, const float* __restrict__ b9,
+                                                               const float* __restrict__ W11, const float* __restrict__ b11,
+                                                               const float* __restrict__ obs, float* __restrict__ dd9, float* __restrict__ recon,
+                                                               float* __restrict__ drecon, float* __restrict__ part, long long R, int hw, int C,
+                                                               float inv_b) {
+    __shared__ __attribute__((aligned(16))) float At[DVH_TR * DVH_LD8], Pt[4 * 32 * 36], Rp[4 * DVH_TR * 12], W11s[64 * 4];
+    const int lane = threadIdx.x & 63, wv = threadIdx.x >> 6, li = lane & 31, lh = lane >> 5;
+    float w9f[2][8][4], b9v[2];
+#pragma unroll
+    for (int j = 0; j < 2; ++j) {
+        const int n = 64 * wv + 32 * j + li;
+#pragma unroll
+        for (int c = 0; c < 8; ++c) {
+            const float4 a = *reinterpret_cast<const float4*>(W9 + n * 64 + c * 8 + 4 * lh);
+            w9f[j][c][0] = a.x; w9f[j][c][1] = a.y; w9f[j][c][2] = a.z; w9f[j][c][3] = a.w;
+        }
+        b9v[j] = b9[n];
+    }
+    if (threadIdx.x < 64) {
+        const int c = threadIdx.x;
+        *reinterpret_cast<float4*>(W11s + c * 4) = make_float4(W11[c], C > 1 ? W11[64 + c] : 0.f, C > 2 ? W11[128 + c] : 0.f, 0.f);
+    }
+    const float b11v[3] = {b11[0], C > 1 ? b11[1] : 0.f, C > 2 ? b11[2] : 0.f};
+    const long long ntiles = (R + DVH_TR - 1) / DVH_TR;
+    const int c4 = threadIdx.x & 15, lr0 = threadIdx.x >> 4;
+    const int rr0 = lane >> 3, c8 = lane & 7;
+    const int prow = lane >> 1, sp = lane & 1;
+    const int S = 2 * hw;
+    float4 v[4];
+#pragma unroll
+    for (int i = 0; i < 4; ++i) v[i] = dvh_ld4(dd8, (long long)blockIdx.x * DVH_TR + lr0 + 16 * i, R, 64, c4);
+    double se = 0.0;
+    for (long long tile = blockIdx.x; tile < ntiles; tile += gridDim.x) {
+        const long long r0 = tile * DVH_TR;
+#pragma unroll
+        for (int i = 0; i < 4; ++i) *reinterpret_cast<float4*>(At + (lr0 + 16 * i) * DVH_LD8 + c4 * 4) = v[i];
+#pragma unroll
+        for (int i = 0; i < 4; ++i) v[i] = dvh_ld4(dd8, (tile + gridDim.x) * DVH_TR + lr0 + 16 * i, R, 64, c4);
+        __syncthreads();
+        f32x16 acc[2][2];
+#pragma unroll
+        for (int i = 0; i < 2; ++i)
+#pragma unroll
+            for (int j = 0; j < 2; ++j)
+#pragma unroll
+                for (int r = 0; r < 16; ++r) acc[i][j][r] = 0.f;
+#pragma unroll
+        for (int c = 0; c < 8; ++c) {
+            const float4 a0 = *reinterpret_cast<const float4*>(At + li * DVH_LD8 + c * 8 + 4 * lh);
+            const float4 a1 = *reinterpret_cast<const float4*>(At + (32 + li) * DVH_LD8 + c * 8 + 4 * lh);
+            const float f0[4] = {a0.x, a0.y, a0.z, a0.w}, f1[4] = {a1.x, a1.y, a1.z, a1.w};
+#pragma unroll
+            for (int s = 0; s < 4; ++s)
+#pragma unroll
+                for (int j = 0; j < 2; ++j) {
+                    acc[0][j] = __builtin_amdgcn_mfma_f32_32x32x2f32(f0[s], w9f[j][c][s], acc[0][j], 0, 0, 0);
+                    acc[1][j] = __builtin_amdgcn_mfma_f32_32x32x2f32(f1[s], w9f[j][c][s], acc[1][j], 0, 0, 0);
+                }
+        }
+        float* const patch = Pt + wv * (32 * 36);
+#pragma unroll
+        for (int i = 0; i < 2; ++i) {
+            float pa[2][3] = {{0.f, 0.f, 0.f}, {0.f, 0.f, 0.f}};
+#pragma unroll
+            for (int j = 0; j < 2; ++j) {
+#pragma unroll
+                for (int r = 0; r < 16; ++r) patch[((r & 3) + 8 * (r >> 2) + 4 * lh) * 36 + li] = fmaxf(acc[i][j][r] + b9v[j], 0.f);
+                __builtin_amdgcn_wave_barrier();
+#pragma unroll
+                for (int ps = 0; ps < 4; ++ps) {
+                    const int rr = ps * 8 + rr0;
+                    const long long row = r0 + 32 * i + rr;
+                    const float4 o = *reinterpret_cast<const float4*>(patch + rr * 36 + c8 * 4);
+                    if (row < R) *reinterpret_cast<float4*>(dd9 + row * 256 + 64 * wv + 32 * j + c8 * 4) = o;
+                }
+#pragma unroll
+                for (int cc = 0; cc < 8; ++cc) {
+                    const float2 x = *reinterpret_cast<const float2*>(patch + prow * 36 + 4 * cc + 2 * sp);
+                    const float4 w = *reinterpret_cast<const float4*>(W11s + (16 * wv + 8 * j + cc) * 4);
+                    pa[0][0] += x.x * w.x; pa[0][1] += x.x * w.y; pa[0][2] += x.x * w.z;
+                    pa[1][0] += x.y * w.x; pa[1][1] += x.y * w.y; pa[1][2] += x.y * w.z;
+                }
+                __builtin_amdgcn_wave_barrier();
+            }
+            float* const rp = Rp + (wv * DVH_TR + 32 * i + prow) * 12 + 6 * sp;
+            rp[0] = pa[0][0]; rp[1] = pa[0][1]; rp[2] = pa[0][2]; rp[3] = pa[1][0]; rp[4] = pa[1][1]; rp[5] = pa[1][2];
+        }
+        __syncthreads();
+        {
+            const int lr = threadIdx.x >> 2, s = threadIdx.x & 3;
+            const long long row = r0 + lr;
+            if (row < R) {
+                float rc[3], d[3] = {0.f, 0.f, 0.f};
+#pragma unroll
+                for (int o = 0; o < 3; ++o)
+                    rc[o] = ((Rp[(0 * DVH_TR + lr) * 12 + s * 3 + o] + Rp[(1 * DVH_TR + lr) * 12 + s * 3 + o]) +
+                             (Rp[(2 * DVH_TR + lr) * 12 + s * 3 + o] + Rp[(3 * DVH_TR + lr) * 12 + s * 3 + o])) + b11v[o];
+                long long b;
+                int py, px;
+                dvh_pixel(row, hw, s, b, py, px);
+#pragma unroll
+                for (int o = 0; o < 3; ++o) {
+                    if (o < C) {
+                        const float e = rc[o] - obs[((b * C + o) * S + py) * S + px];
+                        se += (double)e * (double)e;
+                        d[o] = 2.f * e * inv_b;
+                    } else rc[o] = 0.f;
+                }
+                const long long pix = (b * S + py) * S + px;
+                *reinterpret_cast<float4*>(recon + pix * 4) = make_float4(rc[0], rc[1], rc[2], 0.f);
+                if (drecon) *reinterpret_cast<float4*>(drecon + pix * 4) = make_float4(d[0], d[1], d[2], 0.f);
+            }
+        }
+    }
+    __syncthreads();
+    double* const red = reinterpret_cast<double*>(Rp);
+    red[threadIdx.x] = se;
+    __syncthreads();
+    if (threadIdx.x < 16) {
+        double t = red[threadIdx.x * 16];
+#pragma unroll
+        for (int k = 1; k < 16; ++k) t += red[threadIdx.x * 16 + k];
+        red[256 + threadIdx.x] = t;
+    }
+    __syncthreads();
+    if (threadIdx.x == 0) {
+        double t = red[256];
+#pragma unroll
+        for (int k = 1; k < 16; ++k) t += red[256 + k];
+        part[blockIdx.x] = (float)t;
+    }
+}
+
+__global__ __launch_bounds__(512, 1) void dvae_head_bwd_kernel(const float* __restrict__ drecon, const float* __restrict__ dd9, const float* __restrict__ dd8,
+                                                               const float* __restrict__ W9, const float* __restrict__ W11,
+                                                               float* __restrict__ ddd8, float* __restrict__ slab, long long R, int hw, int C) {
+    extern __shared__ __attribute__((aligned(16))) float dvh_smem[];
+    float* const G = dvh_smem;
+    float* const W9s = G + DVH_TR * DVH_LDG;
+    float* const D8 = W9s + 256 * 64;
+    float* const DR = D8 + DVH_TR * DVH_LD8;
+    const int lane = threadIdx.x & 63, wv = __builtin_amdgcn_readfirstlane(threadIdx.x >> 6), li = lane & 31, lh = lane >> 5;
+#pragma unroll
+    for (int i = 0; i < 8; ++i)
+        *reinterpret_cast<float4*>(W9s + (threadIdx.x + 512 * i) * 4) = *reinterpret_cast<const float4*>(W9 + (threadIdx.x + 512 * i) * 4);
+    const int s1 = wv & 3, i1 = wv >> 2;
+    float w11f[2][4];
+#pragma unroll
+    for (int j = 0; j < 2; ++j)
+#pragma unroll
+        for (int k = 0; k < 4; ++k) w11f[j][k] = (lh == 0 && k < C) ? W11[k * 64 + 32 * j + li] : 0.f;
+    const int S = 2 * hw;
+    const long long ntiles = (R + DVH_TR - 1) / DVH_TR;
+    const int g4 = threadIdx.x & 63, gr0 = threadIdx.x >> 6, e4 = threadIdx.x & 15, er0 = threadIdx.x >> 4;
+    const int pr = (threadIdx.x >> 2) & 63, psub = threadIdx.x & 3;
+    float4 gn[8], en[2], dn;
+    auto load_tile = [&](long long tile) {
+        const long long r0 = tile * DVH_TR;
+#pragma unroll
+        for (int i = 0; i < 8; ++i) gn[i] = dvh_ld4(dd9, r0 + gr0 + 8 * i, R, 256, g4);
+#pragma unroll
+        for (int i = 0; i < 2; ++i) en[i] = dvh_ld4(dd8, r0 + er0 + 32 * i, R, 64, e4);
+        if (threadIdx.x < 256) {
+            const long long row = r0 + pr;
+            long long b;
+            int py, px;
+            dvh_pixel(row < R ? row : R - 1, hw, psub, b, py, px);
+            const float4 t = *reinterpret_cast<const float4*>(drecon + ((b * S + py) * S + px) * 4);
+            dn = row < R ? t : make_float4(0.f, 0.f, 0.f, 0.f);
+        }
+    };
+    f32x16 dWa[2];
+#pragma unroll
+    for (int j = 0; j < 2; ++j)
+#pragma unroll
+        for (int r = 0; r < 16; ++r) dWa[j][r] = 0.f;
+    double db9a[2] = {0.0, 0.0}, db11[3] = {0.0, 0.0, 0.0};
+    float dw11a[3] = {0.f, 0.f, 0.f};
+    dn = make_float4(0.f, 0.f, 0.f, 0.f);
+    load_tile(blockIdx.x);
+    for (long long tile = blockIdx.x; tile < ntiles; tile += gridDim.x) {
+        const long long r0 = tile * DVH_TR;
+        __syncthreads();
+#pragma unroll
+        for (int i = 0; i < 8; ++i) *reinterpret_cast<float4*>(G + (gr0 + 8 * i) * DVH_LDG + g4 * 4) = gn[i];
+#pragma unroll
+        for (int i = 0; i < 2; ++i) *reinterpret_cast<float4*>(D8 + (er0 + 32 * i) * DVH_LD8 + e4 * 4) = en[i];
+        if (threadIdx.x < 256) {
+            *reinterpret_cast<float4*>(DR + threadIdx.x * 4) = dn;
+            db11[0] += dn.x; db11[1] += dn.y; db11[2] += dn.z;
+        }
+        load_tile(tile + gridDim.x);
+        __syncthreads();
+#pragma unroll 2
+        for (int i = 0; i < 8; ++i) {
+            const int row = 8 * wv + i;
+            const float4 m = *reinterpret_cast<const float4*>(G + row * DVH_LDG + g4 * 4);
+            const float4 d0 = *reinterpret_cast<const float4*>(DR + row * 16), d1 = *reinterpret_cast<const float4*>(DR + row * 16 + 4);
+            const float4 d2 = *reinterpret_cast<const float4*>(DR + row * 16 + 8), d3 = *reinterpret_cast<const float4*>(DR + row * 16 + 12);
+            dw11a[0] += (d0.x * m.x + d1.x * m.y) + (d2.x * m.z + d3.x * m.w);
+            dw11a[1] += (d0.y * m.x + d1.y * m.y) + (d2.y * m.z + d3.y * m.w);
+            dw11a[2] += (d0.z * m.x + d1.z * m.y) + (d2.z * m.z + d3.z * m.w);
+        }
+        __syncthreads();
+        {
+            float4 a = *reinterpret_cast<const float4*>(DR + (32 * i1 + li) * 16 + 4 * s1);
+            if (lh) a = make_float4(0.f, 0.f, 0.f, 0.f);
+#pragma unroll
+            for (int j = 0; j < 2; ++j) {
+                f32x16 g;
+#pragma unroll
+                for (int r = 0; r < 16; ++r) g[r] = 0.f;
+                g = __builtin_amdgcn_mfma_f32_32x32x2f32(a.x, w11f[j][0], g, 0, 0, 0);
+                g = __builtin_amdgcn_mfma_f32_32x32x2f32(a.y, w11f[j][1], g, 0, 0, 0);
+                g = __builtin_amdgcn_mfma_f32_32x32x2f32(a.z, w11f[j][2], g, 0, 0, 0);
+                g = __builtin_amdgcn_mfma_f32_32x32x2f32(a.w, w11f[j][3], g, 0, 0, 0);
+#pragma unroll
+                for (int r = 0; r < 16; ++r) {
+                    const int row = 32 * i1 + (r & 3) + 8 * (r >> 2) + 4 * lh;
+                    float* const p = G + row * DVH_LDG + 4 * (32 * j + li) + s1;
+                    const float m = *p;
+                    const float t = m > 0.f ? g[r] : 0.f;
+                    *p = t;
+                    db9a[j] += (double)t;
+                }
+            }
+        }
+        __syncthreads();
+        if (wv < 4) {
+            const int wm0 = (wv >> 1) * 32, wn0 = (wv & 1) * 32;
+            f32x16 acc;
+#pragma unroll
+            for (int r = 0; r < 16; ++r) acc[r] = 0.f;
+#pragma unroll 4
+            for (int c = 0; c < 32; ++c) {
+                const float4 a = *reinterpret_cast<const float4*>(G + (wm0 + li) * DVH_LDG + c * 8 + 4 * lh);
+                const float* const wk = W9s + (c * 8 + 4 * lh) * 64 + wn0 + li;
+                acc = __builtin_amdgcn_mfma_f32_32x32x2f32(a.x, wk[0], acc, 0, 0, 0);
+                acc = __builtin_amdgcn_mfma_f32_32x32x2f32(a.y, wk[64], acc, 0, 0, 0);
+                acc = __builtin_amdgcn_mfma_f32_32x32x2f32(a.z, wk[128], acc, 0, 0, 0);
+                acc = __builtin_amdgcn_mfma_f32_32x32x2f32(a.w, wk[192], acc, 0, 0, 0);
+            }
+#pragma unroll
+            for (int r = 0; r < 16; ++r) {
+                const int lr = wm0 + (r & 3) + 8 * (r >> 2) + 4 * lh;
+                const float mk = D8[lr * DVH_LD8 + wn0 + li];
+                float t = acc[r];
+                t = mk > 0.f ? t : 0.f * t * (mk + 1.f);
+                if (r0 + lr < R) ddd8[(r0 + lr) * 64 + wn0 + li] = t;
+            }
+        }
+        {
+            const int m0 = 32 * wv;
+#pragma unroll 2
+            for (int c = 0; c < 8; ++c) {
+                float fa[4], fb[2][4];
+#pragma unroll
+                for (int j = 0; j < 4; ++j) {
+                    const int k = c * 8 + 4 * lh + j;
+                    fa[j] = G[k * DVH_LDG + m0 + li];
+                    fb[0][j] = D8[k * DVH_LD8 + li]; fb[1][j] = D8[k * DVH_LD8 + 32 + li];
+                }
+#pragma unroll
+                for (int s = 0; s < 4; ++s)
+#pragma unroll
+                    for (int ni = 0; ni < 2; ++ni) dWa[ni] = __builtin_amdgcn_mfma_f32_32x32x2f32(fa[s], fb[ni][s], dWa[ni], 0, 0, 0);
+            }
+        }
+    }
+    float* const sl = slab + (size_t)blockIdx.x * DVAE_HEAD_SLAB;
+#pragma unroll
+    for (int ni = 0; ni < 2; ++ni)
+#pragma unroll
+        for (int r = 0; r < 16; ++r) sl[(32 * wv + (r & 3) + 8 * (r >> 2) + 4 * lh) * 64 + 32 * ni + li] = dWa[ni][r];
+    __syncthreads();
+    double* const red9 = reinterpret_cast<double*>(G);
+    double* const redb = red9 + 1024;
+    double* const redb2 = redb + 1024;
+    float* const red11 = G + 2 * (1024 + 1024 + 64);
+#pragma unroll
+    for (int j = 0; j < 2; ++j) {
+        red9[(i1 * 2 + lh) * 256 + 4 * (32 * j + li) + s1] = db9a[j];
+    }
+#pragma unroll
+    for (int o = 0; o < 3; ++o) red11[wv * 192 + o * 64 + g4] = dw11a[o];
+    if (threadIdx.x < 256) { redb[threadIdx.x * 4] = db11[0]; redb[threadIdx.x * 4 + 1] = db11[1]; redb[threadIdx.x * 4 + 2] = db11[2]; redb[threadIdx.x * 4 + 3] = 0.0; }
+    __syncthreads();
+    if (threadIdx.x < 256) {
+        const int q = threadIdx.x;
+        sl[16384 + q] = (float)((red9[q] + red9[256 + q]) + (red9[512 + q] + red9[768 + q]));
+    } else if (threadIdx.x < 448) {
+        const int q = threadIdx.x - 256;
+        float t = red11[q];
+#pragma unroll
+        for (int k = 1; k < 8; ++k) t += red11[k * 192 + q];
+        sl[16640 + q] = t;
+    } else {
+        const int q = threadIdx.x - 448, comp = q & 3, grp = q >> 2;
+        double t = redb[(grp * 16) * 4 + comp];
+#pragma unroll
+        for (int k = 1; k < 16; ++k) t += redb[(grp * 16 + k) * 4 + comp];
+        redb2[grp * 4 + comp] = t;
+    }
+    __syncthreads();
+    if (threadIdx.x < 4) {
+        double t = redb2[threadIdx.x];
+#pragma unroll
+        for (int k = 1; k < 16; ++k) t += redb2[k * 4 + threadIdx.x];
+        sl[16832 + threadIdx.x] = (float)t;
+    }
+}
+
+__global__ __launch_bounds__(256) void dvae_head_reduce_kernel(const float* __restrict__ slab, int nslab, float* __restrict__ dW9, float* __restrict__ db9,
+                                                               float* __restrict__ dW11, float* __restrict__ db11, int C) {
+    __shared__ float red[8][32];
+    const int ci = threadIdx.x & 31, grp = threadIdx.x >> 5, col = blockIdx.x * 32 + ci;
+    const int per = (nslab + 7) / 8, s0 = grp * per, s1 = min(nslab, s0 + per);
+    float a = 0.f;
+    if (col < DVAE_HEAD_SLAB)
+        for (int s = s0; s < s1; ++s) a += slab[(size_t)s * DVAE_HEAD_SLAB + col];
+    red[grp][ci] = a;
+    __syncthreads();
+    if (threadIdx.x < 32 && col < DVAE_HEAD_SLAB) {
+        float t = red[0][ci];
+#pragma unroll
+        for (int k = 1; k < 8; ++k) t += red[k][ci];
+        if (col < 16384) dW9[col] = t;
+        else if (col < 16640) db9[col - 16384] = t;
+        else if (col < 16832) { if ((col - 16640) / 64 < C) dW11[col - 16640] = t; }
+        else if (col - 16832 < C) db11[col - 16832] = t;
+    }
+}
+
+void dvae_head_plan(long long R, int max_wgs, int out[3]) {
+    const long long ntiles = (R + DVH_TR - 1) / DVH_TR;
+    long long wgs = max_wgs > 0 && max_wgs < DVH_BWD_MAX_WGS ? max_wgs : DVH_BWD_MAX_WGS;
+    if (wgs > ntiles) wgs = ntiles;
+    out[0] = DVH_TR; out[1] = (int)wgs; out[2] = DVAE_HEAD_SLAB;
+}
+
+static int dvh_shape(const char* who, int B, int S, int C, long long* R) {
+    OCRL_REQUIRE(B > 0 && S > 0 && S % 2 == 0, "%s: needs B > 0 and an even image size (B=%d S=%d)", who, B, S);
+    OCRL_REQUIRE(C >= 1 && C <= 3, "%s: obs_channels must be 1..3 (got %d)", who, C);
+    *R = (long long)B * (S / 2) * (S / 2);
+    return 0;
+}
+
+int dvae_head_fwd_launch(const float* dd8, const float* W9, const float* b9, const float* W11, const float* b11, const float* obs, float* dd9,
+                         float* recon, float* drecon, float* mse_out, int B, int S, int C, int max_wgs, float* ws, size_t ws_floats, hipStream_t st) {
+    long long R;
+    RC(dvh_shape("dvae_head_fwd", B, S, C, &R));
+    OCRL_REQUIRE(dd8 && W9 && b9 && W11 && b11 && obs && dd9 && recon && mse_out && ws, "dvae_head_fwd: null argument");
+    OCRL_REQUIRE(aligned16(dd8, W9, dd9, recon, drecon), "dvae_head_fwd: tensors must be 16-byte aligned");
+    const long long ntiles = (R + DVH_TR - 1) / DVH_TR;
+    long long wgs = max_wgs > 0 && max_wgs < DVH_FWD_MAX_WGS ? max_wgs : DVH_FWD_MAX_WGS;
+    if (wgs > ntiles) wgs = ntiles;
+    OCRL_REQUIRE((size_t)wgs <= ws_floats, "dvae_head_fwd: workspace too small (%d partials)", (int)wgs);
+    hipLaunchKernelGGL(dvae_head_fwd_kernel, dim3((unsigned)wgs), dim3(256), 0, st, dd8, W9, b9, W11, b11, obs, dd9, recon, drecon, ws, R, S / 2, C,
+                       1.0f / B);
+    OCRL_CHECK_LAUNCH("dvae_head_fwd");
+    return reduce_partials_launch(ws, (int)wgs, mse_out, 1.0f / B, 0, st);
+}
+
+int dvae_head_bwd_launch(const float* drecon, const float* dd9, const float* dd8, const float* W9, const float* W11, float* ddd8, float* dW9,
+                         float* db9, float* dW11, float* db11, int B, int S, int C, int max_wgs, float* ws, size_t ws_floats, hipStream_t st) {
+    long long R;
+    RC(dvh_shape("dvae_head_bwd", B, S, C, &R));
+    OCRL_REQUIRE(drecon && dd9 && dd8 && W9 && W11 && ddd8 && dW9 && db9 && dW11 && db11 && ws, "dvae_head_bwd: null argument");
+    OCRL_REQUIRE(aligned16(drecon, dd9, dd8, W9, ws), "dvae_head_bwd: tensors must be 16-byte aligned");
+    int plan[3];
+    dvae_head_plan(R, max_wgs, plan);
+    OCRL_REQUIRE((size_t)plan[1] * DVAE_HEAD_SLAB <= ws_floats, "dvae_head_bwd: workspace too small (%d slabs of %d floats)", plan[1], DVAE_HEAD_SLAB);
+    constexpr int smem = DVH_BWD_LDS_FLOATS * 4;
+    static bool attr_set = false;
+    if (!attr_set) {
+        OCRL_HIP(hipFuncSetAttribute((const void*)dvae_head_bwd_kernel, hipFuncAttributeMaxDynamicSharedMemorySize, smem));
+        attr_set = true;
+    }
+    hipLaunchKernelGGL(dvae_head_bwd_kernel, dim3(plan[1]), dim3(512), smem, st, drecon, dd9, dd8, W9, W11, ddd8, ws, R, S / 2, C);
+    OCRL_CHECK_LAUNCH("dvae_head_bwd");
+    hipLaunchKernelGGL(dvae_head_reduce_kernel, dim3((DVAE_HEAD_SLAB + 31) / 32), dim3(256), 0, st, ws, plan[1], dW9, db9, dW11, db11, C);
+    OCRL_CHECK_LAUNCH("dvae_head_reduce");
+    return 0;
+}
diff --git a/ocrl_amd/csrc/kernels.h b/ocrl_amd/csrc/kernels.h
--- a/ocrl_amd/csrc/kernels.h
+++ b/ocrl_amd/csrc/kernels.h
@@ -245,6 +245,12 @@
                         const float* W0, const float* W2, float* de4, float* dW0, float* db0, float* dW2, float* db2, float* dgamma, float* dbeta,
                         long long R, int max_wgs, float* ws, size_t ws_floats, hipStream_t st);
 int reduce_partials_launch(const float* part, int n, float* out, float scale, int accumulate, hipStream_t st);
+#define DVAE_HEAD_SLAB (256 * 64 + 256 + 3 * 64 + 4)
+void dvae_head_plan(long long R, int max_wgs, int out[3]);
+int dvae_head_fwd_launch(const float* dd8, const float* W9, const float* b9, const float* W11, const float* b11, const float* obs, float* dd9,
+                         float* recon, float* drecon, float* mse_out, int B, int S, int C, int max_wgs, float* ws, size_t ws_floats, hipStream_t st);
+int dvae_head_bwd_launch(const float* drecon, const float* dd9, const float* dd8, const float* W9, const float* W11, float* ddd8, float* dW9,
+                         float* db9, float* dW11, float* db11, int B, int S, int C, int max_wgs, float* ws, size_t ws_floats, hipStream_t st);
 int mse_launch(const float* obs, const float* recon, float* drecon, float* out, int B, int C, int H, int W, float* ws, size_t ws_floats, hipStream_t st);
 int gumbel_softmax_launch(const float* raw, const float* e1, const float* e2, float* z, int* tokens, long long R, int V, float tau,
                           unsigned long long seed, hipStream_t st, float* zst = nullptr);
diff --git a/ocrl_amd/csrc/slate_model.cpp b/ocrl_amd/csrc/slate_model.cpp
--- a/ocrl_amd/csrc/slate_model.cpp
+++ b/ocrl_amd/csrc/slate_model.cpp
@@ -217,7 +217,8 @@
     dd0_ = carve("dvae_dec0", BT * 64); dd1_ = carve("dvae_dec1", BT * 64); dd2_ = carve("dvae_dec2", BT * 64); dd3_ = carve("dvae_dec3", BT * 64);
     dd4_ = carve("dvae_dec4", BT * 256); ps1_ = carve(nullptr, BT * 256);
     dd6_ = carve("dvae_dec6", BT * 256); dd7_ = carve("dvae_dec7", BT * 256); dd8_ = carve("dvae_dec8", BT * 256);
-    dd9_ = carve("dvae_dec9", BT * 1024); ps2_ = carve(nullptr, BN * 64);
+    if (dvae_head_ < 0) { const char* e = getenv("OCRL_DVAE_HEAD"); dvae_head_ = e ? atoi(e) : 1; }
+    dd9_ = carve("dvae_dec9", BT * 1024); ps2_ = dvae_head_fused() ? nullptr : carve(nullptr, BN * 64);
     recon_ = carve("recon", BN * 4); drecon_ = carve(nullptr, BN * 4);
     for (int i = 0; i < 2; ++i) {
         dw_fwd_[i] = carve(nullptr, 9 * 64 * 64); dw_bwd_[i] = carve(nullptr, 9 * 64 * 64);
@@ -227,7 +228,7 @@
             if (ws_commit_) { x3_of_[dw_fwd_[i]] = f3; x3_of_[dw_bwd_[i]] = b3; }
         }
     }
-    w11p_ = carve(nullptr, 4 * 64);
+    w11p_ = dvae_head_fused() ? nullptr : carve(nullptr, 4 * 64);
     mem_ = carve("mem", BK * d); emb_ = carve("emb", BT * d);
     for (int b = 0; b < NB; ++b) {
         Blk& k = blk_[b];
@@ -392,8 +393,10 @@
                 if (f != x3_of_.end()) RC(conv_pack_x3_launch(P(w_.dvae_dec[i ? 6 : 1].w), const_cast<float*>(f->second), b != x3_of_.end() ? const_cast<float*>(b->second) : nullptr, L, 3));
             }
         }
-        RC(copy_launch(P(w_.dvae_dec[11].w), w11p_, cfg.obs_channels * 64, L));
-        RC(fill_launch(w11p_ + cfg.obs_channels * 64, (4 - cfg.obs_channels) * 64, 0.f, L));
+        if (!dvae_head_fused()) {
+            RC(copy_launch(P(w_.dvae_dec[11].w), w11p_, cfg.obs_channels * 64, L));
+            RC(fill_launch(w11p_ + cfg.obs_channels * 64, (4 - cfg.obs_channels) * 64, 0.f, L));
+        }
     }
     RC(pack_launch(sa_pack_dev_, sa_pack_n_, sa_pack_max_, sa_wts_, L));
     RC(posmap_launch(P(w_.enc_pos.w), P(w_.enc_pos.b), posmap_, S, C, L));
@@ -490,6 +493,10 @@
     RC(conv_layer_fwd(ps1_, dw_fwd_[1], P(w_.dvae_dec[6].b), dd6_, B, 2 * E, 2 * E, 3, 64, 1, nullptr, nullptr, L));
     RC(lin_fwd(dd6_, 64, P(w_.dvae_dec[7].w), P(w_.dvae_dec[7].b), dd7_, 64, 4 * BT, 64, 64, 1, nullptr, 0, 0.f, 0, L));
     RC(lin_fwd(dd7_, 64, P(w_.dvae_dec[8].w), P(w_.dvae_dec[8].b), dd8_, 64, 4 * BT, 64, 64, 1, nullptr, 0, 0.f, 0, L));
+    if (dvae_head_fused()) {
+        return dvae_head_fwd_launch(dd8_, P(w_.dvae_dec[9].w), P(w_.dvae_dec[9].b), P(w_.dvae_dec[11].w), P(w_.dvae_dec[11].b), last_.obs, dd9_,
+                                    recon_, drecon, metrics_ + (drecon ? 0 : 4), B, S, ch, 0, L.scratch, L.scratch_floats, L);
+    }
     RC(lin_fwd(dd8_, 64, P(w_.dvae_dec[9].w), P(w_.dvae_dec[9].b), dd9_, 256, 4 * BT, 256, 64, 1, nullptr, 0, 0.f, 0, L));
     RC(pixel_shuffle_launch(dd9_, ps2_, B, 2 * E, 2 * E, 64, 1, nullptr, L));
     RC(lin_fwd(ps2_, 64, P(w_.dvae_dec[11].w), P(w_.dvae_dec[11].b), recon_, 4, BN, ch, 64, 0, nullptr, 0, 0.f, 0, L));
@@ -938,6 +945,12 @@
     const int B = last_.B;
     const long long BT = (long long)B * T, BN = (long long)B * N;
     const int ch = cfg.obs_channels;
+    if (dvae_head_fused()) {
+        const size_t slabs = L.scratch_floats / DVAE_HEAD_SLAB;
+        OCRL_REQUIRE(slabs >= 1, "bwd_dvae: scratch too small for the decoder-head slabs");
+        RC(dvae_head_bwd_launch(drecon_, dd9_, dd8_, P(w_.dvae_dec[9].w), P(w_.dvae_dec[11].w), gdA_, G(w_.dvae_dec[9].w), G(w_.dvae_dec[9].b),
+                                G(w_.dvae_dec[11].w), G(w_.dvae_dec[11].b), B, S, ch, slabs < 256 ? (int)slabs : 0, L.scratch, L.scratch_floats, L));
+    } else {
     float* w4 = L.scratch + L.scratch_floats - 1024;
     {
         GemmArgs a;
@@ -956,6 +969,7 @@
     RC(pixel_shuffle_launch(gdA_, gdB_, B, 2 * E, 2 * E, 64, 0, dd9_, L));
     RC(lin_bwd_w(gdB_, 256, dd8_, 64, G(w_.dvae_dec[9].w), G(w_.dvae_dec[9].b), 4 * BT, 256, 64, 1.f, L));
     RC(lin_bwd_x(gdB_, 256, P(w_.dvae_dec[9].w), gdA_, 64, 4 * BT, 256, 64, dd8_, 64, nullptr, 0, L));
+    }
     RC(lin_bwd_w(gdA_, 64, dd7_, 64, G(w_.dvae_dec[8].w), G(w_.dvae_dec[8].b), 4 * BT, 64, 64, 1.f, L));
     RC(lin_bwd_x(gdA_, 64, P(w_.dvae_dec[8].w), gdB_, 64, 4 * BT, 64, 64, dd7_, 64, nullptr, 0, L));
     RC(lin_bwd_w(gdB_, 64, dd6_, 64, G(w_.dvae_dec[7].w), G(w_.dvae_dec[7].b), 4 * BT, 64, 64, 1.f, L));
diff --git a/ocrl_amd/csrc/slate_model.h b/ocrl_amd/csrc/slate_model.h
--- a/ocrl_amd/csrc/slate_model.h
+++ b/ocrl_amd/csrc/slate_model.h
@@ -142,6 +142,8 @@
     std::map<const float*, const float*> x3_of_;
     float *dw_fwd_[2], *dw_bwd_[2];
     float *w11p_;
+    int dvae_head_ = -1;
+    bool dvae_head_fused() const { return dvae_head_ != 0 && cfg.obs_channels <= 3 && S % 2 == 0; }
     float *mem_, *emb_;
     struct Blk {
         float *ln1, *ln1_mean, *ln1_rstd, *q, *k, *v, *lse, *ao, *x1;
```

Result: no change. 1775 (median of 6 runs) (+0.7%).
